# Tariq-Abuhashim/semantic-slam

Measured on AMD Instinct MI355X. Metric: Mvoxels/sec integrated, 512³ grid @ 640×480 depth; achieved HBM GB/s %peak, higher is better.
Workload: dtype f32

## Files before the change

### include/tsdf_hip_diag.h

```cpp
#ifndef TSDF_HIP_DIAG_H
#define TSDF_HIP_DIAG_H

#include "tsdf_hip.h"

#ifdef __cplusplus
extern "C" {
#endif


int tsdf_integrate_sequence_timed(tsdf_volume *vol, const float *depth_dev, const float *cam2world,
                                  int32_t n_frames, float *elapsed_ms);

int tsdf_integrate_frames_timed(tsdf_volume *vol, const float *const *depth_dev, const uint8_t *const *masks_dev,
                                const float *cam2world, int32_t n_frames, float *elapsed_ms);


int tsdf_probe_graph_replay(tsdf_volume *vol, const float *depth_dev, const float *cam2world, int32_t n_frames,
                            int32_t iters, float *ms_launches, float *ms_graph);

int tsdf_probe_stream(tsdf_volume *vol, int32_t non_temporal, int32_t n_iters, float *elapsed_ms);


int tsdf_selftest_fastdiv(int32_t device, uint64_t seed, uint64_t n_samples, float fx, float cx,
                          uint64_t *mismatches, float first_bad[4]);

int tsdf_selftest_fastdiv_band(int32_t device, uint64_t seed, uint64_t n_samples, uint64_t *mismatches,
                               float first_bad[4]);

int tsdf_selftest_round(int32_t device, uint64_t *mismatches, float first_bad[4]);

int tsdf_selftest_tile_tables(int32_t device, const float *depth_dev, const uint8_t *mask_dev, int32_t im_height,
                              int32_t im_width, float max_depth, uint64_t *mismatches);


int32_t tsdf_frames_per_launch(const tsdf_volume *vol);
int tsdf_shortcut_stats(tsdf_volume *vol, int32_t enable, uint64_t counts_out[3]);
int tsdf_brick_list_stats(tsdf_volume *vol, uint64_t counts_out[4]);
int tsdf_classification_info(tsdf_volume *vol, double info_out[2]);

int tsdf_last_cam2base(const tsdf_volume *vol, float out[16]);


int tsdf_set_kernel_variant(tsdf_volume *vol, int32_t variant);

int tsdf_set_brick_shape(tsdf_volume *vol, int32_t quads, int32_t rows, int32_t slices);
int tsdf_brick_shape(const tsdf_volume *vol, int32_t shape_out[3]);
int tsdf_default_brick_shape(const tsdf_config *cfg, int32_t shape_out[3]);

#ifdef __cplusplus
}
#endif
#endif
```

### semantic_slam_amd/capi.py

```python
import ctypes as C
import os

import numpy as np

_PKG = os.path.dirname(os.path.abspath(__file__))
LIB_PATH = os.environ.get("TSDF_HIP_LIB") or os.path.join(_PKG, "libtsdf_hip.so")

ABI_SYMBOLS = [
    "tsdf_config_default", "tsdf_create", "tsdf_destroy", "tsdf_reset", "tsdf_integrate",
    "tsdf_integrate_u16", "tsdf_convert_depth_u16", "tsdf_set_deferral",
    "tsdf_integrate_device", "tsdf_integrate_cam2base", "tsdf_integrate_masked_device",
    "tsdf_integrate_frames_device",
    "tsdf_sync", "tsdf_download", "tsdf_copy_slices", "tsdf_upload", "tsdf_refresh_summary", "tsdf_device_ptrs", "tsdf_slab_voxels", "tsdf_frames_per_launch", "tsdf_shortcut_stats", "tsdf_brick_list_stats", "tsdf_classification_info",
    "tsdf_get_config", "tsdf_last_cam2base", "tsdf_set_stream", "tsdf_get_stream",
    "tsdf_count_surface", "tsdf_extract_surface", "tsdf_extract_crossings", "tsdf_extract_mesh", "tsdf_save_mesh_ply", "tsdf_save_mesh_welded_ply", "tsdf_save_ply", "tsdf_save_bin", "tsdf_load_bin", "tsdf_save_state", "tsdf_load_state",
    "tsdf_integrate_sequence_timed", "tsdf_integrate_frames_timed", "tsdf_probe_graph_replay", "tsdf_probe_stream", "tsdf_selftest_fastdiv", "tsdf_selftest_fastdiv_band", "tsdf_selftest_round", "tsdf_selftest_tile_tables", "tsdf_set_kernel_variant", "tsdf_set_brick_shape", "tsdf_brick_shape", "tsdf_default_brick_shape", "tsdf_last_error",
    "tsdf_version", "tsdf_multiply_matrix", "tsdf_invert_matrix",
    "tsdf_labels_enable", "tsdf_compose_labels", "tsdf_integrate_labels_device", "tsdf_integrate_frames_labels_device",
    "tsdf_download_labels",
    "tsdf_colour_enable", "tsdf_integrate_colour_device", "tsdf_integrate_rgbd", "tsdf_download_colour",
    "tsdf_raycast_params_default", "tsdf_raycast_device", "tsdf_raycast", "tsdf_batch_raycast_device",
    "tsdf_track_params_default", "tsdf_track", "tsdf_track_system",
    "tsdf_batch_track", "tsdf_batch_track_system", "tsdf_track_member_systems",
    "tsdf_fuse_params_default", "tsdf_fuse_volume",
    "tsdf_extent_params_default", "tsdf_volume_extent", "tsdf_batch_extents", "tsdf_group_extent", "tsdf_extent_combine",
    "tsdf_extent_metric", "tsdf_extent_regrid",
    "tsdf_associate_params_default", "tsdf_associate_count", "tsdf_associate_assign", "tsdf_batch_associate",
    "tsdf_segment_params_default", "tsdf_segmenter_create", "tsdf_segmenter_destroy", "tsdf_segmenter_set_stream",
    "tsdf_segment_depth_device", "tsdf_segment_refine_masks_device", "tsdf_segment_frame",
    "tsdf_object_origin", "tsdf_batch_create", "tsdf_batch_destroy", "tsdf_batch_size", "tsdf_batch_volume",
    "tsdf_batch_integrate_device", "tsdf_batch_sync",
    "tsdf_group_create", "tsdf_group_destroy", "tsdf_group_size", "tsdf_group_voxels", "tsdf_group_volume",
    "tsdf_group_integrate", "tsdf_group_integrate_frames", "tsdf_group_set_deferral", "tsdf_group_sync", "tsdf_group_reset", "tsdf_group_download",
    "tsdf_group_extract_surface", "tsdf_group_extract_crossings", "tsdf_group_extract_mesh",
    "tsdf_group_save_ply", "tsdf_group_save_mesh_ply", "tsdf_group_save_bin",
]
DIAG_SYMBOLS = [
    "tsdf_integrate_sequence_timed", "tsdf_integrate_frames_timed",
    "tsdf_probe_graph_replay", "tsdf_probe_stream",
    "tsdf_selftest_fastdiv", "tsdf_selftest_fastdiv_band", "tsdf_selftest_round", "tsdf_selftest_tile_tables",
    "tsdf_shortcut_stats", "tsdf_brick_list_stats", "tsdf_classification_info", "tsdf_frames_per_launch", "tsdf_last_cam2base",
    "tsdf_set_kernel_variant", "tsdf_set_brick_shape", "tsdf_brick_shape", "tsdf_default_brick_shape",
]


class TsdfError(RuntimeError):
    pass


SHIPPED_VARIANTS = (0, 1, 3, 7, 8)


def experiments_build():
    return b"+experiments" in load().tsdf_version()


def variants(*wanted):
    exp = experiments_build()
    return [v for v in wanted if v in SHIPPED_VARIANTS or exp]


class TsdfConfig(C.Structure):
    _fields_ = [
        ("im_height", C.c_int32), ("im_width", C.c_int32),
        ("dim_x", C.c_int32), ("dim_y", C.c_int32), ("dim_z", C.c_int32),
        ("z_begin", C.c_int32), ("z_end", C.c_int32),
        ("voxel_size", C.c_float), ("trunc_margin", C.c_float), ("max_depth", C.c_float),
        ("origin", C.c_float * 3), ("cam_K", C.c_float * 9), ("base2world", C.c_float * 16),
        ("device", C.c_int32), ("id", C.c_int32),
    ]


class RaycastParams(C.Structure):
    _fields_ = [
        ("cam_K", C.c_float * 9), ("im_height", C.c_int32), ("im_width", C.c_int32),
        ("near_m", C.c_float), ("far_m", C.c_float), ("weight_thresh", C.c_float),
    ]


class TrackParams(C.Structure):
    _fields_ = [
        ("ray", RaycastParams), ("n_levels", C.c_int32), ("iters", C.c_int32 * 3), ("dist_thresh", C.c_float * 3),
        ("cos_normal_thresh", C.c_float), ("min_inliers", C.c_int32), ("eps_rot", C.c_float), ("eps_trans", C.c_float),
    ]


class TrackResult(C.Structure):
    _fields_ = [
        ("cam2world", C.c_float * 16), ("status", C.c_int32), ("iters_run", C.c_int32 * 3), ("inliers", C.c_int32),
        ("rmse", C.c_float),
    ]


class FuseParams(C.Structure):
    _fields_ = [("weight_thresh", C.c_float), ("agree_tol", C.c_float), ("write", C.c_int32)]


class FuseCounts(C.Structure):
    _fields_ = [("sampled", C.c_uint64), ("both", C.c_uint64), ("both_band", C.c_uint64), ("agree_band", C.c_uint64)]


class ExtentParams(C.Structure):
    _fields_ = [("weight_thresh", C.c_float), ("band", C.c_float), ("margin", C.c_int32)]


class Extent(C.Structure):
    _fields_ = [
        ("n_observed", C.c_uint64), ("n_surface", C.c_uint64), ("sum", C.c_uint64 * 3), ("sum2", C.c_uint64 * 6),
        ("border", C.c_uint64 * 6), ("lo", C.c_int32 * 3), ("hi", C.c_int32 * 3),
    ]

    def as_dict(self):
        return {"n_observed": int(self.n_observed), "n_surface": int(self.n_surface), "sum": [int(x) for x in self.sum],
                "sum2": [int(x) for x in self.sum2], "border": [int(x) for x in self.border], "lo": [int(x) for x in self.lo],
                "hi": [int(x) for x in self.hi]}

    @classmethod
    def from_dict(cls, d):
        e = cls()
        e.n_observed, e.n_surface = d["n_observed"], d["n_surface"]
        for name in ("sum", "sum2", "border", "lo", "hi"):
            getattr(e, name)[:] = d[name]
        return e


# ... 10 lines not shown


class AssociateLabels(C.Structure):
    _fields_ = [("mask_label", C.c_void_p), ("mask_score", C.c_void_p), ("member_label", C.c_void_p),
                ("member_score", C.c_void_p)]


class SegmentParams(C.Structure):
    _fields_ = [
        ("cam_K", C.c_float * 9), ("im_height", C.c_int32), ("im_width", C.c_int32), ("near_m", C.c_float), ("far_m", C.c_float),
        ("small_radius_m", C.c_float), ("large_radius_m", C.c_float), ("don_thresh", C.c_float), ("seg_radius_m", C.c_float),
        ("min_cluster", C.c_int32), ("max_cluster", C.c_int32), ("overlap", C.c_float), ("inset", C.c_int32),
    ]


TRACK_STATUS = {0: "converged", 1: "iterations exhausted", 2: "lost"}

_lib = None


def load():
    global _lib
    if _lib is not None:
        return _lib
    if not os.path.isfile(LIB_PATH):
        raise TsdfError(f"{LIB_PATH} not built: run `python -c 'import __graft_entry__ as g; g.build()'` "
                        "(there is no CPU fallback)")
    try:
        import torch
    except ImportError:
        pass
    L = C.CDLL(LIB_PATH)
    vp, f32p, i64p = C.c_void_p, C.POINTER(C.c_float), C.POINTER(C.c_int64)
    L.tsdf_config_default.argtypes = [C.POINTER(TsdfConfig), C.c_int32, C.c_int32]
    L.tsdf_create.argtypes = [C.POINTER(TsdfConfig), C.POINTER(vp)]
    L.tsdf_destroy.argtypes = [vp]
    L.tsdf_reset.argtypes = [vp]
    L.tsdf_integrate.argtypes = [vp, vp, vp]
    L.tsdf_set_deferral.argtypes = [vp, C.c_int32]
    L.tsdf_integrate_u16.argtypes = [vp, vp, C.c_float, C.c_int32, C.c_int32, vp]
    L.tsdf_convert_depth_u16.argtypes = [vp, vp, vp, C.c_float, C.c_int32, C.c_int32]
    L.tsdf_integrate_device.argtypes = [vp, vp, vp]
    L.tsdf_integrate_cam2base.argtypes = [vp, vp, vp]
    L.tsdf_integrate_masked_device.argtypes = [vp, vp, vp, vp]
    L.tsdf_integrate_frames_device.argtypes = [vp, vp, vp, vp, C.c_int32]
    L.tsdf_sync.argtypes = [vp]
    L.tsdf_download.argtypes = [vp, vp, vp]
    L.tsdf_upload.argtypes = [vp, vp, vp]
    L.tsdf_copy_slices.argtypes = [vp, C.c_int32, C.c_int32, vp, vp]
    L.tsdf_refresh_summary.argtypes = [vp]
    L.tsdf_device_ptrs.argtypes = [vp, C.POINTER(vp), C.POINTER(vp)]
    L.tsdf_slab_voxels.argtypes = [vp]
    L.tsdf_slab_voxels.restype = C.c_int64
    L.tsdf_frames_per_launch.argtypes = [vp]
    L.tsdf_frames_per_launch.restype = C.c_int32
    L.tsdf_shortcut_stats.argtypes = [vp, C.c_int32, vp]
    L.tsdf_classification_info.argtypes = [vp, vp]
    L.tsdf_brick_list_stats.argtypes = [vp, vp]
    L.tsdf_get_config.argtypes = [vp, C.POINTER(TsdfConfig)]
    L.tsdf_last_cam2base.argtypes = [vp, vp]
    L.tsdf_set_stream.argtypes = [vp, vp]
    L.tsdf_get_stream.argtypes = [vp, C.POINTER(vp)]
    L.tsdf_count_surface.argtypes = [vp, C.c_float, i64p]
    L.tsdf_extract_surface.argtypes = [vp, C.c_float, vp, C.c_int64, i64p]
    L.tsdf_extract_crossings.argtypes = [vp, vp, vp, C.c_float, vp, C.c_int64, i64p]
    L.tsdf_extract_mesh.argtypes = [vp, vp, vp, C.c_float, vp, C.c_int64, i64p]
    L.tsdf_save_mesh_ply.argtypes = [vp, C.c_char_p, C.c_float]
    L.tsdf_save_mesh_welded_ply.argtypes = [vp, C.c_char_p, C.c_float]
    L.tsdf_save_ply.argtypes = [vp, C.c_char_p, C.c_float]
    L.tsdf_save_bin.argtypes = [vp, C.c_char_p]
    L.tsdf_load_bin.argtypes = [vp, C.c_char_p]
    L.tsdf_save_state.argtypes = [vp, C.c_char_p]
    L.tsdf_load_state.argtypes = [vp, C.c_char_p]
    L.tsdf_integrate_sequence_timed.argtypes = [vp, vp, vp, C.c_int32, f32p]
    L.tsdf_integrate_frames_timed.argtypes = [vp, vp, vp, vp, C.c_int32, f32p]
    L.tsdf_probe_graph_replay.argtypes = [vp, vp, vp, C.c_int32, C.c_int32, f32p, f32p]
    L.tsdf_probe_stream.argtypes = [vp, C.c_int32, C.c_int32, f32p]
    L.tsdf_selftest_fastdiv.argtypes = [C.c_int32, C.c_uint64, C.c_uint64, C.c_float, C.c_float, C.POINTER(C.c_uint64), f32p]
    L.tsdf_selftest_fastdiv_band.argtypes = [C.c_int32, C.c_uint64, C.c_uint64, C.POINTER(C.c_uint64), f32p]
    L.tsdf_selftest_round.argtypes = [C.c_int32, C.POINTER(C.c_uint64), f32p]
    L.tsdf_selftest_tile_tables.argtypes = [C.c_int32, vp, vp, C.c_int32, C.c_int32, C.c_float, C.POINTER(C.c_uint64)]
    L.tsdf_set_kernel_variant.argtypes = [vp, C.c_int32]
    L.tsdf_set_brick_shape.argtypes = [vp, C.c_int32, C.c_int32, C.c_int32]
    L.tsdf_brick_shape.argtypes = [vp, C.POINTER(C.c_int32)]
    L.tsdf_default_brick_shape.argtypes = [C.POINTER(TsdfConfig), C.POINTER(C.c_int32)]
    L.tsdf_last_error.restype = C.c_char_p
    L.tsdf_version.restype = C.c_char_p
    L.tsdf_multiply_matrix.argtypes = [vp, vp, vp]
    L.tsdf_multiply_matrix.restype = None
    L.tsdf_invert_matrix.argtypes = [vp, vp]
    L.tsdf_labels_enable.argtypes = [vp, C.c_float]
    L.tsdf_compose_labels.argtypes = [vp, vp, vp, vp, C.c_int32, vp, vp]
    L.tsdf_integrate_labels_device.argtypes = [vp, vp, vp, vp, vp]
    L.tsdf_download_labels.argtypes = [vp, vp, vp, vp]
    L.tsdf_integrate_frames_labels_device.argtypes = [vp, vp, vp, vp, vp, C.c_int32]
    L.tsdf_colour_enable.argtypes = [vp]
    L.tsdf_integrate_colour_device.argtypes = [vp, vp, vp, vp]
    L.tsdf_integrate_rgbd.argtypes = [vp, vp, vp, vp]
    L.tsdf_download_colour.argtypes = [vp, vp]
    L.tsdf_raycast_params_default.argtypes = [C.POINTER(TsdfConfig), C.POINTER(RaycastParams)]
    L.tsdf_raycast_device.argtypes = [vp, C.POINTER(RaycastParams), vp, vp, vp, vp, vp]
    L.tsdf_raycast.argtypes = [vp, C.POINTER(RaycastParams), vp, vp, vp, vp, vp]
    L.tsdf_batch_raycast_device.argtypes = [vp, C.POINTER(RaycastParams), vp, vp, vp, vp]
    L.tsdf_track_params_default.argtypes = [C.POINTER(TsdfConfig), C.POINTER(TrackParams)]
    L.tsdf_track.argtypes = [vp, C.POINTER(TrackParams), vp, vp, vp, C.POINTER(TrackResult)]
    L.tsdf_track_system.argtypes = [vp, C.POINTER(TrackParams), vp, vp, vp, vp, C.c_int32, vp]
    L.tsdf_batch_track.argtypes = [vp, C.POINTER(TrackParams), vp, vp, vp, vp, C.POINTER(TrackResult), vp]
    L.tsdf_batch_track_system.argtypes = [vp, C.POINTER(TrackParams), vp, vp, vp, vp, C.c_int32, vp]
    L.tsdf_track_member_systems.argtypes = [C.c_int32, C.POINTER(TrackParams), vp, vp, vp, C.c_int32, vp, vp, vp, vp,
                                            C.c_int32, vp]
    L.tsdf_fuse_params_default.argtypes = [C.POINTER(TsdfConfig), C.POINTER(FuseParams)]
    L.tsdf_fuse_volume.argtypes = [vp, vp, C.POINTER(FuseParams), C.POINTER(FuseCounts)]
    L.tsdf_extent_params_default.argtypes = [C.POINTER(TsdfConfig), C.POINTER(ExtentParams)]
    L.tsdf_volume_extent.argtypes = [vp, C.POINTER(ExtentParams), C.POINTER(Extent)]
    L.tsdf_batch_extents.argtypes = [vp, C.POINTER(ExtentParams), C.POINTER(Extent)]
    L.tsdf_group_extent.argtypes = [vp, C.POINTER(ExtentParams), C.POINTER(Extent)]
    L.tsdf_extent_combine.argtypes = [C.POINTER(Extent), C.POINTER(Extent), C.POINTER(Extent)]
    L.tsdf_extent_metric.argtypes = [C.POINTER(TsdfConfig), C.POINTER(Extent), C.POINTER(ExtentMetric)]
    L.tsdf_extent_regrid.argtypes = [C.POINTER(TsdfConfig), C.POINTER(Extent), C.c_int32, C.c_int32, C.POINTER(TsdfConfig)]
    L.tsdf_associate_params_default.argtypes = [C.POINTER(TsdfConfig), C.POINTER(AssociateParams)]
    L.tsdf_associate_count.argtypes = [C.c_int32, C.POINTER(AssociateParams), vp, vp, C.c_int32, vp, vp, C.c_int32, vp]
    L.tsdf_associate_assign.argtypes = [C.POINTER(AssociateParams), vp, C.c_int32, C.c_int32, C.POINTER(AssociateLabels), vp,
                                        vp]
    L.tsdf_batch_associate.argtypes = [vp, C.POINTER(AssociateParams), vp, vp, vp, C.c_int32, C.POINTER(AssociateLabels),
                                       vp, vp, vp]
    L.tsdf_segment_params_default.argtypes = [C.POINTER(TsdfConfig), C.POINTER(SegmentParams)]
    L.tsdf_segmenter_create.argtypes = [C.c_int32, C.c_int32, C.c_int32, C.POINTER(vp)]
    L.tsdf_segmenter_destroy.argtypes = [vp]
    L.tsdf_segmenter_set_stream.argtypes = [vp, vp]
    L.tsdf_segment_depth_device.argtypes = [vp, C.POINTER(SegmentParams), vp, vp, vp, C.POINTER(C.c_int32)]
    L.tsdf_segment_refine_masks_device.argtypes = [vp, C.POINTER(SegmentParams), vp, C.c_int32, vp, C.c_int32, vp, vp]
    L.tsdf_segment_frame.argtypes = [vp, C.POINTER(SegmentParams), vp, vp, C.c_int32, vp, vp, C.POINTER(C.c_int32)]
    L.tsdf_object_origin.argtypes = [C.c_int32, vp, vp, C.c_int32, C.c_int32, vp, vp]
    L.tsdf_batch_create.argtypes = [C.POINTER(TsdfConfig), C.c_int32, C.POINTER(vp)]
    L.tsdf_batch_destroy.argtypes = [vp]
    L.tsdf_batch_size.argtypes = [vp]
    L.tsdf_batch_volume.argtypes = [vp, C.c_int32, C.POINTER(vp)]
    L.tsdf_batch_integrate_device.argtypes = [vp, vp, vp, vp]
    L.tsdf_batch_sync.argtypes = [vp]
    L.tsdf_group_create.argtypes = [C.POINTER(TsdfConfig), C.POINTER(C.c_int32), C.c_int32, C.POINTER(vp)]
    L.tsdf_group_destroy.argtypes = [vp]
    L.tsdf_group_size.argtypes = [vp]
    L.tsdf_group_voxels.argtypes = [vp]
    L.tsdf_group_voxels.restype = C.c_int64
    L.tsdf_group_volume.argtypes = [vp, C.c_int32, C.POINTER(vp)]
    L.tsdf_group_integrate.argtypes = [vp, vp, vp]
    L.tsdf_group_integrate_frames.argtypes = [vp, vp, vp, C.c_int32]
    L.tsdf_group_set_deferral.argtypes = [vp, C.c_int32]
    L.tsdf_group_sync.argtypes = [vp]
    L.tsdf_group_reset.argtypes = [vp]
    L.tsdf_group_download.argtypes = [vp, vp, vp]
    for name in ("tsdf_group_extract_surface", "tsdf_group_extract_crossings", "tsdf_group_extract_mesh"):
        getattr(L, name).argtypes = [vp, C.c_float, vp, C.c_int64, i64p]
    L.tsdf_group_save_ply.argtypes = [vp, C.c_char_p, C.c_float]
    L.tsdf_group_save_mesh_ply.argtypes = [vp, C.c_char_p, C.c_float]
    L.tsdf_group_save_bin.argtypes = [vp, C.c_char_p]
    _lib = L
    return L


def check(rc, what=""):
    if rc != 0:
        raise TsdfError(f"{what} failed ({rc}): {load().tsdf_last_error().decode()}")


def _f32(a, n=None):
# ... 346 lines not shown
        check(self.lib.tsdf_integrate_sequence_timed(self._h, depth_ptr, p.ctypes.data, n, C.byref(ms)),
              "tsdf_integrate_sequence_timed")
        return ms.value

    def integrate_frames_timed(self, depth_ptrs, poses, mask_ptrs=None):
        p = _f32(np.asarray(poses, dtype=np.float32))
        n = p.size // 16
        assert len(depth_ptrs) == n
        d = (C.c_void_p * n)(*[C.c_void_p(x) for x in depth_ptrs])
        m = None
        if mask_ptrs is not None:
            m = (C.c_void_p * n)(*[C.c_void_p(x) if x else C.c_void_p() for x in mask_ptrs])
        ms = C.c_float()
        check(self.lib.tsdf_integrate_frames_timed(self._h, d, m, p.ctypes.data, n, C.byref(ms)),
              "tsdf_integrate_frames_timed")
        return ms.value

    def frames_timed_call(self, depth_ptrs, poses, mask_ptrs=None):
        p = _f32(np.asarray(poses, dtype=np.float32))
        n = p.size // 16
        assert len(depth_ptrs) == n
        d = (C.c_void_p * n)(*depth_ptrs)
        m = None
        if mask_ptrs is not None:
            m = (C.c_void_p * n)(*[x if x else None for x in mask_ptrs])
        ms = C.c_float()

        def call():
            check(self.lib.tsdf_integrate_frames_timed(self._h, d, m, p.ctypes.data, n, C.byref(ms)), "tsdf_integrate_frames_timed")
            return ms.value
        return call

    def probe_graph_replay(self, depth_ptr, poses, iters=20):
        p = _f32(np.asarray(poses, dtype=np.float32))
        a, b = C.c_float(), C.c_float()
        check(self.lib.tsdf_probe_graph_replay(self._h, depth_ptr, p.ctypes.data, p.size // 16, iters, C.byref(a), C.byref(b)),
              "tsdf_probe_graph_replay")
        return a.value, b.value

    def probe_stream(self, non_temporal=False, iters=20):
        ms = C.c_float()
        check(self.lib.tsdf_probe_stream(self._h, int(non_temporal), iters, C.byref(ms)), "tsdf_probe_stream")
        return ms.value / iters

    def last_cam2base(self):
        out = np.empty(16, np.float32)
        check(self.lib.tsdf_last_cam2base(self._h, out.ctypes.data), "tsdf_last_cam2base")
        return out

    def sync(self):
        check(self.lib.tsdf_sync(self._h), "tsdf_sync")

    def reset(self):
        check(self.lib.tsdf_reset(self._h), "tsdf_reset")

    def download(self):
        n = self.n_voxels
        t, w = np.empty(n, np.float32), np.empty(n, np.float32)
        check(self.lib.tsdf_download(self._h, t.ctypes.data, w.ctypes.data), "tsdf_download")
        return t, w

    def copy_slices(self, z_local, n_slices):
        n = n_slices * self.cfg.dim_x * self.cfg.dim_y
        t, w = np.empty(n, np.float32), np.empty(n, np.float32)
        check(self.lib.tsdf_copy_slices(self._h, z_local, n_slices, t.ctypes.data, w.ctypes.data), "tsdf_copy_slices")
        return t, w

    def copy_slices_to_device(self, z_local, n_slices, tsdf_ptr, weight_ptr):
        check(self.lib.tsdf_copy_slices(self._h, z_local, n_slices, tsdf_ptr, weight_ptr), "tsdf_copy_slices")

    def upload(self, tsdf, weight):
        t, w = _f32(tsdf, self.n_voxels), _f32(weight, self.n_voxels)
        check(self.lib.tsdf_upload(self._h, t.ctypes.data, w.ctypes.data), "tsdf_upload")

    def set_stream(self, stream_ptr):
        check(self.lib.tsdf_set_stream(self._h, stream_ptr), "tsdf_set_stream")

    def set_kernel_variant(self, v):
        check(self.lib.tsdf_set_kernel_variant(self._h, v), "tsdf_set_kernel_variant")

    def set_brick_shape(self, quads=0, rows=0, slices=0):
        check(self.lib.tsdf_set_brick_shape(self._h, quads, rows, slices), "tsdf_set_brick_shape")

    def brick_shape(self):
        out = (C.c_int32 * 3)()
        check(self.lib.tsdf_brick_shape(self._h, out), "tsdf_brick_shape")
        return tuple(out)

    def labels_enable(self, prob_threshold=0.5):
        check(self.lib.tsdf_labels_enable(self._h, prob_threshold), "tsdf_labels_enable")

    def compose_labels(self, masks_ptr, labels, scores, label_im_ptr, score_im_ptr):
        lab = np.ascontiguousarray(labels, np.uint16)
        sc = _f32(scores)
        check(self.lib.tsdf_compose_labels(self._h, masks_ptr, lab.ctypes.data, sc.ctypes.data, lab.size,
                                           label_im_ptr, score_im_ptr), "tsdf_compose_labels")

    def integrate_labels_device(self, depth_ptr, label_im_ptr, score_im_ptr, cam2world):
        p = _f32(cam2world, 16)
        check(self.lib.tsdf_integrate_labels_device(self._h, depth_ptr, label_im_ptr, score_im_ptr, p.ctypes.data),
              "tsdf_integrate_labels_device")

    def integrate_frames_labels_device(self, depth_ptrs, label_im_ptrs, score_im_ptrs, poses):
        p = _f32(np.asarray(poses, dtype=np.float32))
        n = p.size // 16
        assert len(depth_ptrs) == len(label_im_ptrs) == len(score_im_ptrs) == n
        arr = lambda xs: (C.c_void_p * n)(*[C.c_void_p(x) for x in xs])
        check(self.lib.tsdf_integrate_frames_labels_device(self._h, arr(depth_ptrs), arr(label_im_ptrs), arr(score_im_ptrs),
                                                           p.ctypes.data, n), "tsdf_integrate_frames_labels_device")

    def download_labels(self):
        n = self.n_voxels
        lab, fp, bp = np.empty(n, np.uint16), np.empty(n, np.float32), np.empty(n, np.float32)
        check(self.lib.tsdf_download_labels(self._h, lab.ctypes.data, fp.ctypes.data, bp.ctypes.data), "tsdf_download_labels")
        return lab, fp, bp

    def colour_enable(self):
        check(self.lib.tsdf_colour_enable(self._h), "tsdf_colour_enable")

    def integrate_colour_device(self, depth_ptr, rgb_ptr, cam2world):
        p = _f32(cam2world, 16)
        check(self.lib.tsdf_integrate_colour_device(self._h, depth_ptr, rgb_ptr, p.ctypes.data), "tsdf_integrate_colour_device")

    def integrate_rgbd(self, depth_host, rgb_host, cam2world):
        d = _f32(depth_host, self.cfg.im_height * self.cfg.im_width)
        c = np.ascontiguousarray(rgb_host, dtype=np.uint8).ravel()
        if c.size != 3 * self.cfg.im_height * self.cfg.im_width:
            raise ValueError("colour image must be height x width x 3 bytes")
        p = _f32(cam2world, 16)
        check(self.lib.tsdf_integrate_rgbd(self._h, d.ctypes.data, c.ctypes.data, p.ctypes.data), "tsdf_integrate_rgbd")

    def download_colour(self):
        out = np.empty(self.n_voxels, np.uint32)
        check(self.lib.tsdf_download_colour(self._h, out.ctypes.data), "tsdf_download_colour")
        return out

    def raycast(self, cam2world, params=None, normals=True, labels=False, colour=False):
        p = raycast_params_default(self.cfg) if params is None else params
        h, w = p.im_height, p.im_width
        out = {"depth": np.empty((h, w), np.float32)}
        if normals:
            out["normal"] = np.empty((h, w, 3), np.float32)
        if labels:
            out["label"] = np.empty((h, w), np.uint16)
        if colour:
            out["colour"] = np.empty((h, w), np.uint32)
        ptr = lambda k: out[k].ctypes.data if k in out else None
        c2w = _f32(cam2world, 16)
        check(self.lib.tsdf_raycast(self._h, C.byref(p), c2w.ctypes.data, ptr("depth"), ptr("normal"), ptr("label"),
                                    ptr("colour")), "tsdf_raycast")
        return out

    def raycast_device(self, cam2world, depth_ptr, normal_ptr=None, label_ptr=None, colour_ptr=None, params=None):
        p = raycast_params_default(self.cfg) if params is None else params
        c2w = _f32(cam2world, 16)
        check(self.lib.tsdf_raycast_device(self._h, C.byref(p), c2w.ctypes.data, depth_ptr, normal_ptr, label_ptr, colour_ptr),
              "tsdf_raycast_device")

    def track(self, depth_ptr, guess_cam2world, params=None, mask_ptr=None):
        p = track_params_default(self.cfg) if params is None else params
        guess = _f32(guess_cam2world, 16)
        res = TrackResult()
        check(self.lib.tsdf_track(self._h, C.byref(p), depth_ptr, mask_ptr, guess.ctypes.data, C.byref(res)), "tsdf_track")
        pose = np.array(res.cam2world, np.float32).reshape(4, 4)
        stats = {"status": res.status, "status_name": TRACK_STATUS[res.status], "iters_run": list(res.iters_run),
                 "inliers": res.inliers, "rmse": res.rmse}
# ... 286 lines not shown
```

### semantic_slam_amd/csrc/frame_store.h

```cpp
#pragma once
#include <hip/hip_runtime.h>

#include <mutex>
#include <thread>
#include <utility>
#include <vector>

#include "hip_owned.h"

namespace tsdf_store {

constexpr int kRingSlots = 4;
constexpr int kSoftCapFrames = 160;
constexpr int kSoftCapTables = 16;

struct Slot {
    hip_owned::DevPtr<void> dev;
    const hip_owned::Event *release = nullptr;
    const void *owner = nullptr;
    int state = 0;
    unsigned long long seq = 0;
};

struct RingSlot {
// ... 14 lines not shown
    int device = 0;
    size_t px = 0;
    int refs = 0;
    std::mutex mu;
    RingSlot ring[kRingSlots];
    int ring_next = 0;
    SlotClass frames, masks, tables;
    hip_owned::Stream copy_stream;
};

inline std::mutex &registry_mutex() { static std::mutex m; return m; }
inline std::vector<FrameStore *> &registry() { static std::vector<FrameStore *> r; return r; }

inline hipError_t store_ref(int device, size_t px, size_t table_bytes, FrameStore **out)
{
    std::lock_guard<std::mutex> lk(registry_mutex());
    for (FrameStore *s : registry())
        if (s->device == device && s->px == px && s->tables.bytes == table_bytes) { ++s->refs; *out = s; return hipSuccess; }
    FrameStore *s = new FrameStore();
    s->device = device; s->px = px; s->refs = 1;
    s->frames.bytes = px * sizeof(float); s->frames.soft_cap = kSoftCapFrames; s->frames.quota = 64;
    s->masks.bytes = px; s->masks.soft_cap = kSoftCapFrames; s->masks.quota = 64;
    s->tables.bytes = table_bytes; s->tables.soft_cap = kSoftCapTables; s->tables.quota = 2;
    (void)hipSetDevice(device);
    const hipError_t e = hip_owned::stream_create(s->copy_stream);
    if (e != hipSuccess) { delete s; return e; }
    registry().push_back(s);
    *out = s;
    return hipSuccess;
}

inline void store_unref(FrameStore *s)
{
    if (!s) return;
    std::lock_guard<std::mutex> lk(registry_mutex());
    if (--s->refs > 0) return;
    (void)hipSetDevice(s->device);
    if (s->copy_stream) (void)hipStreamSynchronize(s->copy_stream);
    for (RingSlot &slot : s->ring)
        if (slot.copied) (void)hipEventSynchronize(slot.copied);
    auto &r = registry();
    for (size_t i = 0; i < r.size(); ++i) if (r[i] == s) { r.erase(r.begin() + (long)i); break; }
    delete s;
}

inline hipError_t ring_acquire(FrameStore *s, int *index)
{
    int i = -1;
    for (;;) {
        {
            std::lock_guard<std::mutex> lk(s->mu);
            for (int k = 0; k < kRingSlots; ++k) {
                const int j = (s->ring_next + k) % kRingSlots;
                if (!s->ring[j].busy) { i = j; s->ring[j].busy = true; s->ring_next = (j + 1) % kRingSlots; break; }
            }
        }
        if (i >= 0) break;
        std::this_thread::yield();
    }
    RingSlot &r = s->ring[i];
    hipError_t e = hipSuccess;
    if (!r.host) {
        hip_owned::HostPtr<float> host;
        hip_owned::Event copied;
        e = hip_owned::host_alloc(host, s->px * sizeof(float), hipHostMallocPortable);
        if (e == hipSuccess) e = hip_owned::event_create(copied);
        if (e == hipSuccess) { r.host = std::move(host); r.copied = std::move(copied); }
    }
    if (e == hipSuccess && r.used) e = hipEventSynchronize(r.copied);
    if (e != hipSuccess) { std::lock_guard<std::mutex> lk(s->mu); r.busy = false; return e; }
    *index = i;
    return hipSuccess;
}

inline hipError_t ring_release(FrameStore *s, int i, hipStream_t stream)
{
    const hipError_t e = hipEventRecord(s->ring[i].copied, stream);
    std::lock_guard<std::mutex> lk(s->mu);
    s->ring[i].used = true;
    s->ring[i].busy = false;
    return e;
}

inline hipError_t slot_acquire(FrameStore *s, SlotClass *c, const void *owner, hipStream_t first_user, bool force, int *index, void **dev)
{
    std::lock_guard<std::mutex> lk(s->mu);
    *index = -1;
    int pick = -1, mine = -1, oldest = -1, own = 0;
    for (size_t i = 0; i < c->slots.size(); ++i) {
        const Slot &x = c->slots[i];
        if (x.state == 0) { if (pick < 0) pick = (int)i; continue; }
        if (x.owner == owner) ++own;
        if (x.state != 2) continue;
        if (x.owner == owner && (mine < 0 || x.seq < c->slots[(size_t)mine].seq)) mine = (int)i;
        if (oldest < 0 || x.seq < c->slots[(size_t)oldest].seq) oldest = (int)i;
    }
    const bool at_cap = (int)c->slots.size() >= c->soft_cap;
    int wait_for = -1;
    if (pick < 0 && mine >= 0 && (own >= c->quota || at_cap)) wait_for = mine;
    else if (pick < 0 && at_cap && oldest >= 0) wait_for = oldest;
    if (wait_for >= 0) {
        const hipError_t e = hipStreamWaitEvent(first_user, *c->slots[(size_t)wait_for].release, 0);
        if (e != hipSuccess) return e;
        pick = wait_for;
    }
    if (pick < 0) {
        if (at_cap && !force) return hipSuccess;
        Slot x;
        const hipError_t e = hip_owned::dev_alloc(x.dev, c->bytes ? c->bytes : 1);
        if (e != hipSuccess) return e;
        c->slots.push_back(std::move(x));
        pick = (int)c->slots.size() - 1;
    }
    Slot &x = c->slots[(size_t)pick];
    x.state = 1; x.owner = owner; x.release = nullptr;
    *index = pick;
    *dev = x.dev;
    return hipSuccess;
}

inline void slots_release_after(FrameStore *s, SlotClass *c, const int *idx, int n, const hip_owned::Event *release, const void *owner)
{
    std::lock_guard<std::mutex> lk(s->mu);
    for (int k = 0; k < n; ++k) {
        if (idx[k] < 0) continue;
        Slot &x = c->slots[(size_t)idx[k]];
        x.state = 2; x.release = release; x.owner = owner; x.seq = ++c->seq;
    }
}

inline void slots_drop_owner(FrameStore *s, const void *owner)
{
    std::lock_guard<std::mutex> lk(s->mu);
    for (SlotClass *c : {&s->frames, &s->masks, &s->tables})
        for (Slot &x : c->slots)
            if (x.state != 0 && x.owner == owner) { x.state = 0; x.release = nullptr; x.owner = nullptr; }
}

inline size_t store_device_bytes(FrameStore *s)
{
    std::lock_guard<std::mutex> lk(s->mu);
    size_t b = 0;
    for (SlotClass *c : {&s->frames, &s->masks, &s->tables}) b += c->slots.size() * c->bytes;
    return b;
}

}
```

### semantic_slam_amd/csrc/host_derive.h

```cpp
#pragma once
#include <algorithm>
#include <cmath>
#include <cstddef>
#include <cstdint>

#include "tsdf_hip.h"

namespace tsdf_host {

inline bool brick_shape_ok(const tsdf_config &c, int q, int r, int s)
{
    return c.dim_x % 4 == 0 && q >= 1 && r >= 1 && s >= 1 && q * r * s <= 64 && (c.dim_x / 4) % q == 0 &&
           (long long)s * c.dim_x * c.dim_y < (1ll << 30);
}

inline void choose_brick_default(const tsdf_config &c, int &bq, int &br, int &bs)
{
    bq = 0; br = 0; bs = 1;
    if (c.dim_x % 4 != 0) return;
    const int quads = c.dim_x / 4;
    const int nz = c.z_end - c.z_begin;
    double best = 1e300;
    for (int q = 1; q <= 64 && q <= quads; ++q) {
        if (quads % q) continue;
        for (int sl = 1; q * sl <= 64 && sl <= std::max(nz, 1); ++sl) {
            const int r = std::min(64 / (q * sl), std::max(c.dim_y, 1));
            if (!brick_shape_ok(c, q, r, sl)) continue;
            const double X = 4.0 * q, Y = r, Z = sl;
            const double cost = (X + 8.0) * (Y + 8.0) * (Z + 10.0) / (X * Y * Z) * (1.0 + 0.25 / q) * 64.0 / (q * r * sl);
            if (cost < best) { best = cost; bq = q; br = r; bs = sl; }
        }
    }
}

struct ProjectionGuards {
    float cz_margin;
    int fast_ok;
    int trunc_fast;
    float cz_short;
    float cz_pad;
    float px_margin_u, px_margin_v;
};

inline ProjectionGuards derive_projection_guards(const tsdf_config &c, const float *c2b)
{
    ProjectionGuards g;
    const double fx = c.cam_K[0], fy = c.cam_K[4], cx = c.cam_K[2], cy = c.cam_K[5];
    const double ext[3] = {(double)(c.dim_x - 1) * c.voxel_size, (double)(c.dim_y - 1) * c.voxel_size,
                           (double)(c.dim_z - 1) * c.voxel_size};
    const double o[3] = {c.origin[0], c.origin[1], c.origin[2]}, t[3] = {c2b[3], c2b[7], c2b[11]};
    double dmax[3];
    for (int k = 0; k < 3; ++k) dmax[k] = std::fmax(std::fabs(o[k] - t[k]), std::fabs(o[k] + ext[k] - t[k])) * 1.001 + 1e-30;
    const double rows[3][3] = {{c2b[0], c2b[4], c2b[8]}, {c2b[1], c2b[5], c2b[9]}, {c2b[2], c2b[6], c2b[10]}};
    bool ok = true;
    double bz = 0;
    for (int i = 0; i < 3; ++i) {
        double b = 0;
        for (int k = 0; k < 3; ++k) b += std::fabs(rows[i][k]) * dmax[k];
        ok = ok && (b < 5.7e17);
        if (i == 2) bz = b;
    }
    g.cz_margin = ok ? (float)std::fmax(1e-5 * bz, 1e-17) : 3.0e38f;
    ok = ok && std::fabs(fx) < 16384.0 && std::fabs(fy) < 16384.0 &&
         std::fabs(cx) < 1048576.0 && std::fabs(cy) < 1048576.0 &&
         (int64_t)c.im_width * c.im_height <= (1 << 24) &&
         c.im_width < (1 << 24) && c.im_height < (1 << 24);
    g.fast_ok = ok ? 1 : 0;
    g.trunc_fast = (ok && c.trunc_margin >= 9.5367431640625e-07f && c.trunc_margin <= 1048576.0f &&
                    c.max_depth <= 5.7e17f) ? 1 : 0;
    double bmax = 0, eps = 0;
    for (int i = 0; i < 3; ++i) {
        double b = 0, e = 0;
        for (int k = 0; k < 3; ++k) {
            const double Ek = 1.2e-7 * (std::fabs(o[k]) + ext[k] + std::fabs(t[k])) + 6e-8 * dmax[k];
            b += std::fabs(rows[i][k]) * dmax[k];
            e += std::fabs(rows[i][k]) * Ek;
        }
        bmax = std::fmax(bmax, b);
        eps = std::fmax(eps, 2.0 * (e + 3.0e-7 * b));
    }
    const bool sok = ok && bmax > 0 && eps < 1e30;
    g.cz_short = sok ? (float)(std::fmax(bmax / 64.0, eps / 3.2e-5) * 1.0001) : 3.0e38f;
    g.cz_pad = sok ? (float)(std::fmax(2.0 * eps, (double)g.cz_margin) * 1.0001) : 3.0e38f;
    g.px_margin_u = (float)(0.5625 + 3.2e-5 * (std::fabs(fx) + 4.0 * (c.im_width + std::fabs(cx))));
    g.px_margin_v = (float)(0.5625 + 3.2e-5 * (std::fabs(fy) + 4.0 * (c.im_height + std::fabs(cy))));
    return g;
}

constexpr int kMaxFramesPerLaunch = 32;
constexpr int kTileLdsEntries = 5120;
constexpr int kFineTile = 4;
constexpr int kFineLevels = 3;

enum class Classify { Adaptive, Never, Always };

struct Variant {
    bool known = false;
    bool fuses = false;
    bool scalar = false;
    Classify classify = Classify::Adaptive;
};

inline Variant decode_variant(int variant)
{
    switch (variant) {
        case 0: return {true, true, false, Classify::Adaptive};
        case 1: return {true, false, true, Classify::Adaptive};
        case 3: return {true, false, false, Classify::Adaptive};
        case 7: return {true, true, false, Classify::Never};
        case 8: return {true, true, false, Classify::Always};
        default: return {};
    }
}

inline int64_t slab_voxels(const tsdf_config &c) { return (int64_t)c.dim_x * c.dim_y * (int64_t)(c.z_end - c.z_begin); }

inline int tile_levels(int n) { int l = 0; while (n > 0) { ++l; n >>= 1; } return l; }

inline size_t tile_table_elems(int tiles_w, int tiles_h)
{
    return (size_t)tile_levels(tiles_w) * tile_levels(tiles_h) * tiles_w * tiles_h;
}

constexpr int64_t kMaxTableTiles = 16384;
inline bool tiles_fit(int tiles_w, int tiles_h) { return (int64_t)tiles_w * tiles_h <= kMaxTableTiles; }

constexpr int64_t kFineTileMinVoxels = 10000000;
inline int tile_edge(const tsdf_config &c, bool batch_member)
{
    const int64_t fine_tiles = (int64_t)((c.im_width + 7) / 8) * ((c.im_height + 7) / 8);
    return (!batch_member && slab_voxels(c) >= kFineTileMinVoxels && fine_tiles <= kTileLdsEntries) ? 8 : 16;
}

constexpr int64_t kFineLevelMinVoxels = 64000000;
inline bool fine_tables(const tsdf_config &c, int tile) { return tile == 8 && slab_voxels(c) >= kFineLevelMinVoxels; }

inline size_t launch_table_bytes(const tsdf_config &c, int tile, bool fine)
{
    const int tw = (c.im_width + tile - 1) / tile, th = (c.im_height + tile - 1) / tile;
    const int fw = (c.im_width + kFineTile - 1) / kFineTile, fh = (c.im_height + kFineTile - 1) / kFineTile;
    const size_t fine_elems = fine ? (size_t)kFineLevels * kFineLevels * fw * fh : 0;
    return tiles_fit(tw, th) ? kMaxFramesPerLaunch * (tile_table_elems(tw, th) + fine_elems) * (2 * sizeof(float)) : 0;
}

constexpr int64_t kPipelineMaxVoxels = 64000000;
inline bool pipelines(const tsdf_config &c) { return slab_voxels(c) < kPipelineMaxVoxels; }

constexpr int64_t kClassifyMinVoxels = 48000000;
inline bool classify_one_frame(Classify mode, int64_t launch_voxels)
{
    if (mode == Classify::Never) return false;
    return mode == Classify::Always || launch_voxels >= kClassifyMinVoxels;
}

constexpr double kMinClaimFraction = 0.10;
constexpr int kProbeEvery = 8;
inline bool classify_fused(Classify mode, bool claims_known, double claim_fraction, int launches_unclassified)
{
    if (mode != Classify::Adaptive) return mode == Classify::Always;
    return !claims_known || claim_fraction >= kMinClaimFraction || launches_unclassified >= kProbeEvery - 1;
}

constexpr int64_t kWindowBytes = 512ll << 20;

struct SweepWindow { int cache_lo, cache_hi; };

inline SweepWindow sweep_window(int nz, int dim_x, int dim_y, int64_t window_bytes, bool reverse)
{
    const int64_t slice_bytes = 8 * (int64_t)dim_x * dim_y;
    const int w = (int)std::min<int64_t>(nz, window_bytes / slice_bytes);
    return reverse ? SweepWindow{0, w} : SweepWindow{nz - w, nz};
}

inline bool batch_defers(int members, int64_t total_voxels) { return 2 * (int64_t)members < 10 + total_voxels / 1000000; }

constexpr int64_t kBatchMinVoxelsPerMember = 2000000;
inline bool batch_classifies(Classify mode, int members, int64_t launch_voxels)
{
    const bool big_enough = mode == Classify::Always || launch_voxels >= (int64_t)members * kBatchMinVoxelsPerMember;
    return big_enough && classify_one_frame(mode, launch_voxels);
}

constexpr int kBatchSideStreams = 4;
inline int batch_lanes(int members) { return members < 8 ? 1 : kBatchSideStreams; }

struct Regions {
    size_t add(size_t bytes) { const size_t at = (end_ + 255) / 256 * 256; end_ = at + bytes; return at; }
    size_t total() const { return end_; }
    size_t end_ = 0;
};

}
```

### semantic_slam_amd/csrc/tsdf_capi.hip

```cpp
#include "../../include/tsdf_hip.h"
#include "../../include/tsdf_hip_diag.h"

#include <hip/hip_runtime.h>

#include <algorithm>
#include <cmath>
#include <cstdarg>
#include <cstdio>
#include <cstdlib>
#include <cstring>
#include <new>
#include <string>
#include <vector>

#include "pose_math.h"
#include "host_derive.h"
#include "host_copy.h"
#include "hip_owned.h"
#include "frame_store.h"
#include "tsdf_kernels.hip.h"
#include "tsdf_multiframe.hip.h"
#include "tsdf_labels.hip.h"
#include "tsdf_colour.hip.h"
#include "tsdf_extract.hip.h"
#include "tsdf_raycast.hip.h"
#include "tsdf_track.hip.h"
#include "tsdf_batch_track.hip.h"
#include "tsdf_fuse.hip.h"
#include "tsdf_extent.hip.h"
#include "tsdf_associate.hip.h"
#include "tsdf_segment.hip.h"
#ifdef TSDF_EXPERIMENTS
#include "tsdf_experiments.hip.h"
#endif

using namespace hip_owned;

namespace {

thread_local std::string g_last_error;

int fail(int code, const char *fmt, ...)
{
    char buf[512];
    va_list ap;
    va_start(ap, fmt);
    vsnprintf(buf, sizeof buf, fmt, ap);
    va_end(ap);
    g_last_error = buf;
    return code;
}

#define HIP_TRY_OR(undo, expr)                                                                 \
    do {                                                                                       \
        hipError_t _e = (expr);                                                                \
        if (_e != hipSuccess)                                                                  \
            return undo(fail(TSDF_ERR_HIP, "%s failed: %s (%s:%d)", #expr,                     \
                             hipGetErrorString(_e), __FILE__, __LINE__));                      \
    } while (0)
#define HIP_TRY(expr) HIP_TRY_OR(, expr)

constexpr int kStageSlots = 3;

#ifdef TSDF_EXPERIMENTS
constexpr bool kExperiments = true;
#else
constexpr bool kExperiments = false;
#endif

#ifndef TSDF_BRICK_NT
#define TSDF_BRICK_NT 0
#endif
constexpr bool kBrickNT = TSDF_BRICK_NT != 0;
constexpr size_t kClaimBlockBytes = (tsdfk::kCounterBytes + sizeof(tsdfk::ClassPoseTable) + 255) / 256 * 256;
#ifndef TSDF_WEDGE_MODE
#define TSDF_WEDGE_MODE 0
#endif
constexpr int kWedgeMode = TSDF_WEDGE_MODE;

}

struct tsdf_volume {
    tsdf_config cfg = {};
    float base2world_inv[16] = {};
    float last_cam2base[16] = {};
    int64_t n_vox = 0;
    DevPtr<float> d_tsdf;
    DevPtr<float> d_weight;
    Stream own_stream;
    hipStream_t stream = nullptr;
    tsdf_store::FrameStore *store = nullptr;
    hipStream_t copy_stream = nullptr;
    Event flush_done[2];
    int flush_parity = 0;
    int table_slot = -1;
    int defer_n = tsdfk::kMaxFramesPerLaunch;
    Event pend_copied;
    int pend_count = 0;
    int pend_slot[tsdfk::kMaxFramesPerLaunch] = {}, pend_mask_slot[tsdfk::kMaxFramesPerLaunch] = {};
    const float *pend_depth[tsdfk::kMaxFramesPerLaunch] = {};
    struct tsdf_batch *owner = nullptr;
    struct tsdf_group *group_owner = nullptr;
    bool in_flush = false;
    float pend_c2b[16 * tsdfk::kMaxFramesPerLaunch] = {};
    const uint8_t *pend_mask[tsdfk::kMaxFramesPerLaunch] = {};
    int variant = 0;
    int sweep_parity = 0;
#ifdef TSDF_EXPERIMENTS
    StageRing<Staged<tsdfk::FramePose>, kStageSlots> frames;
#endif
    DevPtr<uint16_t> d_label;
    DevPtr<float> d_fp, d_bp;
    float prob_thd = 0.0f;
    DevPtr<uint32_t> d_colour;
    StageRing<Staged<uint8_t>, kStageSlots> rgb;
    DevPtr<uint32_t> d_flags;
    size_t n_flags = 0;
    int nseg = 0;
    int chunks_per_slice = 0;
    bool flat = false;
    int brick_q = 0, brick_r = 0, brick_s = 0;
    int tile = 0;
    bool fine_tables = false;
    bool flags_known_zero = false;
#ifdef TSDF_EXPERIMENTS
    DevBuf<unsigned int> d_super;
#endif
    DevBuf<uint4> d_work;
    int64_t work_nsuper = 0, work_bucket_supers = 0;
    int work_wedge_mode = -1;
    DevPtr<unsigned int> d_shortcut_stats;
    DevPtr<unsigned long long> d_claims;
    HostPtr<unsigned long long> h_claims;
    Event claims_done;
    Stream pre_stream, rb_stream;
    int rb_parity = -1;
    Event pre_done[2], list_free[2], seq_ready;
    int list_parity = 0;
    bool list_used[2] = {false, false};
    bool pipeline_ok = false;
    bool claims_pending = false, claims_known = false;
    double claims_total = 0.0;
    double claim_fraction = 0.0;
    int launches_unclassified = 0;
    DevBuf<char> d_scratch;
    DevBuf<uint8_t> d_wg_class;
    DevBuf<char> d_list;
    DevBuf<char> d_track;
    HostPtr<tsdfk::TrackState> h_track;
    DevPtr<unsigned long long> d_fuse;
    HostPtr<unsigned long long> h_fuse;
    Event fuse_src_ready, fuse_done;
    DevPtr<unsigned long long> d_extent;
    HostPtr<unsigned long long> h_extent;
};

using tsdf_host::kBatchSideStreams;

struct tsdf_batch {
    int device = 0;
    std::vector<tsdf_volume *> vols;
    Stream stream;
    struct FrameBlocks { Staged<tsdfk::IntegrateParams> params; Staged<tsdfk::FramePose> poses; };
    StageRing<FrameBlocks, kStageSlots> blocks;
    DevPtr<int2> d_slice_map;
    int total_slices = 0, max_blocks = 0;
    DevPtr<int2> d_group_map;
    int total_groups = 0;
    std::vector<int> group_s;
    DevPtr<float2> d_tiles;
    size_t tiles_per_object = 0;
    DevPtr<uint8_t> d_wg_class;
    DevBuf<uint8_t> d_brick_class;
    DevPtr<float> d_depth_pool;
    DevPtr<uint8_t> d_mask_pool;
    std::vector<float> pend_c2b;
    std::vector<const uint8_t *> pend_mask;
    int pend_count = 0;
    bool in_flush = false;
    Stream side[kBatchSideStreams];
    Event side_done[kBatchSideStreams];
    Event collected;
    StageRing<Staged<tsdfk::RayVolume>, 1> ray;
    DevBuf<char> d_assoc;
    HostBuf<uint32_t> h_assoc;
    DevBuf<char> d_track;
    HostBuf<char> h_track;
    DevPtr<unsigned long long> d_extent;
    HostPtr<unsigned long long> h_extent;
    Staged<tsdfk::ExtentVolume> extent_vols;
    int extent_blocks = 0;
};

namespace {

int flush_pending(tsdf_volume *v);
int batch_flush(tsdf_batch *b);
int group_flush(tsdf_group *g);
int batch_collect(tsdf_batch *b, const float *depth_dev, const uint8_t *const *masks_dev, const float cam2world[16]);

int bind_device(tsdf_volume *v, bool flush = true)
{
    HIP_TRY(hipSetDevice(v->cfg.device));
    if (v->owner && !v->in_flush) {
        int rc = batch_flush(v->owner);
        if (rc) return rc;
    }
    if (v->group_owner && !v->in_flush) {
        int rc = group_flush(v->group_owner);
        if (rc) return rc;
    }
    if (flush && v->pend_count > 0 && !v->in_flush) return flush_pending(v);
    return TSDF_OK;
}

int store_slot(tsdf_volume *v, tsdf_store::SlotClass *c, hipStream_t first_user, int *index, void **dev)
{
    hipError_t e = tsdf_store::slot_acquire(v->store, c, v, first_user, false, index, dev);
    if (e == hipSuccess && *index < 0) {
        if (v->pend_count > 0 && !v->in_flush) {
            int rc = flush_pending(v);
            if (rc) return rc;
        }
        e = tsdf_store::slot_acquire(v->store, c, v, first_user, true, index, dev);
    }
    if (e != hipSuccess) return fail(TSDF_ERR_HIP, "frame store: %s", hipGetErrorString(e));
    return TSDF_OK;
}

int store_release(tsdf_volume *v, tsdf_store::SlotClass *c, const int *idx, int n)
{
    const Event *evt = &v->flush_done[v->flush_parity];
    HIP_TRY(hipEventRecord(*evt, v->stream));
    tsdf_store::slots_release_after(v->store, c, idx, n, evt, v);
    return TSDF_OK;
}

void store_next_pass(tsdf_volume *v) { v->flush_parity ^= 1; }

int tables_begin(tsdf_volume *v, float2 **tiles, hipStream_t first_user = nullptr)
{
    void *dev = nullptr;
    hipError_t e = tsdf_store::slot_acquire(v->store, &v->store->tables, v, first_user ? first_user : v->stream, true, &v->table_slot, &dev);
    if (e != hipSuccess) return fail(TSDF_ERR_HIP, "frame store (tile tables): %s", hipGetErrorString(e));
    *tiles = static_cast<float2 *>(dev);
    return TSDF_OK;
}

int tables_end(tsdf_volume *v)
{
    if (v->table_slot < 0) return TSDF_OK;
    const int slot = v->table_slot;
    v->table_slot = -1;
    return store_release(v, &v->store->tables, &slot, 1);
}

using tsdf_host::brick_shape_ok;

void choose_brick_for(const tsdf_config &c, int &bq, int &br, int &bs)
{
#ifdef TSDF_EXPERIMENTS
    if (const char *e = std::getenv("TSDF_BRICK3D")) {
        int q = 0, r = 0, sl = 0;
        if (c.dim_x % 4 == 0 && std::sscanf(e, "%d,%d,%d", &q, &r, &sl) == 3 && brick_shape_ok(c, q, r, sl)) {
            bq = q; br = r; bs = sl;
            return;
        }
    }
#endif
    tsdf_host::choose_brick_default(c, bq, br, bs);
}

void choose_brick(tsdf_volume *v) { choose_brick_for(v->cfg, v->brick_q, v->brick_r, v->brick_s); }

tsdfk::IntegrateParams make_params(const tsdf_volume *v, const float *depth_dev,
                                   const uint8_t *mask_dev, const float *c2b, int vx)
{
    const tsdf_config &c = v->cfg;
    tsdfk::IntegrateParams p;
    p.depth = depth_dev;
    p.mask = mask_dev;
    p.tsdf = v->d_tsdf;
    p.weight = v->d_weight;
    p.fx = c.cam_K[0]; p.fy = c.cam_K[4]; p.cx = c.cam_K[2]; p.cy = c.cam_K[5];
    p.rx0 = c2b[0]; p.rx1 = c2b[4]; p.rx2 = c2b[8];
    p.ry0 = c2b[1]; p.ry1 = c2b[5]; p.ry2 = c2b[9];
    p.rz0 = c2b[2]; p.rz1 = c2b[6]; p.rz2 = c2b[10];
    p.tx = c2b[3]; p.ty = c2b[7]; p.tz = c2b[11];
    p.ox = c.origin[0]; p.oy = c.origin[1]; p.oz = c.origin[2];
    p.vs = c.voxel_size; p.trunc = c.trunc_margin; p.max_depth = c.max_depth;
    p.dim_x = c.dim_x; p.dim_y = c.dim_y;
    p.nz = c.z_end - c.z_begin; p.z_begin = c.z_begin;
    p.H = c.im_height; p.W = c.im_width;
    p.xgroups = (c.dim_x + vx - 1) / vx;
    p.flags = v->d_flags;
    p.nseg = v->nseg;
    p.quads_per_row = c.dim_x / 4;
    p.quads_per_slice = (int)((int64_t)c.dim_x * c.dim_y / 4);
    p.chunks_per_slice = v->chunks_per_slice;
    p.brick_q = v->brick_q; p.brick_r = v->brick_r; p.brick_s = v->brick_s > 0 ? v->brick_s : 1;
    p.bricks_per_group = 0; p.brick_groups = 0;
    p.brick_q_magic = 0; p.brick_per_magic = 0;
    if (p.brick_q > 0) {
        p.bricks_per_group = p.quads_per_row / p.brick_q;
        p.brick_groups = (c.dim_y + p.brick_r - 1) / p.brick_r;
        p.brick_q_magic = 65536 / p.brick_q + 1;
        p.brick_per_magic = 65536 / (p.brick_q * p.brick_r) + 1;
    }
    const tsdf_host::ProjectionGuards g = tsdf_host::derive_projection_guards(c, c2b);
    p.cz_margin = g.cz_margin; p.fast_ok = g.fast_ok; p.trunc_fast = g.trunc_fast;
    p.cz_short = g.cz_short; p.cz_pad = g.cz_pad;
    p.tiles_w = (c.im_width + v->tile - 1) / v->tile;
    p.tiles_h = (c.im_height + v->tile - 1) / v->tile;
    p.tile_inv = 1.0f / (float)v->tile;
    p.fine = nullptr;
    p.fine_w = v->fine_tables ? (c.im_width + tsdfk::kFineTile - 1) / tsdfk::kFineTile : 0;
    p.fine_h = v->fine_tables ? (c.im_height + tsdfk::kFineTile - 1) / tsdfk::kFineTile : 0;
    p.px_margin_u = g.px_margin_u; p.px_margin_v = g.px_margin_v;
    p.shortcut_stats = v->d_shortcut_stats;
    p.claim_counter = nullptr;
    p.wg_class = nullptr;
    return p;
}

void pose_from_params(tsdfk::FramePose &fp, const tsdfk::IntegrateParams &q)
{
    fp.depth = q.depth; fp.mask = q.mask;
    fp.rx0 = q.rx0; fp.rx1 = q.rx1; fp.rx2 = q.rx2;
    fp.ry0 = q.ry0; fp.ry1 = q.ry1; fp.ry2 = q.ry2;
    fp.rz0 = q.rz0; fp.rz1 = q.rz1; fp.rz2 = q.rz2;
    fp.tx = q.tx; fp.ty = q.ty; fp.tz = q.tz;
    fp.fast_ok = q.fast_ok; fp.cz_margin = q.cz_margin;
    fp.label_im = nullptr; fp.score_im = nullptr;
    fp.tiles = nullptr;
    fp.cz_short = q.cz_short; fp.cz_pad = q.cz_pad;
}

static_assert(tsdf_host::kMaxFramesPerLaunch == tsdfk::kMaxFramesPerLaunch, "host_derive.h: kMaxFramesPerLaunch");
static_assert(tsdf_host::kTileLdsEntries == tsdfk::kTileLdsEntries, "host_derive.h: kTileLdsEntries");
static_assert(tsdf_host::kFineTile == tsdfk::kFineTile, "host_derive.h: kFineTile");
static_assert(tsdf_host::kFineLevels == tsdfk::kFineLevels, "host_derive.h: kFineLevels");
using tsdf_host::tiles_fit;

int build_tile_tables(hipStream_t stream, const tsdf_config &c, const tsdfk::IntegrateParams &p, const float *const *depth,
                      const uint8_t *const *masks, int n, float2 *tables, unsigned long long *zero_me = nullptr, float2 *fine = nullptr,
                      bool beside_a_launch = false)
{
    const size_t per = tsdf_host::tile_table_elems(p.tiles_w, p.tiles_h);
    if (fine != nullptr && (p.tile_inv != 0.125f || n > tsdfk::kMaxFramesPerLaunch))
        return fail(TSDF_ERR_INVALID, "build_tile_tables: fine tables go with 8-pixel tiles, one launch at a time");
    for (int k = 0; k < n; k += tsdfk::kMaxFramesPerLaunch) {
        const int m = std::min(tsdfk::kMaxFramesPerLaunch, n - k);
        tsdfk::TileSummaryParams tp;
        for (int f = 0; f < tsdfk::kMaxFramesPerLaunch; ++f) {
            tp.depth[f] = depth[k + (f < m ? f : 0)];
            tp.mask[f] = masks ? masks[k + (f < m ? f : 0)] : nullptr;
        }
        tp.tiles = tables + (size_t)k * per;
        tp.H = c.im_height; tp.W = c.im_width; tp.tiles_w = p.tiles_w; tp.tiles_h = p.tiles_h;
        tp.max_depth = c.max_depth;
        tp.fine = fine; tp.fw = p.fine_w; tp.fh = p.fine_h;
        if (p.tile_inv == 0.0625f) {
            const int strips = ((p.tiles_w + 3) / 4) * p.tiles_h;
            hipLaunchKernelGGL(tsdfk::depth_tile_summary<16>, dim3((unsigned)((strips + 3) / 4), m), dim3(64, 4), 0, stream, tp);
        } else {
            const int strips = ((p.tiles_w + 7) / 8) * p.tiles_h;
            hipLaunchKernelGGL(tsdfk::depth_tile_summary<8>, dim3((unsigned)((strips + 3) / 4), m), dim3(64, 4), 0, stream, tp);
        }
        if (p.tiles_w * p.tiles_h <= tsdfk::kTileLdsEntries) {
            const unsigned threads = (p.tiles_w * p.tiles_h > 2048 && !beside_a_launch) ? 1024 : 256;
            const unsigned fine_blocks = fine ? ((unsigned)(p.fine_w * p.fine_h) + threads - 1) / threads : 0u;
            hipLaunchKernelGGL(tsdfk::tile_sparse_table, dim3((unsigned)tsdf_host::tile_levels(p.tiles_w) + fine_blocks, m), dim3(threads), 0, stream, tp.tiles,
                               p.tiles_w, p.tiles_h, k == 0 ? zero_me : (unsigned long long *)nullptr, fine, p.fine_w, p.fine_h);
        } else {
            if (zero_me && k == 0) HIP_TRY(hipMemsetAsync(zero_me, 0, tsdfk::kCounterBytes, stream));
            hipLaunchKernelGGL(tsdfk::tile_sparse_table_scan, dim3((unsigned)tsdf_host::tile_levels(p.tiles_w), m), dim3(256), 0, stream, tp.tiles,
                               p.tiles_w, p.tiles_h);
            if (fine)
                hipLaunchKernelGGL(tsdfk::fine_tile_levels, dim3((unsigned)((p.fine_w * p.fine_h + 255) / 256), m), dim3(256), 0, stream, fine, p.fine_w, p.fine_h);
        }
    }
    HIP_TRY(hipGetLastError());
    return TSDF_OK;
}

int launch_masked_bricks(tsdf_volume *v, tsdfk::IntegrateParams &p)
{
    const int blocks = (p.brick_groups * p.bricks_per_group + 3) / 4, nz = (p.nz + p.brick_s - 1) / p.brick_s;
    float2 *tiles = nullptr;
    int rc0 = tables_begin(v, &tiles);
    if (rc0) return rc0;
    const size_t n_bricks = (size_t)blocks * nz * 4;
    HIP_TRY(v->d_wg_class.ensure(n_bricks));
    const float *d = p.depth;
    const uint8_t *m = p.mask;
    int rc = build_tile_tables(v->stream, v->cfg, p, &d, &m, 1, tiles);
    if (rc) return rc;
    tsdfk::FramePose pose;
    pose_from_params(pose, p);
    pose.tiles = tiles;
    hipLaunchKernelGGL(tsdfk::classify_bricks, dim3((unsigned)((n_bricks + 255) / 256)), dim3(256), 0, v->stream, p, pose,
                       v->d_wg_class, blocks, nz);
    p.wg_class = v->d_wg_class;
    hipLaunchKernelGGL((tsdfk::integrate_single_bricks<kBrickNT>), dim3(blocks, 1, nz), dim3(64, 4, 1), 0, v->stream, p, pose);
    HIP_TRY(hipGetLastError());
    return tables_end(v);
}

int drop_summary(tsdf_volume *v)
{
    if (v->flags_known_zero || v->n_flags == 0) return TSDF_OK;
    HIP_TRY(hipMemsetAsync(v->d_flags, 0, v->n_flags * sizeof(uint32_t), v->stream));
    v->flags_known_zero = true;
    return TSDF_OK;
}

int rebuild_summary(tsdf_volume *v)
{
    if (v->n_flags == 0 || v->n_vox == 0) return TSDF_OK;
    const int nz = v->cfg.z_end - v->cfg.z_begin;
    const int qps = (int)((int64_t)v->cfg.dim_x * v->cfg.dim_y / 4);
// ... 66 lines not shown
#endif
    const tsdf_host::Variant var = variant_of(v->variant);
    if (c.dim_x % 4 != 0 || var.scalar) {
        int rc = drop_summary(v);
        if (rc) return rc;
        const tsdfk::IntegrateParams p = make_params(v, depth_dev, mask_dev, c2b, 1);
        dim3 block(64, 4, 1), grid((c.dim_x + 63) / 64, (c.dim_y + 3) / 4, nz);
        if (mask_dev) hipLaunchKernelGGL((tsdfk::integrate_scalar<true>), grid, block, 0, v->stream, p);
        else hipLaunchKernelGGL((tsdfk::integrate_scalar<false>), grid, block, 0, v->stream, p);
        HIP_TRY(hipGetLastError());
        return TSDF_OK;
    }
    if (v->flat) {
        return launch_multi(v, &depth_dev, mask_dev ? &mask_dev : nullptr, c2b, 1);
    }
    tsdfk::IntegrateParams p = make_params(v, depth_dev, mask_dev, c2b, 4);
    v->flags_known_zero = false;
    const dim3 block(64, 4, 1), grid((p.xgroups + 63) / 64, (p.dim_y + 7) / 8, p.nz);
    if (mask_dev) {
        const bool classify = tsdf_host::classify_one_frame(var.classify, v->n_vox) && tiles_fit(p.tiles_w, p.tiles_h);
        if (classify && p.brick_q > 0 && (!kExperiments || v->variant != 11)) {
            int rc = launch_masked_bricks(v, p);
            if (rc) return rc;
        } else {
#ifdef TSDF_EXPERIMENTS
            if (v->variant == 11 && classify) return launch_integrate_experiment(v, depth_dev, mask_dev, c2b);
#endif
            set_sweep(v, p);
            hipLaunchKernelGGL((tsdfk::integrate_tile<2, true>), grid, block, 0, v->stream, p);
        }
    } else {
        set_sweep(v, p);
        hipLaunchKernelGGL((tsdfk::integrate_tile<2, false>), grid, block, 0, v->stream, p);
    }
    HIP_TRY(hipGetLastError());
    return TSDF_OK;
}

void compose_cam2base(const tsdf_volume *v, const float *cam2world, float *c2b)
{
    tsdf_host::multiply_matrix(v->base2world_inv, cam2world, c2b);
}

int launch_multi(tsdf_volume *v, const float *const *depth_dev, const uint8_t *const *masks_dev,
                 const float *c2b, int n, const uint16_t *const *label_ims, const float *const *score_ims, hipEvent_t inputs_ready)
{
    const tsdf_config &c = v->cfg;
    const int nz = c.z_end - c.z_begin;
    if (nz == 0 || n == 0) return TSDF_OK;
    auto fill_pose = [&](tsdfk::FramePose &fp, int f) {
        pose_from_params(fp, make_params(v, depth_dev[f], masks_dev ? masks_dev[f] : nullptr, c2b + 16 * f, 4));
        fp.label_im = label_ims ? label_ims[f] : nullptr;
        fp.score_im = label_ims ? score_ims[f] : nullptr;
    };
    const dim3 block(64, 4, 1);
    if (n == 1 && !label_ims) {
        tsdfk::IntegrateParams common = make_params(v, depth_dev[0], nullptr, c2b, 4);
        tsdfk::FramePose pose;
        fill_pose(pose, 0);
        std::memcpy(v->last_cam2base, c2b, sizeof v->last_cam2base);
        v->flags_known_zero = false;
#ifdef TSDF_EXPERIMENTS
        {
            bool handled = false;
            int rc = launch_single_experiment(v, common, pose, depth_dev[0], c2b, &handled);
            if (rc || handled) return rc;
        }
#endif
        if (v->flat && pose.mask != nullptr && tsdf_host::classify_one_frame(variant_of(v->variant).classify, v->n_vox) &&
            tiles_fit(common.tiles_w, common.tiles_h) && common.brick_q > 0) {
            tsdfk::IntegrateParams cp = make_params(v, depth_dev[0], pose.mask, c2b, 4);
            return launch_masked_bricks(v, cp);
        }
        if (v->flat) {
            dim3 grid((v->chunks_per_slice + 3) / 4, 1, nz);
            hipLaunchKernelGGL((tsdfk::integrate_multi_single<true, true>), grid, block, 0, v->stream, common, pose);
        } else {
            dim3 grid((common.xgroups + 63) / 64, (c.dim_y + 3) / 4, nz);
            hipLaunchKernelGGL((tsdfk::integrate_multi_single<true, false>), grid, block, 0, v->stream, common, pose);
        }
        HIP_TRY(hipGetLastError());
        return TSDF_OK;
    }
    std::memcpy(v->last_cam2base, c2b + 16 * (n - 1), sizeof v->last_cam2base);
    v->flags_known_zero = false;
    tsdfk::MultiParamsInline mi;
    mi.common = make_params(v, depth_dev[0], nullptr, c2b, 4);
    mi.n_frames = n;
    for (int f = 0; f < n; ++f) fill_pose(mi.frames[f], f);
    for (int f = n; f < tsdfk::kMaxFramesPerLaunch; ++f) mi.frames[f] = mi.frames[0];
    mi.labels.label = v->d_label; mi.labels.fp = v->d_fp; mi.labels.bp = v->d_bp; mi.labels.prob_thd = v->prob_thd;
    bool any_mask = false;
    for (int f = 0; f < n && masks_dev; ++f) any_mask = any_mask || masks_dev[f] != nullptr;

    if (v->claims_pending) {
        const hipError_t qe = hipEventQuery(v->claims_done);
        if (qe == hipSuccess) {
            v->claim_fraction = claims_read_back(v);
            v->claims_pending = false;
            v->claims_known = true;
        } else if (qe == hipErrorNotReady) {
            (void)hipGetLastError();
        } else {
            v->claims_pending = false;
            v->claims_known = false;
            (void)hipGetLastError();
            return fail(TSDF_ERR_HIP, "claims read-back: hipEventQuery failed: %s", hipGetErrorString(qe));
        }
    }
    bool classify = tiles_fit(mi.common.tiles_w, mi.common.tiles_h) && mi.common.brick_q > 0;
    mi.z_fastest = 2;
#ifdef TSDF_EXPERIMENTS
    experiment_adjust(v, label_ims != nullptr, &classify, &mi.z_fastest);
#endif
    classify = classify && tsdf_host::classify_fused(variant_of(v->variant).classify, v->claims_known, v->claim_fraction,
                                                     v->launches_unclassified);
    v->launches_unclassified = classify ? 0 : v->launches_unclassified + 1;
    const bool count_claims = classify && !v->claims_pending;
    if (classify && !v->d_claims) {
        DevPtr<unsigned long long> dc;
        HostPtr<unsigned long long> hc;
        Event ev[6];
        hipError_t e = dev_alloc(dc, 2 * kClaimBlockBytes);
        if (e == hipSuccess) e = host_alloc(hc, tsdfk::kCounterBytes, hipHostMallocDefault);
        for (int i = 0; i < 6 && e == hipSuccess; ++i) e = event_create(ev[i]);
        if (e != hipSuccess) return fail(TSDF_ERR_HIP, "claim counters: %s", hipGetErrorString(e));
        v->d_claims = std::move(dc); v->h_claims = std::move(hc); v->claims_done = std::move(ev[0]);
        v->pre_done[0] = std::move(ev[1]); v->pre_done[1] = std::move(ev[2]); v->list_free[0] = std::move(ev[3]);
        v->list_free[1] = std::move(ev[4]); v->seq_ready = std::move(ev[5]);
    }
    const int P = v->pipeline_ok ? v->list_parity : 0;
    unsigned long long *const claims_p = classify ? v->d_claims + (size_t)P * (kClaimBlockBytes / sizeof(unsigned long long)) : nullptr;
    bool pipelined = classify && inputs_ready != nullptr && v->pipeline_ok;
#ifdef TSDF_EXPERIMENTS
    if (!tsdf_host::decode_variant(v->variant).known || std::getenv("TSDF_NO_PIPELINE")) pipelined = false;
#endif
    if (pipelined && !v->pre_stream) {
        Stream a, b;
        int prio = 0;
#ifdef TSDF_EXPERIMENTS
        if (std::getenv("TSDF_PRE_PRIORITY")) { int lo = 0, hi = 0; (void)hipDeviceGetStreamPriorityRange(&lo, &hi); prio = hi; }
#endif
        hipError_t e = hipStreamCreateWithPriority(a.put(), hipStreamNonBlocking, prio);
        if (e == hipSuccess) e = stream_create(b);
        if (e != hipSuccess) return fail(TSDF_ERR_HIP, "side streams: %s", hipGetErrorString(e));
        v->pre_stream = std::move(a); v->rb_stream = std::move(b);
    }
    const int nz_groups = (nz + mi.common.brick_s - 1) / mi.common.brick_s;
    bool listed = classify;
#ifdef TSDF_EXPERIMENTS
    listed = listed && !experiment_takes_multi(v, label_ims != nullptr, classify);
#endif
    tsdfk::BrickListParams bl;
    int64_t n_super = 0, cap = 0;
    const size_t lists = v->pipeline_ok ? 2 : 1;
    if (listed) {
        bl.nsx = (mi.common.bricks_per_group + tsdfk::kSuperBX - 1) / tsdfk::kSuperBX;
        bl.nsy = (mi.common.brick_groups + tsdfk::kSuperBY - 1) / tsdfk::kSuperBY;
        bl.nsz = (nz_groups + tsdfk::kSuperBZ - 1) / tsdfk::kSuperBZ;
        bl.wedge_mode = kWedgeMode;
#ifdef TSDF_EXPERIMENTS
        if (const char *e = std::getenv("TSDF_WEDGE_MODE")) bl.wedge_mode = std::atoi(e);
#endif
        bl.super_h = tsdfk::kSuperBY * mi.common.brick_r;
        bl.super_d = tsdfk::kSuperBZ * mi.common.brick_s;
        bl.wedge_oy = (int)std::lround(std::fmax(-30000.0, std::fmin(30000.0, (double)c.origin[1] / c.voxel_size)));
        bl.wedge_oz = (int)std::lround(std::fmax(-30000.0, std::fmin(30000.0, (double)c.origin[2] / c.voxel_size + c.z_begin)));
        bl.fy_px = (int)std::lround(std::fmax(1.0, std::fmin(16000.0, std::fabs((double)c.cam_K[4]))));
        if (!(c.voxel_size > 0) || std::isnan(c.origin[1]) || std::isnan(c.origin[2])) bl.wedge_mode = 0;
        n_super = (int64_t)bl.nsx * bl.nsy * bl.nsz;
        if (v->work_nsuper != n_super || v->work_wedge_mode != bl.wedge_mode) {
            std::vector<int64_t> per((size_t)tsdfk::kListBuckets, 0);
            for (int64_t id = 0; id < n_super; ++id) {
                const int sz = (int)(id % bl.nsz), sx = (int)((id / bl.nsz) % bl.nsx), sy = (int)((id / bl.nsz) / bl.nsx);
                ++per[(size_t)tsdfk::list_bucket((unsigned int)id, sx, sy, sz, bl)];
            }
            v->work_bucket_supers = *std::max_element(per.begin(), per.end());
            v->work_nsuper = n_super;
            v->work_wedge_mode = bl.wedge_mode;
        }
        cap = v->work_bucket_supers * tsdfk::kSuperBricks;
        const int64_t total = cap * tsdfk::kListBuckets;
        if (total > 0x7fffffffll - 1024) return fail(TSDF_ERR_INVALID, "fused launch: %lld bricks exceed the work list's 32-bit index", (long long)total);
        if (!v->d_work.fits(lists * (size_t)total) && v->d_work) {
            if (v->pre_stream) HIP_TRY(hipStreamSynchronize(v->pre_stream));
            HIP_TRY(hipStreamSynchronize(v->stream));
        }
        HIP_TRY(v->d_work.ensure(lists * (size_t)total));
    }
    const hipStream_t ps = pipelined ? v->pre_stream : v->stream;
    auto unwind = [&](int code) {
        if (pipelined && hipEventRecord(v->pre_done[P], ps) == hipSuccess) (void)hipStreamWaitEvent(v->stream, v->pre_done[P], 0);
        (void)tables_end(v);
        return code;
    };
    if (pipelined) {
        HIP_TRY_OR(unwind, hipStreamWaitEvent(ps, inputs_ready, 0));
        if (v->list_used[P]) HIP_TRY_OR(unwind, hipStreamWaitEvent(ps, v->list_free[P], 0));
        if (v->rb_parity == P) HIP_TRY_OR(unwind, hipStreamWaitEvent(ps, v->claims_done, 0));
    } else if (classify && v->rb_parity == P) {
        HIP_TRY(hipStreamWaitEvent(v->stream, v->claims_done, 0));
    }
    if (count_claims) mi.common.claim_counter = claims_p + 1;
    if (classify) {
        const size_t per_frame = tsdf_host::tile_table_elems(mi.common.tiles_w, mi.common.tiles_h);
        float2 *tiles = nullptr;
        int rc = tables_begin(v, &tiles, ps);
        if (rc) return unwind(rc);
        float2 *fine = v->fine_tables ? tiles + (size_t)tsdfk::kMaxFramesPerLaunch * per_frame : nullptr;
        rc = build_tile_tables(ps, c, mi.common, depth_dev, masks_dev, n, tiles, claims_p, fine, pipelined);
        if (rc) return unwind(rc);
        mi.common.fine = fine;
        for (int f = 0; f < n; ++f) mi.frames[f].tiles = tiles + (size_t)f * per_frame;
        for (int f = n; f < tsdfk::kMaxFramesPerLaunch; ++f) mi.frames[f] = mi.frames[0];
    }
    double claims_total = 0.0;
    bool launched = false;
#ifdef TSDF_EXPERIMENTS
    {
        int rc = launch_multi_experiment(v, mi, depth_dev, masks_dev, c2b, n, label_ims != nullptr, any_mask, classify, &launched, &claims_total);
        if (rc) return unwind(rc);
    }
#endif
    if (listed) {
        const int64_t per_group = (int64_t)mi.common.brick_groups * mi.common.bricks_per_group;
        uint4 *const work_p = v->d_work + (size_t)P * (v->d_work.capacity() / lists);
        bl.list = work_p;
        bl.counters = reinterpret_cast<unsigned char *>(claims_p);
        bl.bucket_cap = (unsigned int)cap;
        bl.poses = reinterpret_cast<tsdfk::ClassPoseTable *>(bl.counters + tsdfk::kCounterBytes);
        hipLaunchKernelGGL(tsdfk::classify_brick_list, dim3((unsigned)((n_super + 3) / 4)), block, 0, ps, mi, bl);
        if (pipelined) {
            HIP_TRY_OR(unwind, hipEventRecord(v->pre_done[P], ps));
            HIP_TRY_OR(unwind, hipStreamWaitEvent(v->stream, v->pre_done[P], 0));
        }
        const dim3 grid_list((unsigned)(((cap + 3) / 4 + 1) * tsdfk::kListBuckets));
        const uint4 *wl = work_p;
        const unsigned char *wc = bl.counters;
        const tsdfk::ClassPoseTable *wp = bl.poses;
        if (label_ims)
            hipLaunchKernelGGL((tsdfk::integrate_brick_list<kBrickNT, true, false>), grid_list, block, 0, v->stream, mi, wl, wc, bl.bucket_cap, wp);
        else if (any_mask)
            hipLaunchKernelGGL((tsdfk::integrate_brick_list<kBrickNT, false, true>), grid_list, block, 0, v->stream, mi, wl, wc, bl.bucket_cap, wp);
        else
            hipLaunchKernelGGL((tsdfk::integrate_brick_list<kBrickNT, false, false>), grid_list, block, 0, v->stream, mi, wl, wc, bl.bucket_cap, wp);
        claims_total = (double)per_group * nz_groups * n;
        launched = true;
    }
    if (!launched) {
        dim3 grid_flat((v->chunks_per_slice + 3) / 4, 1, nz), grid_rows((mi.common.xgroups + 63) / 64, (c.dim_y + 3) / 4, nz);
        const dim3 &g0 = v->flat ? grid_flat : grid_rows;
        if (g0.x > 65535u) mi.z_fastest = 0;
        if (mi.z_fastest) {
            std::swap(grid_flat.x, grid_flat.z);
            std::swap(grid_rows.x, grid_rows.z);
        }
        if (label_ims && v->flat)
            hipLaunchKernelGGL((tsdfk::integrate_multi_inline<1, true, true, true, false>), grid_flat, block, 0, v->stream, mi);
        else if (label_ims)
            hipLaunchKernelGGL((tsdfk::integrate_multi_inline<1, true, false, true, false>), grid_rows, block, 0, v->stream, mi);
        else if (v->flat && any_mask)
            hipLaunchKernelGGL((tsdfk::integrate_multi_inline<1, true, true, false, true>), grid_flat, block, 0, v->stream, mi);
        else if (v->flat)
            hipLaunchKernelGGL((tsdfk::integrate_multi_inline<1, true, true, false, false>), grid_flat, block, 0, v->stream, mi);
        else if (any_mask)
            hipLaunchKernelGGL((tsdfk::integrate_multi_inline<1, true, false, false, true>), grid_rows, block, 0, v->stream, mi);
        else
            hipLaunchKernelGGL((tsdfk::integrate_multi_inline<1, true, false, false, false>), grid_rows, block, 0, v->stream, mi);
    }
    if (listed) {
        HIP_TRY_OR(unwind, hipEventRecord(v->list_free[P], v->stream));
        v->list_used[P] = true;
        v->list_parity = v->pipeline_ok ? P ^ 1 : 0;
    }
    if (count_claims) {
        v->claims_total = claims_total;
        const hipStream_t rs = (pipelined && listed) ? v->rb_stream : v->stream;
        if (rs != v->stream) HIP_TRY_OR(unwind, hipStreamWaitEvent(rs, v->list_free[P], 0));
        HIP_TRY_OR(unwind, hipMemcpyAsync(v->h_claims, claims_p, tsdfk::kCounterBytes, hipMemcpyDeviceToHost, rs));
        HIP_TRY_OR(unwind, hipEventRecord(v->claims_done, rs));
        v->claims_pending = true;
        v->rb_parity = (rs != v->stream) ? P : -1;
    }
    HIP_TRY_OR(unwind, hipGetLastError());
    const int rc_end = tables_end(v);
    if (pipelined) store_next_pass(v);
    return rc_end;
}

int frames_per_launch(const tsdf_volume *)
{
    return tsdfk::kMaxFramesPerLaunch;
}

bool can_fuse(const tsdf_volume *v) { return variant_of(v->variant).fuses && v->cfg.dim_x % 4 == 0; }

int integrate_frames(tsdf_volume *v, const float *const *depth_dev, const uint8_t *const *masks_dev,
                     const float *cam2world, int n_frames)
{
    const bool fuse = can_fuse(v);
    int rc = TSDF_OK;
    bool seq_event = false;
    for (int k = 0; k < n_frames && rc == TSDF_OK;) {
        const int n = fuse ? std::min(frames_per_launch(v), n_frames - k) : 1;
        float c2b[16 * tsdfk::kMaxFramesPerLaunch];
        for (int i = 0; i < n; ++i) compose_cam2base(v, cam2world + 16 * (k + i), c2b + 16 * i);
        if (fuse && !seq_event && v->seq_ready && v->pipeline_ok && n_frames > n) {
            HIP_TRY(hipEventRecord(v->seq_ready, v->stream));
            seq_event = true;
        }
        if (fuse) rc = launch_multi(v, depth_dev + k, masks_dev ? masks_dev + k : nullptr, c2b, n, nullptr, nullptr, seq_event ? v->seq_ready : nullptr);
        else rc = launch_integrate(v, depth_dev[k], masks_dev ? masks_dev[k] : nullptr, c2b);
        k += n;
    }
    return rc;
}

int flush_pending(tsdf_volume *v)
{
    if (v->pend_count == 0 || v->in_flush) return TSDF_OK;
    v->in_flush = true;
    const int n = v->pend_count;
    v->pend_count = 0;
    int rc = TSDF_OK;
    hipError_t e = hipSetDevice(v->cfg.device);
    if (e == hipSuccess) e = hipEventRecord(v->pend_copied, v->copy_stream);
    if (e == hipSuccess) e = hipStreamWaitEvent(v->stream, v->pend_copied, 0);
    if (e == hipSuccess) {
        bool any_mask = false;
        for (int f = 0; f < n; ++f) any_mask = any_mask || v->pend_mask[f] != nullptr;
        if (can_fuse(v) && n > 1) {
            rc = launch_multi(v, v->pend_depth, any_mask ? v->pend_mask : nullptr, v->pend_c2b, n);
        } else {
            for (int f = 0; f < n && rc == TSDF_OK; ++f) rc = launch_integrate(v, v->pend_depth[f], v->pend_mask[f], v->pend_c2b + 16 * f);
        }
        if (rc == TSDF_OK) rc = store_release(v, &v->store->frames, v->pend_slot, n);
        if (rc == TSDF_OK && any_mask) rc = store_release(v, &v->store->masks, v->pend_mask_slot, n);
        store_next_pass(v);
    }
    v->in_flush = false;
    if (e != hipSuccess) return fail(TSDF_ERR_HIP, "deferred integration: %s", hipGetErrorString(e));
    return rc;
}

struct Collected {
    int slot, mask_slot;
    float *dev;
    const uint8_t *mask;
};

int pool_slot_begin(tsdf_volume *v, hipStream_t first_user, Collected *c)
{
    c->slot = c->mask_slot = -1;
    c->mask = nullptr;
    void *dev = nullptr;
    int rc = store_slot(v, &v->store->frames, first_user, &c->slot, &dev);
    c->dev = static_cast<float *>(dev);
    return rc;
}

int pool_slot_commit(tsdf_volume *v, const Collected &c, const float cam2world[16], const float *cam2base = nullptr)
{
    const int slot = v->pend_count;
    v->pend_slot[slot] = c.slot;
    v->pend_mask_slot[slot] = c.mask_slot;
    v->pend_depth[slot] = c.dev;
    v->pend_mask[slot] = c.mask;
    if (cam2base) std::memcpy(v->pend_c2b + 16 * slot, cam2base, 16 * sizeof(float));
    else compose_cam2base(v, cam2world, v->pend_c2b + 16 * slot);
    std::memcpy(v->last_cam2base, v->pend_c2b + 16 * slot, sizeof v->last_cam2base);
    v->pend_count = slot + 1;
    if (v->pend_count >= std::min(v->defer_n, (int)tsdfk::kMaxFramesPerLaunch)) return flush_pending(v);
    return TSDF_OK;
}

int collect_device_frame(tsdf_volume *v, const float *depth_dev, const uint8_t *mask_dev, const float *cam2world,
                         const float *cam2base)
{
    const size_t px = (size_t)v->cfg.im_height * v->cfg.im_width;
    Collected c;
    int rc = pool_slot_begin(v, v->stream, &c);
    if (rc) return rc;
    HIP_TRY(hipMemcpyAsync(c.dev, depth_dev, px * sizeof(float), hipMemcpyDeviceToDevice, v->stream));
    if (mask_dev) {
        void *m = nullptr;
        rc = store_slot(v, &v->store->masks, v->stream, &c.mask_slot, &m);
        if (rc) return rc;
        HIP_TRY(hipMemcpyAsync(m, mask_dev, px, hipMemcpyDeviceToDevice, v->stream));
// ... 75 lines not shown
int tsdf_config_default(tsdf_config *cfg, int32_t im_height, int32_t im_width)
{
    if (!cfg) return fail(TSDF_ERR_INVALID, "tsdf_config_default: cfg is NULL");
    std::memset(cfg, 0, sizeof *cfg);
    cfg->im_height = im_height;
    cfg->im_width = im_width;
    cfg->dim_x = cfg->dim_y = cfg->dim_z = 200;
    cfg->z_begin = 0;
    cfg->z_end = 200;
    cfg->voxel_size = 0.004f;
    cfg->trunc_margin = cfg->voxel_size * 5;
    cfg->max_depth = 6.0f;
    const float K[9] = {535.4f, 0, 320.1f, 0, 539.2f, 247.6f, 0, 0, 1};
    std::memcpy(cfg->cam_K, K, sizeof K);
    for (int i = 0; i < 4; ++i) cfg->base2world[5 * i] = 1.0f;
    return TSDF_OK;
}

static int config_ok(const tsdf_config *cfg)
{
    if (cfg->dim_x <= 0 || cfg->dim_y <= 0 || cfg->dim_z <= 0)
        return fail(TSDF_ERR_INVALID, "tsdf_create: grid dims must be positive (%d,%d,%d)",
                    cfg->dim_x, cfg->dim_y, cfg->dim_z);
    if (cfg->z_begin < 0 || cfg->z_end < cfg->z_begin || cfg->z_end > cfg->dim_z)
        return fail(TSDF_ERR_INVALID, "tsdf_create: slab [%d,%d) outside grid z range [0,%d)",
                    cfg->z_begin, cfg->z_end, cfg->dim_z);
    if (cfg->im_height <= 0 || cfg->im_width <= 0 ||
        (int64_t)cfg->im_height * cfg->im_width > (int64_t)1 << 30)
        return fail(TSDF_ERR_INVALID, "tsdf_create: bad image size %dx%d", cfg->im_height, cfg->im_width);
    if (!(cfg->voxel_size > 0.0f) || !(cfg->trunc_margin > 0.0f))
        return fail(TSDF_ERR_INVALID, "tsdf_create: voxel_size and trunc_margin must be > 0");
    if (cfg->dim_y > 65535 * 4 || (cfg->z_end - cfg->z_begin) > 65535)
        return fail(TSDF_ERR_INVALID, "tsdf_create: slab exceeds launch limits (dim_y <= 262140, slices <= 65535)");
    if ((int64_t)cfg->dim_x * cfg->dim_y > ((int64_t)1 << 31) - 1024)
        return fail(TSDF_ERR_INVALID, "tsdf_create: a slice may hold at most 2^31 voxels (dim_x * dim_y)");
    return TSDF_OK;
}

static int create_volume(const tsdf_config *cfg, bool batch_member, tsdf_volume **out)
{
    *out = nullptr;
    int ok = config_ok(cfg);
    if (ok) return ok;

    int n_dev = 0;
    if (hipGetDeviceCount(&n_dev) != hipSuccess || n_dev <= 0)
        return fail(TSDF_ERR_NO_DEVICE, "tsdf_create: no HIP device visible (this library has no CPU path)");
    if (cfg->device < 0 || cfg->device >= n_dev)
        return fail(TSDF_ERR_INVALID, "tsdf_create: device %d not in [0,%d)", cfg->device, n_dev);

    tsdf_volume *v = new (std::nothrow) tsdf_volume();
    if (!v) return fail(TSDF_ERR_INVALID, "tsdf_create: out of host memory");
    v->cfg = *cfg;
    v->n_vox = (int64_t)cfg->dim_x * cfg->dim_y * (cfg->z_end - cfg->z_begin);
    tsdf_host::invert_matrix(cfg->base2world, v->base2world_inv);

    int rc = TSDF_OK;
    auto cleanup = [&](int code) { tsdf_destroy(v); return code; };
    if (hipSetDevice(cfg->device) != hipSuccess)
        return cleanup(fail(TSDF_ERR_HIP, "tsdf_create: hipSetDevice(%d) failed", cfg->device));
    hipError_t e;
    if ((e = stream_create(v->own_stream)) != hipSuccess)
        return cleanup(fail(TSDF_ERR_HIP, "tsdf_create: hipStreamCreate: %s", hipGetErrorString(e)));
    v->stream = v->own_stream;
    size_t bytes = (size_t)(v->n_vox > 0 ? v->n_vox : 1) * sizeof(float);
    if ((e = dev_alloc(v->d_tsdf, bytes)) != hipSuccess ||
        (e = dev_alloc(v->d_weight, bytes)) != hipSuccess)
        return cleanup(fail(TSDF_ERR_HIP, "tsdf_create: hipMalloc of %zu bytes x2: %s", bytes, hipGetErrorString(e)));
    v->flat = cfg->dim_x % 256 != 0;
    v->nseg = v->flat ? 0 : cfg->dim_x / 256;
    v->chunks_per_slice = (int)(((int64_t)cfg->dim_x * cfg->dim_y + 255) / 256);
    choose_brick(v);
    v->n_flags = cfg->dim_x % 4 == 0 ? (size_t)v->chunks_per_slice * (size_t)(cfg->z_end - cfg->z_begin) : 0;
    if ((e = dev_alloc(v->d_flags, (v->n_flags ? v->n_flags : 1) * sizeof(uint32_t))) != hipSuccess)
        return cleanup(fail(TSDF_ERR_HIP, "tsdf_create: hipMalloc of the summary: %s", hipGetErrorString(e)));
    v->tile = tsdf_host::tile_edge(*cfg, batch_member);
    v->fine_tables = tsdf_host::fine_tables(*cfg, v->tile);
    v->pipeline_ok = tsdf_host::pipelines(*cfg);
#ifdef TSDF_EXPERIMENTS
    if (const char *e = std::getenv("TSDF_FINE_TILES")) v->fine_tables = v->tile == 8 && std::atoi(e) != 0;
    if (const char *e = std::getenv("TSDF_PIPELINE")) v->pipeline_ok = std::atoi(e) != 0;
#endif
    const size_t table_bytes = tsdf_host::launch_table_bytes(*cfg, v->tile, v->fine_tables);
    if ((e = tsdf_store::store_ref(cfg->device, (size_t)cfg->im_height * cfg->im_width, table_bytes, &v->store)) != hipSuccess ||
        (e = event_create(v->flush_done[0])) != hipSuccess ||
        (e = event_create(v->flush_done[1])) != hipSuccess ||
        (e = event_create(v->pend_copied)) != hipSuccess)
        return cleanup(fail(TSDF_ERR_HIP, "tsdf_create: frame store: %s", hipGetErrorString(e)));
    v->copy_stream = v->store->copy_stream;
    if ((rc = fill(v)) != TSDF_OK) return cleanup(rc);
    *out = v;
    return TSDF_OK;
}

int tsdf_create(const tsdf_config *cfg, tsdf_volume **out)
{
    if (!cfg || !out) return fail(TSDF_ERR_INVALID, "tsdf_create: NULL argument");
    return create_volume(cfg, false, out);
}

int tsdf_destroy(tsdf_volume *v)
{
    if (!v) return TSDF_OK;
    (void)hipSetDevice(v->cfg.device);
    if (v->own_stream) (void)hipStreamSynchronize(v->own_stream);
    if (v->stream && v->stream != v->own_stream) (void)hipStreamSynchronize(v->stream);
    if (v->copy_stream) (void)hipStreamSynchronize(v->copy_stream);
    if (v->pre_stream) (void)hipStreamSynchronize(v->pre_stream);
    if (v->rb_stream) (void)hipStreamSynchronize(v->rb_stream);
    v->pend_count = 0;
    if (v->store) {
        tsdf_store::slots_drop_owner(v->store, v);
        tsdf_store::store_unref(v->store);
        v->store = nullptr;
    }
    delete v;
    return TSDF_OK;
}

int tsdf_reset(tsdf_volume *v)
{
    if (!v) return fail(TSDF_ERR_INVALID, "tsdf_reset: NULL handle");
    int rc = bind_device(v);
    if (rc) return rc;
    return fill(v);
}

int tsdf_integrate(tsdf_volume *v, const float *depth_host, const float cam2world[16])
{
    if (!v || !depth_host || !cam2world) return fail(TSDF_ERR_INVALID, "tsdf_integrate: NULL argument");
    const bool defer = v->defer_n > 1;
    int rc = bind_device(v, !defer);
    if (rc) return rc;
    const size_t img = (size_t)v->cfg.im_height * v->cfg.im_width * sizeof(float);
    int slot = -1;
    void *dev = nullptr;
    rc = stage_begin(v, img, [&](float *pinned) { tsdf_host::copy_to_pinned(pinned, depth_host, img); }, &slot, &dev);
    if (rc) return rc;
    if (defer) {
        Collected c;
        c.slot = slot; c.mask_slot = -1; c.dev = static_cast<float *>(dev); c.mask = nullptr;
        return pool_slot_commit(v, c, cam2world);
    }
    rc = stream_waits_for_copies(v);
    if (rc) return rc;
    float c2b[16];
    compose_cam2base(v, cam2world, c2b);
    rc = launch_integrate(v, static_cast<const float *>(dev), nullptr, c2b);
    if (rc) return rc;
    return stage_end(v, &slot, 1);
}

int tsdf_set_deferral(tsdf_volume *v, int32_t n_frames)
{
    if (!v) return fail(TSDF_ERR_INVALID, "tsdf_set_deferral: NULL handle");
    if (n_frames < 0 || n_frames > tsdfk::kMaxFramesPerLaunch)
        return fail(TSDF_ERR_INVALID, "tsdf_set_deferral: n_frames must be in [0, %d]", tsdfk::kMaxFramesPerLaunch);
    int rc = bind_device(v);
    if (rc) return rc;
    v->defer_n = n_frames;
    return TSDF_OK;
}

int tsdf_convert_depth_u16(tsdf_volume *v, const uint16_t *raw_dev, float *depth_dev, float depth_factor,
                           int32_t row_step, int32_t col_step)
{
// ... 33 lines not shown
            tsdf_store::slots_release_after(v->store, &v->store->frames, held, n, &v->pend_copied, v);
        }
        return failed;
    };
    rc = store_slot(v, &v->store->frames, v->copy_stream, &slot, &dev);
    if (rc) { slot = -1; return give_back(rc); }
    hipLaunchKernelGGL(tsdfk::depth_u16_to_f32, dim3((unsigned)((px + 255) / 256)), dim3(256), 0, v->copy_stream,
                       static_cast<const uint16_t *>(raw_dev), static_cast<float *>(dev), v->cfg.im_height, v->cfg.im_width,
                       1.0f / depth_factor, row_step, col_step);
    {
        const hipError_t le = hipGetLastError();
        if (le != hipSuccess) return give_back(fail(TSDF_ERR_HIP, "depth_u16_to_f32: %s", hipGetErrorString(le)));
    }
    {
        const hipError_t ee = hipEventRecord(v->pend_copied, v->copy_stream);
        if (ee != hipSuccess) return give_back(fail(TSDF_ERR_HIP, "hipEventRecord: %s", hipGetErrorString(ee)));
    }
    tsdf_store::slots_release_after(v->store, &v->store->frames, &raw_slot, 1, &v->pend_copied, v);
    raw_slot = -1;
    if (defer) {
        Collected c;
        c.slot = slot; c.mask_slot = -1; c.dev = static_cast<float *>(dev); c.mask = nullptr;
        return pool_slot_commit(v, c, cam2world);
    }
    {
        const hipError_t we = hipStreamWaitEvent(v->stream, v->pend_copied, 0);
        if (we != hipSuccess) return give_back(fail(TSDF_ERR_HIP, "hipStreamWaitEvent: %s", hipGetErrorString(we)));
    }
    float c2b[16];
    compose_cam2base(v, cam2world, c2b);
    rc = launch_integrate(v, static_cast<const float *>(dev), nullptr, c2b);
    const int rc_end = stage_end(v, &slot, 1);
    return rc ? rc : rc_end;
}

int tsdf_integrate_device(tsdf_volume *v, const float *depth_dev, const float cam2world[16])
{
    if (!v || !depth_dev || !cam2world) return fail(TSDF_ERR_INVALID, "tsdf_integrate_device: NULL argument");
    const bool defer = v->defer_n > 1 && can_fuse(v);
    int rc = bind_device(v, !defer);
    if (rc) return rc;
    if (defer) return collect_device_frame(v, depth_dev, nullptr, cam2world, nullptr);
    float c2b[16];
    compose_cam2base(v, cam2world, c2b);
    return launch_integrate(v, depth_dev, nullptr, c2b);
}

int tsdf_integrate_cam2base(tsdf_volume *v, const float *depth_dev, const float cam2base[16])
{
    if (!v || !depth_dev || !cam2base) return fail(TSDF_ERR_INVALID, "tsdf_integrate_cam2base: NULL argument");
    const bool defer = v->defer_n > 1 && can_fuse(v);
    int rc = bind_device(v, !defer);
    if (rc) return rc;
    if (defer) return collect_device_frame(v, depth_dev, nullptr, nullptr, cam2base);
    return launch_integrate(v, depth_dev, nullptr, cam2base);
}

int tsdf_integrate_frames_device(tsdf_volume *v, const float *const *depth_dev, const uint8_t *const *masks_dev,
                                 const float *cam2world, int32_t n_frames)
{
    if (!v || !depth_dev || !cam2world || n_frames < 0)
        return fail(TSDF_ERR_INVALID, "tsdf_integrate_frames_device: bad argument");
    for (int k = 0; k < n_frames; ++k)
        if (!depth_dev[k]) return fail(TSDF_ERR_INVALID, "tsdf_integrate_frames_device: depth_dev[%d] is NULL", k);
    int rc = bind_device(v);
    if (rc) return rc;
    return integrate_frames(v, depth_dev, masks_dev, cam2world, n_frames);
}

int tsdf_integrate_frames_labels_device(tsdf_volume *v, const float *const *depth_dev, const uint16_t *const *label_im_dev,
                                        const float *const *score_im_dev, const float *cam2world, int32_t n_frames)
{
    if (!v || !depth_dev || !label_im_dev || !score_im_dev || !cam2world || n_frames < 0)
        return fail(TSDF_ERR_INVALID, "tsdf_integrate_frames_labels_device: bad argument");
    if (!v->d_label) return fail(TSDF_ERR_INVALID, "tsdf_integrate_frames_labels_device: call tsdf_labels_enable first");
    for (int k = 0; k < n_frames; ++k)
        if (!depth_dev[k] || !label_im_dev[k] || !score_im_dev[k])
            return fail(TSDF_ERR_INVALID, "tsdf_integrate_frames_labels_device: frame %d has a NULL image", k);
    int rc = bind_device(v);
    if (rc) return rc;
    bool seq_event = false;
    for (int k = 0; k < n_frames && rc == TSDF_OK;) {
        const int n = std::min(frames_per_launch(v), n_frames - k);
        float c2b[16 * tsdfk::kMaxFramesPerLaunch];
        for (int i = 0; i < n; ++i) compose_cam2base(v, cam2world + 16 * (k + i), c2b + 16 * i);
        if (!seq_event && v->seq_ready && v->pipeline_ok && n_frames > n) {
            HIP_TRY(hipEventRecord(v->seq_ready, v->stream));
            seq_event = true;
        }
        rc = launch_multi(v, depth_dev + k, nullptr, c2b, n, label_im_dev + k, score_im_dev + k, seq_event ? v->seq_ready : nullptr);
        k += n;
    }
    return rc;
}

int tsdf_integrate_masked_device(tsdf_volume *v, const float *depth_dev, const uint8_t *mask_dev,
                                 const float cam2world[16])
{
    if (!v || !depth_dev || !mask_dev || !cam2world)
        return fail(TSDF_ERR_INVALID, "tsdf_integrate_masked_device: NULL argument");
    const bool defer = v->defer_n > 1 && can_fuse(v);
    int rc = bind_device(v, !defer);
    if (rc) return rc;
    if (defer) return collect_device_frame(v, depth_dev, mask_dev, cam2world, nullptr);
    float c2b[16];
    compose_cam2base(v, cam2world, c2b);
    return launch_integrate(v, depth_dev, mask_dev, c2b);
}

int tsdf_sync(tsdf_volume *v)
{
    if (!v) return fail(TSDF_ERR_INVALID, "tsdf_sync: NULL handle");
    int rc = bind_device(v);
    if (rc) return rc;
    HIP_TRY(hipStreamSynchronize(v->stream));
    return TSDF_OK;
}

int tsdf_download(tsdf_volume *v, float *tsdf_host, float *weight_host)
{
    if (!v) return fail(TSDF_ERR_INVALID, "tsdf_download: NULL handle");
    int rc = bind_device(v);
    if (rc) return rc;
    size_t bytes = (size_t)v->n_vox * sizeof(float);
    HIP_TRY(hipStreamSynchronize(v->stream));
    if (bytes == 0) return TSDF_OK;
    if (tsdf_host) HIP_TRY(hipMemcpy(tsdf_host, v->d_tsdf, bytes, hipMemcpyDeviceToHost));
    if (weight_host) HIP_TRY(hipMemcpy(weight_host, v->d_weight, bytes, hipMemcpyDeviceToHost));
    return TSDF_OK;
}

int tsdf_copy_slices(tsdf_volume *v, int32_t z_local, int32_t n_slices, void *tsdf_dst, void *weight_dst)
{
    if (!v) return fail(TSDF_ERR_INVALID, "tsdf_copy_slices: NULL handle");
    const int nz = v->cfg.z_end - v->cfg.z_begin;
    if (z_local < 0 || n_slices < 0 || z_local + n_slices > nz)
        return fail(TSDF_ERR_INVALID, "tsdf_copy_slices: slices [%d,%d) outside the slab's %d", z_local, z_local + n_slices, nz);
    int rc = bind_device(v);
    if (rc) return rc;
    const size_t slice = (size_t)v->cfg.dim_x * v->cfg.dim_y;
    const size_t bytes = slice * (size_t)n_slices * sizeof(float);
    if (bytes == 0) return TSDF_OK;
    if (tsdf_dst) HIP_TRY(hipMemcpyAsync(tsdf_dst, v->d_tsdf + slice * z_local, bytes, hipMemcpyDefault, v->stream));
    if (weight_dst) HIP_TRY(hipMemcpyAsync(weight_dst, v->d_weight + slice * z_local, bytes, hipMemcpyDefault, v->stream));
    HIP_TRY(hipStreamSynchronize(v->stream));
    return TSDF_OK;
}

int tsdf_upload(tsdf_volume *v, const float *tsdf_host, const float *weight_host)
{
    if (!v) return fail(TSDF_ERR_INVALID, "tsdf_upload: NULL handle");
    int rc = bind_device(v);
    if (rc) return rc;
    size_t bytes = (size_t)v->n_vox * sizeof(float);
    HIP_TRY(hipStreamSynchronize(v->stream));
    if (bytes == 0) return TSDF_OK;
    if (tsdf_host) HIP_TRY(hipMemcpy(v->d_tsdf, tsdf_host, bytes, hipMemcpyHostToDevice));
    if (weight_host) HIP_TRY(hipMemcpy(v->d_weight, weight_host, bytes, hipMemcpyHostToDevice));
    return rebuild_summary(v);
}

int tsdf_refresh_summary(tsdf_volume *v)
{
    if (!v) return fail(TSDF_ERR_INVALID, "tsdf_refresh_summary: NULL handle");
    int rc = bind_device(v);
    if (rc) return rc;
    return rebuild_summary(v);
// ... 509 lines not shown
```

### semantic_slam_amd/csrc/tsdf_diag.hip.h

```cpp
#pragma once

namespace {

template <typename Queue>
int time_on_stream(tsdf_volume *v, const char *who, float *elapsed_ms, Queue &&queue)
{
    Event e0, e1;
    HIP_TRY(event_create(e0, hipEventDefault));
    HIP_TRY(event_create(e1, hipEventDefault));
    HIP_TRY(hipEventRecord(e0, v->stream));
    const int rc = queue();
    hipError_t er = hipEventRecord(e1, v->stream);
    hipError_t es = hipEventSynchronize(e1);
    float ms = 0.f;
    hipError_t et = hipEventElapsedTime(&ms, e0, e1);
    if (rc) return rc;
    if (er != hipSuccess || es != hipSuccess || et != hipSuccess)
        return fail(TSDF_ERR_HIP, "%s: event timing failed", who);
    *elapsed_ms = ms;
    return TSDF_OK;
}

int frames_timed(tsdf_volume *v, const float *const *depth_dev, const uint8_t *const *masks_dev,
                 const float *cam2world, int32_t n_frames, float *elapsed_ms, const char *who)
// ... 250 lines not shown
int32_t tsdf_frames_per_launch(const tsdf_volume *v)
{
    if (!v) return 0;
    return can_fuse(v) ? frames_per_launch(v) : 1;
}

int tsdf_shortcut_stats(tsdf_volume *v, int32_t enable, uint64_t counts_out[3])
{
    if (!v) return fail(TSDF_ERR_INVALID, "tsdf_shortcut_stats: NULL handle");
    int rc = bind_device(v);
    if (rc) return rc;
    HIP_TRY(hipStreamSynchronize(v->stream));
    if (counts_out) {
        unsigned int h[3] = {0, 0, 0};
        if (v->d_shortcut_stats) HIP_TRY(hipMemcpy(h, v->d_shortcut_stats, sizeof h, hipMemcpyDeviceToHost));
        for (int i = 0; i < 3; ++i) counts_out[i] = h[i];
    }
    if (enable && !v->d_shortcut_stats) HIP_TRY(dev_alloc(v->d_shortcut_stats, 8 * sizeof(unsigned int)));
    if (v->d_shortcut_stats) {
        if (enable) HIP_TRY(hipMemset(v->d_shortcut_stats, 0, 8 * sizeof(unsigned int)));
        else v->d_shortcut_stats.reset();
    }
    return TSDF_OK;
}

int tsdf_brick_list_stats(tsdf_volume *v, uint64_t counts_out[4])
{
    if (!v || !counts_out) return fail(TSDF_ERR_INVALID, "tsdf_brick_list_stats: NULL argument");
    int rc = bind_device(v);
    if (rc) return rc;
    HIP_TRY(hipStreamSynchronize(v->stream));
    unsigned int h[8] = {0, 0, 0, 0, 0, 0, 0, 0};
    if (v->d_shortcut_stats) HIP_TRY(hipMemcpy(h, v->d_shortcut_stats, sizeof h, hipMemcpyDeviceToHost));
    for (int i = 0; i < 4; ++i) counts_out[i] = h[3 + i];
    return TSDF_OK;
}

int tsdf_classification_info(tsdf_volume *v, double info_out[2])
{
    if (!v || !info_out) return fail(TSDF_ERR_INVALID, "tsdf_classification_info: NULL argument");
    int rc = bind_device(v);
    if (rc) return rc;
    HIP_TRY(hipStreamSynchronize(v->stream));
    if (v->rb_stream) HIP_TRY(hipStreamSynchronize(v->rb_stream));
    if (v->claims_pending && hipEventQuery(v->claims_done) == hipSuccess) {
        v->claim_fraction = claims_read_back(v);
        v->claims_pending = false;
        v->claims_known = true;
    }
    info_out[0] = v->claims_known ? v->claim_fraction : -1.0;
    info_out[1] = (double)v->launches_unclassified;
    return TSDF_OK;
}

int tsdf_last_cam2base(const tsdf_volume *v, float out[16])
{
    if (!v || !out) return fail(TSDF_ERR_INVALID, "tsdf_last_cam2base: NULL argument");
    std::memcpy(out, v->last_cam2base, sizeof v->last_cam2base);
    return TSDF_OK;
}


int tsdf_set_kernel_variant(tsdf_volume *v, int32_t variant)
{
    if (!v) return fail(TSDF_ERR_INVALID, "tsdf_set_kernel_variant: NULL handle");
    if (!variant_of(variant).known)
        return fail(TSDF_ERR_INVALID, "tsdf_set_kernel_variant: unknown variant %d (this build knows 0, 1, 3, 7, 8%s)", variant,
                    kExperiments ? " and the experiments" : "; the others live in the -DTSDF_EXPERIMENTS build");
    v->variant = variant;
    return TSDF_OK;
}

int tsdf_set_brick_shape(tsdf_volume *v, int32_t quads, int32_t rows, int32_t slices)
{
    if (!v) return fail(TSDF_ERR_INVALID, "tsdf_set_brick_shape: NULL handle");
    if (quads == 0 && rows == 0 && slices == 0) { choose_brick(v); return TSDF_OK; }
    if (!brick_shape_ok(v->cfg, quads, rows, slices))
        return fail(TSDF_ERR_INVALID, "tsdf_set_brick_shape: %d quads x %d rows x %d slices: needs quads * rows * slices <= 64 and "
                    "quads dividing dim_x / 4 = %d", quads, rows, slices, v->cfg.dim_x / 4);
    v->brick_q = quads; v->brick_r = rows; v->brick_s = slices;
    return TSDF_OK;
}

int tsdf_brick_shape(const tsdf_volume *v, int32_t shape_out[3])
{
    if (!v || !shape_out) return fail(TSDF_ERR_INVALID, "tsdf_brick_shape: NULL argument");
    shape_out[0] = v->brick_q; shape_out[1] = v->brick_q ? v->brick_r : 0; shape_out[2] = v->brick_q ? v->brick_s : 0;
    return TSDF_OK;
}

int tsdf_default_brick_shape(const tsdf_config *cfg, int32_t shape_out[3])
{
    if (!cfg || !shape_out) return fail(TSDF_ERR_INVALID, "tsdf_default_brick_shape: NULL argument");
    if (cfg->dim_x <= 0 || cfg->dim_y <= 0 || cfg->z_end < cfg->z_begin)
        return fail(TSDF_ERR_INVALID, "tsdf_default_brick_shape: bad grid");
    int q, r, s;
    choose_brick_for(*cfg, q, r, s);
    shape_out[0] = q; shape_out[1] = q ? r : 0; shape_out[2] = q ? s : 0;
    return TSDF_OK;
}

}
```

### semantic_slam_amd/csrc/tsdf_multiframe.hip.h

```cpp
#pragma once
#include "tsdf_kernels.hip.h"

namespace tsdfk {

constexpr int kMaxFramesPerLaunch = 32;
constexpr int kFineTile = 4;
constexpr int kFineLevels = 3;
__host__ __device__ inline size_t fine_table_elems(int fw, int fh) { return (size_t)kFineLevels * kFineLevels * fw * fh; }

struct FramePose {
    const float *depth;
    const uint8_t *mask;
    float rx0, ry0, rx1, ry1, rx2, ry2, rz0, rz1, rz2, tz, tx, ty;
    int fast_ok;
    float cz_margin;
    const uint16_t *label_im;
    const float *score_im;
    const float2 *tiles;
    float cz_short;
    float cz_pad;
};

constexpr int kListBuckets = 64;
constexpr int kBucketStride = 256;
constexpr int kCounterBytes = kListBuckets * kBucketStride;

struct TileSummaryParams {
    const float *depth[kMaxFramesPerLaunch];
    const uint8_t *mask[kMaxFramesPerLaunch];
    float2 *tiles;
    int H, W, tiles_w, tiles_h;
    float max_depth;
    float2 *fine = nullptr;
    int fw = 0, fh = 0;
};

__device__ __forceinline__ int tile_levels(int n) { return 32 - __clz(n); }
__device__ __forceinline__ size_t tile_table_elems(int tw, int th) { return (size_t)tile_levels(tw) * tile_levels(th) * tw * th; }

template <int kTile>
__global__ __launch_bounds__(256) void depth_tile_summary_per_tile(TileSummaryParams tp)
{
    static_assert(kTile == 8 || kTile == 16, "one wavefront per tile: 64 lanes x 1 or 4 pixels");
    const int tile = blockIdx.x * 4 + threadIdx.y, f = blockIdx.y;
    if (tile >= tp.tiles_w * tp.tiles_h) return;
    const int ty = tile / tp.tiles_w, tx = tile - ty * tp.tiles_w;
    const int lane = threadIdx.x;
    constexpr int kPxPerLane = kTile * kTile / 64, kLanesPerRow = kTile / kPxPerLane;
    const int py = ty * kTile + lane / kLanesPerRow, px0 = tx * kTile + (lane % kLanesPerRow) * kPxPerLane;
    const float *d = tp.depth[f];
    const uint8_t *m = tp.mask[f];
    const float inf = __builtin_inff();
    float mn = inf, mx = -inf;
    bool all_valid = true, nan = false;
    if (py < tp.H) {
#pragma unroll
        for (int i = 0; i < kPxPerLane; ++i) {
            const int px = px0 + i;
            if (px < tp.W) {
                float v = d[(size_t)py * tp.W + px];
                if (m != nullptr) v = v * (m[(size_t)py * tp.W + px] >= 128 ? 1.0f : 0.0f);
                nan |= v != v;
                const bool valid = (v > 0.0f) & (v <= tp.max_depth);
                all_valid &= valid;
                if (valid) { mn = fminf(mn, v); mx = fmaxf(mx, v); }
            }
        }
    }
#pragma unroll
    for (int off = 32; off > 0; off >>= 1) {
        mn = fminf(mn, __shfl_xor(mn, off));
        mx = fmaxf(mx, __shfl_xor(mx, off));
    }
    const bool any_nan = __ballot(nan) != 0ull, every_valid = __ballot(!all_valid) == 0ull;
    if (lane == 0) {
        float2 out;
        out.x = (every_valid && !any_nan) ? mn : -inf;
        out.y = any_nan ? inf : mx;
        tp.tiles[(size_t)f * tile_table_elems(tp.tiles_w, tp.tiles_h) + (size_t)ty * tp.tiles_w + tx] = out;
    }
}

template <int kTile>
__global__ __launch_bounds__(256) void depth_tile_summary(TileSummaryParams tp)
{
    static_assert(kTile == 8 || kTile == 16, "64-pixel strips of 16- or 8-pixel tiles");
    constexpr int kTilesPerStrip = 64 / kTile;
    constexpr int kLanesPerTileRow = kTile / 4;
// ... 232 lines not shown
    const bool vec = (tp.W & 3) == 0 && (reinterpret_cast<uintptr_t>(d) & 15) == 0 && (m == nullptr || (reinterpret_cast<uintptr_t>(m) & 3) == 0);
#pragma unroll
    for (int r = 0; r < kFineTile; ++r) {
        const int py = ty * kFineTile + r;
        if (py >= tp.H) continue;
        const size_t at = (size_t)py * tp.W + px0;
        float v[4];
        bool in[4];
        if (vec) {
            const float4 q = *reinterpret_cast<const float4 *>(d + at);
            v[0] = q.x; v[1] = q.y; v[2] = q.z; v[3] = q.w;
            in[0] = in[1] = in[2] = in[3] = true;
            if (m != nullptr) {
                const uchar4 k = *reinterpret_cast<const uchar4 *>(m + at);
                v[0] = v[0] * (k.x >= 128 ? 1.0f : 0.0f); v[1] = v[1] * (k.y >= 128 ? 1.0f : 0.0f);
                v[2] = v[2] * (k.z >= 128 ? 1.0f : 0.0f); v[3] = v[3] * (k.w >= 128 ? 1.0f : 0.0f);
            }
        } else {
#pragma unroll
            for (int j = 0; j < 4; ++j) {
                in[j] = px0 + j < tp.W;
                v[j] = in[j] ? d[at + j] : 0.0f;
                if (in[j] && m != nullptr) v[j] = v[j] * (m[at + j] >= 128 ? 1.0f : 0.0f);
            }
        }
#pragma unroll
        for (int j = 0; j < 4; ++j) {
            if (!in[j]) continue;
            nan |= v[j] != v[j];
            const bool valid = (v[j] > 0.0f) & (v[j] <= tp.max_depth);
            all_valid &= valid;
            if (valid) { mn = fminf(mn, v[j]); mx = fmaxf(mx, v[j]); }
        }
    }
    float2 out;
    out.x = (all_valid && !nan) ? mn : -inf;
    out.y = nan ? inf : mx;
    tp.fine[(size_t)f * fine_table_elems(tp.fw, tp.fh) + (size_t)ty * tp.fw + tx] = out;
}

__global__ __launch_bounds__(256) void fine_tile_levels(float2 *fine, int fw, int fh)
{
    const int k = blockIdx.x * 256 + threadIdx.x;
    if (k >= fw * fh) return;
    fine_levels_at(fine + (size_t)blockIdx.y * fine_table_elems(fw, fh), fw, fh, k);
}

__global__ __launch_bounds__(256) void fine_table_reference(FineTileParams tp)
{
    const int n = tp.fw * tp.fh;
    const int id = blockIdx.x * 256 + threadIdx.x, f = blockIdx.y;
    if (id >= kFineLevels * kFineLevels * n) return;
    const int level = id / n, k = id - level * n, ky = level / kFineLevels, kx = level - ky * kFineLevels;
    const int ty = k / tp.fw, tx = k - ty * tp.fw;
    const int x0 = tx * kFineTile, x1 = min((tx + (1 << kx)) * kFineTile, tp.W), y0 = ty * kFineTile, y1 = min((ty + (1 << ky)) * kFineTile, tp.H);
    const float inf = __builtin_inff();
    float mn = inf, mx = -inf;
    bool all_valid = true, nan = false;
    for (int y = y0; y < y1; ++y)
        for (int x = x0; x < x1; ++x) {
            float v = tp.depth[f][(size_t)y * tp.W + x];
            if (tp.mask[f] != nullptr) v = v * (tp.mask[f][(size_t)y * tp.W + x] >= 128 ? 1.0f : 0.0f);
            nan |= v != v;
            const bool valid = (v > 0.0f) & (v <= tp.max_depth);
            all_valid &= valid;
            if (valid) { mn = fminf(mn, v); mx = fmaxf(mx, v); }
        }
    float2 out;
    out.x = (all_valid && !nan) ? mn : -inf;
    out.y = nan ? inf : mx;
    tp.fine[(size_t)f * fine_table_elems(tp.fw, tp.fh) + (size_t)level * n + k] = out;
}

struct ClassPose {
    float rx0, ry0, rz0, tx;
    float rx1, ry1, rz1, ty;
    float rx2, ry2, rz2, tz;
    const float2 *tiles;
    float cz_short, cz_pad;
};
static_assert(sizeof(ClassPose) == 64, "four 16-byte words");

struct ClassPoseTable {
    float4 w[4][kMaxFramesPerLaunch];
};

__device__ __forceinline__ ClassPose class_pose(const FramePose &q)
{
    ClassPose c;
    c.rx0 = q.rx0; c.ry0 = q.ry0; c.rz0 = q.rz0; c.tx = q.tx;
    c.rx1 = q.rx1; c.ry1 = q.ry1; c.rz1 = q.rz1; c.ty = q.ty;
    c.rx2 = q.rx2; c.ry2 = q.ry2; c.rz2 = q.rz2; c.tz = q.tz;
    c.tiles = q.tiles; c.cz_short = q.cz_short; c.cz_pad = q.cz_pad;
    return c;
}

__device__ __forceinline__ ClassPose class_pose(const ClassPoseTable *__restrict__ t, const int f)
{
    union { ClassPose c; float4 w[4]; } u;
#pragma unroll
    for (int k = 0; k < 4; ++k) u.w[k] = t->w[k][f];
    return u.c;
}

__device__ __forceinline__ void class_pose_store(ClassPoseTable *t, const int f, const ClassPose &c)
{
    union { ClassPose c; float4 w[4]; } u;
    u.c = c;
#pragma unroll
    for (int k = 0; k < 4; ++k) t->w[k][f] = u.w[k];
}

template <bool PAIRED = false>
__device__ __forceinline__ int classify_patch(const IntegrateParams &p, const ClassPose &q, const int xa,
                                              const int xb, const int ya, const int yb, const int gz, const int gz1 = -1,
                                              const float2 *__restrict__ fine = nullptr)
{
    if constexpr (!PAIRED) { if (q.tiles == nullptr) return 0; }
    const float dxa = (p.ox + (float)xa * p.vs) - q.tx, dxb = (p.ox + (float)xb * p.vs) - q.tx;
    const float dya = (p.oy + (float)ya * p.vs) - q.ty, dyb = (p.oy + (float)yb * p.vs) - q.ty;
    const float inf = __builtin_inff();
    float umin = inf, umax = -inf, vmin = inf, vmax = -inf, czmin = inf, czmax = -inf;
    bool finite = true;
    auto slice_corners = [&](const int z) {
        const float dz = (p.oz + (float)z * p.vs) - q.tz;
        const float zx = q.rx2 * dz, zy = q.ry2 * dz, zz = q.rz2 * dz;
        auto corner = [&](const float dx, const float dy) {
            const float cx = q.rx0 * dx + q.rx1 * dy + zx;
            const float cy = q.ry0 * dx + q.ry1 * dy + zy;
            const float cz = q.rz0 * dx + q.rz1 * dy + zz;
            const float inv = __builtin_amdgcn_rcpf(cz);
            const float u = p.fx * (cx * inv) + p.cx, v = p.fy * (cy * inv) + p.cy;
            umin = fminf(umin, u); umax = fmaxf(umax, u);
            vmin = fminf(vmin, v); vmax = fmaxf(vmax, v);
            czmin = fminf(czmin, cz); czmax = fmaxf(czmax, cz);
            finite &= (u == u) & (v == v) & (cz == cz);
        };
        corner(dxa, dya); corner(dxb, dya);
        corner(dxa, dyb); corner(dxb, dyb);
    };
    if constexpr (PAIRED) {
        slice_corners((threadIdx.x & 32u) ? max(gz1, gz) : gz);
        umin = fminf(umin, __shfl_xor(umin, 32)); umax = fmaxf(umax, __shfl_xor(umax, 32));
        vmin = fminf(vmin, __shfl_xor(vmin, 32)); vmax = fmaxf(vmax, __shfl_xor(vmax, 32));
        czmin = fminf(czmin, __shfl_xor(czmin, 32)); czmax = fmaxf(czmax, __shfl_xor(czmax, 32));
        finite = finite & (__shfl_xor((int)finite, 32) != 0);
        if (q.tiles == nullptr) return 0;
    } else {
        slice_corners(gz);
        if (gz1 > gz) slice_corners(gz1);
    }
    if (!(finite & (czmin > q.cz_short) & (czmax < 3.0e38f))) return 0;
    const float u0 = umin - p.px_margin_u, u1 = umax + p.px_margin_u;
    const float v0 = vmin - p.px_margin_v, v1 = vmax + p.px_margin_v;
    const float wmax = (float)(p.W - 1), hmax = (float)(p.H - 1);
    if (!(u1 >= 0.0f) | !(v1 >= 0.0f) | !(u0 <= wmax) | !(v0 <= hmax)) return 2;
    const bool inside = (u0 >= 0.0f) & (v0 >= 0.0f) & (u1 <= wmax) & (v1 <= hmax);
    const float uc0 = fmaxf(u0, 0.0f), uc1 = fminf(u1, wmax), vc0 = fmaxf(v0, 0.0f), vc1 = fminf(v1, hmax);
    int tx0 = (int)(uc0 * p.tile_inv), tx1 = (int)(uc1 * p.tile_inv);
    int ty0 = (int)(vc0 * p.tile_inv), ty1 = (int)(vc1 * p.tile_inv);
    int kx = 31 - __clz(tx1 - tx0 + 1), ky = 31 - __clz(ty1 - ty0 + 1);
    int tw = p.tiles_w;
    const float2 *L = q.tiles + (size_t)(ky * tile_levels(p.tiles_w) + kx) * (p.tiles_w * p.tiles_h);
    if (fine != nullptr) {
        const float finv = 1.0f / (float)kFineTile;
        const int fx0 = (int)(uc0 * finv), fx1 = (int)(uc1 * finv), fy0 = (int)(vc0 * finv), fy1 = (int)(vc1 * finv);
        const int fkx = 31 - __clz(fx1 - fx0 + 1), fky = 31 - __clz(fy1 - fy0 + 1);
        if (fkx < kFineLevels && fky < kFineLevels) {
            tx0 = fx0; tx1 = fx1; ty0 = fy0; ty1 = fy1; kx = fkx; ky = fky; tw = p.fine_w;
            L = fine + (size_t)(fky * kFineLevels + fkx) * (p.fine_w * p.fine_h);
        }
    }
    const int xb2 = tx1 - (1 << kx) + 1, yb2 = ty1 - (1 << ky) + 1;
    const float2 a = L[ty0 * tw + tx0], b = L[ty0 * tw + xb2];
    const float2 c = L[yb2 * tw + tx0], d = L[yb2 * tw + xb2];
    const float dmin = fminf(fminf(a.x, b.x), fminf(c.x, d.x));
    const float dmax = fmaxf(fmaxf(a.y, b.y), fmaxf(c.y, d.y));
    const float thr_free = (czmax + q.cz_pad) + p.trunc;
    const float thr_skip = (czmin - q.cz_pad) - p.trunc;
    if (inside & (dmin >= thr_free)) return 1;
    if (dmax <= thr_skip) return 2;
    return 0;
}

__global__ __launch_bounds__(256) void classify_bricks(IntegrateParams p, FramePose pose, uint8_t *cls, int blocks, int nzg)
{
    const int id = blockIdx.x * 256 + threadIdx.x;
    if (id >= blocks * nzg * 4) return;
    const int wave = id & 3, wg = (id >> 2) % blocks, lz = (id >> 2) / blocks;
    const int brick = wg * 4 + wave;
    const int g = brick / p.bricks_per_group, i = brick - g * p.bricks_per_group;
    int c = 2;
    if (g < p.brick_groups) {
        const int xa = i * p.brick_q * 4, ya = g * p.brick_r;
        const int z0 = lz * p.brick_s, z1 = min(z0 + p.brick_s - 1, p.nz - 1);
        c = classify_patch(p, class_pose(pose), xa, xa + p.brick_q * 4 - 1, ya, min(ya + p.brick_r - 1, p.dim_y - 1), p.z_begin + z0,
                           p.z_begin + z1);
    }
    cls[id] = (uint8_t)c;
}

__global__ __launch_bounds__(256) void classify_bricks_batched(const IntegrateParams *__restrict__ params,
                                                               const FramePose *__restrict__ poses,
                                                               const int2 *__restrict__ group_map, uint8_t *cls,
                                                               int max_blocks, int total_groups)
{
    const int id = blockIdx.x * 256 + threadIdx.x;
    if (id >= max_blocks * total_groups * 4) return;
    const int wave = id & 3, wg = (id >> 2) % max_blocks, z = (id >> 2) / max_blocks;
    const int2 m = group_map[z];
    const IntegrateParams p = params[m.x];
    const int brick = wg * 4 + wave;
    const int g = brick / p.bricks_per_group, i = brick - g * p.bricks_per_group;
    int c = 2;
    if (g < p.brick_groups) {
        const int xa = i * p.brick_q * 4, ya = g * p.brick_r;
        const int z0 = m.y * p.brick_s, z1 = min(z0 + p.brick_s - 1, p.nz - 1);
        c = classify_patch(p, class_pose(poses[m.x]), xa, xa + p.brick_q * 4 - 1, ya, min(ya + p.brick_r - 1, p.dim_y - 1), p.z_begin + z0,
                           p.z_begin + z1);
    }
    cls[id] = (uint8_t)c;
}

struct LabelState {
    uint16_t *label;
    float *fp, *bp;
    float prob_thd;
};

struct MultiParamsInline {
    IntegrateParams common;
    FramePose frames[kMaxFramesPerLaunch];
    int n_frames;
    LabelState labels;
    int z_fastest;
#ifdef TSDF_EXPERIMENTS
    const unsigned int *super_mask;
    int nz_super;
#endif
};

constexpr int kSuperZ = 4;

template <int R, bool NT, bool FLAT, bool LABELS = false, bool MASKS = true, bool SHORT = false, bool BRICK = false, bool EAGER_W = false>
__device__ __forceinline__ void multi_body(const IntegrateParams &p, const FramePose *__restrict__ frames,
                                           const int n_frames, const int b0, const int b1, const int lz,
                                           const LabelState ls = LabelState(), const unsigned int free_frames = 0u,
                                           const unsigned int skip_frames = 0u)
{
    static_assert(!SHORT || R == 1, "patch classification is written for one row per lane");
    static_assert(!LABELS || R == 1, "label fusion rides on the one-row kernel");
    static_assert(!FLAT || R == 1, "the flat mapping handles one quad per lane");
    static_assert(!BRICK || (R == 1 && !FLAT), "bricks are their own mapping");
    static_assert(!EAGER_W || BRICK, "eager weights are for the bricks of a work list");
    int xg, gy0;
    size_t row0, flag0;
    size_t brick_base = 0;
    unsigned int lane_byte = 0u;
    uint32_t flag32 = 0u;
    constexpr bool kBuf = BRICK && !NT;
    __amdgpu_buffer_rsrc_t t_buf, w_buf;
    auto load_quad = [&](const bool tsdf, const int r) -> float4 {
        if constexpr (kBuf) {
            const v4u v = __builtin_amdgcn_raw_buffer_load_b128(tsdf ? t_buf : w_buf, (int)lane_byte, 0, 0);
            return make_float4(__uint_as_float(v.x), __uint_as_float(v.y), __uint_as_float(v.z), __uint_as_float(v.w));
        } else {
            return vol_load<NT>((tsdf ? p.tsdf : p.weight) + row0 + (size_t)r * p.dim_x);
        }
    };
    auto store_quad = [&](const bool tsdf, const int r, const float4 q) {
        if constexpr (kBuf) {
            const v4u v = {__float_as_uint(q.x), __float_as_uint(q.y), __float_as_uint(q.z), __float_as_uint(q.w)};
            __builtin_amdgcn_raw_buffer_store_b128(v, tsdf ? t_buf : w_buf, (int)lane_byte, 0, 0);
        } else {
            vol_store<NT>((tsdf ? p.tsdf : p.weight) + row0 + (size_t)r * p.dim_x, q);
        }
    };
    int lzz = lz;
    auto brick_flag_index = [&](const int gy, const int quad) -> size_t {
        if (p.nseg > 0) return ((size_t)lzz * p.dim_y + gy) * (size_t)p.nseg + (size_t)(quad >> 6);
        return (size_t)lzz * p.chunks_per_slice + (size_t)((gy * p.quads_per_row + quad) >> 6);
    };
    if constexpr (BRICK) {
        const int brick = b0;
        const int g = brick / p.bricks_per_group, i = brick - g * p.bricks_per_group;
        const int per = p.brick_q * p.brick_r;
        const int zz = (int)(((unsigned)threadIdx.x * (unsigned)p.brick_per_magic) >> 16), rem = (int)threadIdx.x - zz * per;
        const int rr = (int)(((unsigned)rem * (unsigned)p.brick_q_magic) >> 16), qq = rem - rr * p.brick_q;
        xg = i * p.brick_q + qq;
        gy0 = g * p.brick_r + rr;
        lzz = lz * p.brick_s + zz;
        if (g >= p.brick_groups || zz >= p.brick_s || lzz >= p.nz || gy0 >= p.dim_y) return;
        brick_base = ((size_t)(lz * p.brick_s) * p.dim_y + (size_t)(g * p.brick_r)) * (size_t)p.dim_x + (size_t)(i * p.brick_q) * 4;
        lane_byte = (((unsigned)zz * (unsigned)p.dim_y + (unsigned)rr) * (unsigned)p.dim_x + (unsigned)qq * 4u) * 4u;
        row0 = brick_base + (size_t)(lane_byte >> 2);
        if constexpr (kBuf) {
            t_buf = __builtin_amdgcn_make_buffer_rsrc(p.tsdf + brick_base, 0, -1, 0x00020000);
            w_buf = __builtin_amdgcn_make_buffer_rsrc(p.weight + brick_base, 0, -1, 0x00020000);
        }
        flag0 = brick_flag_index(gy0, xg);
        flag32 = (uint32_t)flag0;
    } else if constexpr (FLAT) {
        const int chunk = b0 * 4 + threadIdx.y;
        const int q = chunk * 64 + threadIdx.x;
        if (q >= p.quads_per_slice) return;
        gy0 = q / p.quads_per_row;
        xg = q - gy0 * p.quads_per_row;
        row0 = ((size_t)lz * p.quads_per_slice + q) * 4;
        flag0 = (size_t)lz * p.chunks_per_slice + chunk;
    } else {
        xg = b0 * 64 + threadIdx.x;
        gy0 = (b1 * 4 + threadIdx.y) * R;
        if (xg >= p.xgroups || gy0 >= p.dim_y) return;
        row0 = ((size_t)lz * p.dim_y + gy0) * (size_t)p.dim_x + (size_t)xg * 4;
        flag0 = ((size_t)lz * p.dim_y + gy0) * (size_t)p.nseg + b0;
    }
    const int gz = p.z_begin + lzz;

    uint32_t fl[R];
    bool ones[R];
    float4 t4[R], w4[R];
    bool touched[R], tchanged[R];
#pragma unroll
    for (int r = 0; r < R; ++r) {
        fl[r] = (R == 1 || gy0 + r < p.dim_y) ? p.flags[flag0 + (size_t)r * p.nseg] : 0u;
        ones[r] = (fl[r] & 1u) != 0u;
        t4[r] = make_float4(1.f, 1.f, 1.f, 1.f);
        w4[r] = make_float4(0.f, 0.f, 0.f, 0.f);
        touched[r] = tchanged[r] = false;
    }
    bool have_w = false;
// ... 15 lines not shown
    float diff[R][4];
    bool upd[R][4], rowany[R], bandr[R];
    bool any = false, band = false;
    auto apply_frame = [&]() __attribute__((always_inline)) {
#pragma unroll
        for (int r = 0; r < R; ++r) {
            if (rowany[r] && !touched[r]) {
                if (!have_w) w4[r] = load_quad(false, r);
                if (!(fl[r] & 1u)) t4[r] = load_quad(true, r);
                touched[r] = true;
            }
        }
        float dist[R][4];
        if (__ballot(band) != 0ull) {
            if (fast_frame && p.trunc_fast != 0) {
#pragma unroll
                for (int r = 0; r < R; ++r)
#pragma unroll
                    for (int j = 0; j < 4; ++j) dist[r][j] = fminf(1.0f, fast_div_r(diff[r][j], p.trunc, trunc_r1));
            } else {
#pragma unroll
                for (int r = 0; r < R; ++r)
#pragma unroll
                    for (int j = 0; j < 4; ++j) dist[r][j] = fminf(1.0f, diff[r][j] / p.trunc);
            }
        } else {
#pragma unroll
            for (int r = 0; r < R; ++r)
#pragma unroll
                for (int j = 0; j < 4; ++j) dist[r][j] = 1.0f;
        }

#pragma unroll
        for (int r = 0; r < R; ++r) {
            if (__ballot(!(ones[r] && (fl[r] & 2u)) || bandr[r]) == 0ull) {
                if (upd[r][0]) w4[r].x += 1.0f;
                if (upd[r][1]) w4[r].y += 1.0f;
                if (upd[r][2]) w4[r].z += 1.0f;
                if (upd[r][3]) w4[r].w += 1.0f;
                continue;
            }
            float tv[4] = {t4[r].x, t4[r].y, t4[r].z, t4[r].w};
            float wv[4] = {w4[r].x, w4[r].y, w4[r].z, w4[r].w};
            float num[4], wn[4];
            const bool wave_band = __ballot(bandr[r]) != 0ull;
            bool need = false;
#pragma unroll
            for (int j = 0; j < 4; ++j) {
                wn[j] = wv[j] + 1.0f;
                num[j] = tv[j] * wv[j] + dist[r][j];
            }
            if (!wave_band) {
#pragma unroll
                for (int j = 0; j < 4; ++j) need |= upd[r][j] && !(num[j] == wn[j] && wn[j] < 3.0e38f && wn[j] > 0.0f);
            }
            float nt[4];
            if (wave_band || __ballot(rowany[r] && need) != 0ull) {
#pragma unroll
                for (int j = 0; j < 4; ++j) nt[j] = num[j] / wn[j];
            } else {
#pragma unroll
                for (int j = 0; j < 4; ++j) nt[j] = 1.0f;
            }
            bool changed = wave_band, notone = false;
#pragma unroll
            for (int j = 0; j < 4; ++j) {
                const float newt = upd[r][j] ? nt[j] : tv[j];
                if (!wave_band) changed |= __float_as_uint(newt) != __float_as_uint(tv[j]);
                notone |= upd[r][j] && __float_as_uint(newt) != 0x3f800000u;
                tv[j] = newt;
                wv[j] = upd[r][j] ? wn[j] : wv[j];
            }
            t4[r] = make_float4(tv[0], tv[1], tv[2], tv[3]);
            w4[r] = make_float4(wv[0], wv[1], wv[2], wv[3]);
            tchanged[r] |= changed;
            {
                const unsigned long long nb = __ballot(notone);
                if constexpr (BRICK) { if (notone) ones[r] = false; }
                else { if (nb != 0ull) ones[r] = false; }
            }
        }
    };

    unsigned int todo = n_frames >= 32 ? 0xffffffffu : ((1u << n_frames) - 1u);
    if constexpr (SHORT) {
        if (p.shortcut_stats != nullptr && (threadIdx.x & 63) == 0 && (skip_frames & todo) != 0u)
            atomicAdd(p.shortcut_stats + 2, (unsigned)__popc(skip_frames & todo));
        todo &= ~skip_frames;
    }
#pragma unroll 1
    for (int f = 0; f < n_frames; ++f) {
        if constexpr (SHORT) {
            if (todo == 0u) break;
            f = __ffs((int)todo) - 1;
            todo &= todo - 1u;
            const bool all_free = (free_frames >> f) & 1u;
            if (all_free) {
                if (__ballot(!((touched[0] || have_w) && ones[0] && (fl[0] & 2u))) == 0ull) {
                    touched[0] = true;
                    const unsigned int rest = ~(free_frames >> f);
                    unsigned int run = rest != 0u ? (unsigned)(__ffs((int)rest) - 1) : 32u - (unsigned)f;
                    run = min(run, (unsigned)(n_frames - f));
                    const float4 w = w4[0];
                    const bool whole = w.x == truncf(w.x) && w.y == truncf(w.y) && w.z == truncf(w.z) && w.w == truncf(w.w) &&
                                       fmaxf(fmaxf(w.x, w.y), fmaxf(w.z, w.w)) < 16777184.0f;
                    if (run > 1u && __ballot(!whole) == 0ull) {
                        const float k = (float)run;
                        w4[0].x += k; w4[0].y += k; w4[0].z += k; w4[0].w += k;
                        todo &= ~((run >= 32u ? 0xffffffffu : ((1u << run) - 1u)) << f);
                        if (p.shortcut_stats != nullptr && (threadIdx.x & 63) == 0) atomicAdd(p.shortcut_stats + 1, run);
                        continue;
                    }
                    if (p.shortcut_stats != nullptr && (threadIdx.x & 63) == 0) atomicAdd(p.shortcut_stats + 1, 1u);
                    w4[0].x += 1.0f; w4[0].y += 1.0f; w4[0].z += 1.0f; w4[0].w += 1.0f;
                    continue;
                }
                if (p.shortcut_stats != nullptr && (threadIdx.x & 63) == 0) atomicAdd(p.shortcut_stats + 1, 1u);
#pragma unroll
                for (int r = 0; r < R; ++r) {
                    rowany[r] = true;
                    bandr[r] = false;
#pragma unroll
                    for (int j = 0; j < 4; ++j) { upd[r][j] = true; diff[r][j] = p.trunc; }
                }
                band = false;
                apply_frame();
                continue;
            }
        }
        if constexpr (SHORT) {
            if (p.shortcut_stats != nullptr && (threadIdx.x & 63) == 0) atomicAdd(p.shortcut_stats, 1u);
        }
        any = false;
        band = false;
        {
        const FramePose q = frames[f];

        float ax[4], ay[4], az[4];
#pragma unroll
        for (int j = 0; j < 4; ++j) {
            const float dx = bxv[j] - q.tx;
            ax[j] = q.rx0 * dx; ay[j] = q.ry0 * dx; az[j] = q.rz0 * dx;
        }
        const float dz = bz - q.tz;
        const float x2 = q.rx2 * dz, y2 = q.ry2 * dz, z2 = q.rz2 * dz;
        float pcz[R][4], dval[R][4];
        int mval[MASKS ? R : 1][4];
        uint32_t pixel[LABELS ? R : 1][4];
        auto fetch = [&](const int r, const int j, const bool ok, const uint32_t px) {
            if constexpr (LABELS) pixel[r][j] = px;
            float d = 0.0f;
            int m = 255;
            if (ok) {
                d = gather_f32(q.depth, px);
                if constexpr (MASKS) if (q.mask != nullptr) m = q.mask[px];
            }
            dval[r][j] = d;
            if constexpr (MASKS) mval[r][j] = m;
        };
#pragma unroll
        for (int r = 0; r < R; ++r) {
            const float z1 = q.rz1 * (byv[r] - q.ty);
#pragma unroll
            for (int j = 0; j < 4; ++j) pcz[r][j] = az[j] + z1 + z2;
        }
        bool all_front = (pcz[0][0] > q.cz_margin) & (pcz[0][3] > q.cz_margin);
        bool all_behind = (pcz[0][0] < -q.cz_margin) & (pcz[0][3] < -q.cz_margin);
        if constexpr (R > 1) {
            all_front &= (pcz[R - 1][0] > q.cz_margin) & (pcz[R - 1][3] > q.cz_margin);
            all_behind &= (pcz[R - 1][0] < -q.cz_margin) & (pcz[R - 1][3] < -q.cz_margin);
        }
        const bool unsafe = !(all_front | all_behind);
        fast_frame = q.fast_ok != 0 && __ballot(unsafe) == 0ull;
        if (fast_frame) {
            const bool front = all_front;
#pragma unroll
            for (int r = 0; r < R; ++r) {
                const bool row_ok = R == 1 || gy0 + r < p.dim_y;
                const float dy = byv[r] - q.ty;
                const v2f XY1 = {q.rx1 * dy, q.ry1 * dy};
                const v2f XY2 = {x2, y2};
#pragma unroll
                for (int j = 0; j < 4; ++j) {
                    const v2f A = {ax[j], ay[j]};
                    const v2f n = A + XY1 + XY2;
                    const float cz = pcz[r][j];
                    const v2f uv = F * fast_div2(n, cz) + C;
                    const int iu = round_half_up_i32(uv.x), iv = round_half_up_i32(uv.y);
                    const bool ok = row_ok & front & (uv.x > -0.5f) & (uv.y > -0.5f) &
                                    ((unsigned)iu < (unsigned)p.W) & ((unsigned)iv < (unsigned)p.H);
                    fetch(r, j, ok, (uint32_t)pixel_index24(iv, p.W, iu));
                }
// ... 33 lines not shown
            bandr[r] = false;
#pragma unroll
            for (int j = 0; j < 4; ++j) {
                const float d = dval[r][j];
                const float df = d - pcz[r][j];
                diff[r][j] = df;
                const bool u = !((d <= 0.0f) | (d > p.max_depth)) & !(df <= -p.trunc);
                upd[r][j] = u;
                rowany[r] |= u;
                bandr[r] |= u & !(df >= p.trunc);
            }
            band |= bandr[r];
            any |= rowany[r];
        }
        if (__ballot(any) == 0ull) continue;

        if constexpr (LABELS) {
            if (q.label_im != nullptr && __ballot(band) != 0ull) {
                uint16_t lab_in[4];
                float sc_in[4];
                bool hit = false;
#pragma unroll
                for (int j = 0; j < 4; ++j) {
                    const bool seen = upd[0][j] & (diff[0][j] < p.trunc);
                    lab_in[j] = 0;
                    sc_in[j] = 0.0f;
                    if (seen) { lab_in[j] = q.label_im[pixel[0][j]]; sc_in[j] = q.score_im[pixel[0][j]]; }
                    hit |= lab_in[j] != 0;
                }
                if (hit) {
                    ushort4 L4 = *reinterpret_cast<const ushort4 *>(ls.label + row0);
                    float4 F4 = *reinterpret_cast<const float4 *>(ls.fp + row0);
                    float4 B4 = *reinterpret_cast<const float4 *>(ls.bp + row0);
                    uint16_t L[4] = {L4.x, L4.y, L4.z, L4.w};
                    float Fv[4] = {F4.x, F4.y, F4.z, F4.w}, Bv[4] = {B4.x, B4.y, B4.z, B4.w};
#pragma unroll
                    for (int j = 0; j < 4; ++j) {
                        const uint16_t l = lab_in[j];
                        const float sc = sc_in[j];
                        if (l == 0) continue;
                        if (L[j] == 0) { L[j] = l; Fv[j] = sc; Bv[j] = 0.0f; }
                        else if (L[j] == l) { Fv[j] = Fv[j] + sc; }
                        else {
                            Bv[j] = Bv[j] + sc;
                            if (Fv[j] / (Fv[j] + Bv[j]) < ls.prob_thd) { L[j] = l; Fv[j] = sc; Bv[j] = 0.0f; }
                        }
                    }
                    ushort4 Lo; Lo.x = L[0]; Lo.y = L[1]; Lo.z = L[2]; Lo.w = L[3];
                    *reinterpret_cast<ushort4 *>(ls.label + row0) = Lo;
                    *reinterpret_cast<float4 *>(ls.fp + row0) = make_float4(Fv[0], Fv[1], Fv[2], Fv[3]);
                    *reinterpret_cast<float4 *>(ls.bp + row0) = make_float4(Bv[0], Bv[1], Bv[2], Bv[3]);
                }
            }
        }

        }

        apply_frame();
    }

#pragma unroll
    for (int r = 0; r < R; ++r) {
        const bool store_t = __ballot(touched[r] && tchanged[r]) != 0ull;
        if (touched[r]) {
            if (store_t) store_quad(true, r, t4[r]);
            store_quad(false, r, w4[r]);
        }
        if ((fl[r] & 1u) && !ones[r]) {
            if constexpr (BRICK) {
                p.flags[flag32] = fl[r] & 2u;
            } else {
                p.flags[flag0 + (size_t)r * p.nseg] = fl[r] & 2u;
            }
        }
    }
}

#ifndef TSDF_BRICK_WAVES
#define TSDF_BRICK_WAVES 8
#endif
template <int R, bool NT, bool FLAT, bool LABELS = false, bool MASKS = true>
__global__ __launch_bounds__(256, R == 2 ? 6 : 1) void integrate_multi_inline(MultiParamsInline mp)
{
    typedef const char __attribute__((address_space(4))) *kernarg_ptr;
    kernarg_ptr base = (kernarg_ptr)__builtin_amdgcn_kernarg_segment_ptr();
    typedef const FramePose __attribute__((address_space(4))) *frames_ptr;
    frames_ptr frames = (frames_ptr)(base + offsetof(MultiParamsInline, frames));
    const int wg_x = mp.z_fastest ? (int)blockIdx.z : (int)blockIdx.x, wg_y = (int)blockIdx.y;
    int wg_z = mp.z_fastest ? (int)blockIdx.x : (int)blockIdx.z;
    if (mp.z_fastest == 2) {
        wg_z += (int)((unsigned)(wg_x + wg_y) % gridDim.x);
        if (wg_z >= (int)gridDim.x) wg_z -= (int)gridDim.x;
    }
    multi_body<R, NT, FLAT, LABELS, MASKS>(mp.common, (const FramePose *)frames, mp.n_frames, wg_x, wg_y, wg_z, mp.labels);
}

constexpr int kSuperBX = 4, kSuperBY = 2, kSuperBZ = 1;
constexpr int kSuperBricks = kSuperBX * kSuperBY * kSuperBZ;
static_assert(kSuperBricks <= 32, "one lane of a half-wave per brick of the super-brick");
constexpr unsigned int kBrickUndecided = 0x80000000u;

struct BrickListParams {
    uint4 *list;
    unsigned char *counters;
    unsigned int bucket_cap;
    ClassPoseTable *poses;
    int nsx, nsy, nsz;
    int wedge_mode, wedge_oy, wedge_oz, super_h, super_d, fy_px;
};

__host__ __device__ inline unsigned int list_bucket(const unsigned int id, const int sx, const int sy, const int sz, const BrickListParams &bl)
{
    const unsigned int h = id * 2654435761u;
    if (bl.wedge_mode == 0) return h >> 26;
    const int yc = bl.wedge_oy + (2 * sy + 1) * bl.super_h / 2;
    int zc = bl.wedge_oz + (2 * sz + 1) * bl.super_d / 2;
    if (zc < 1) zc = 1;
    int t = (yc * 256) / zc;
    t = t > 65536 ? 65536 : (t < -65536 ? -65536 : t);
    const int stripe = (t * bl.fy_px) >> (bl.wedge_mode == 3 ? 11 : 12);
    const int rot = bl.wedge_mode >= 2 ? 3 * (sx >> 2) : 0;
    return ((h >> 29) << 3) | ((unsigned int)(stripe + rot) & 7u);
}

__global__ __launch_bounds__(256) void classify_brick_list(MultiParamsInline mp, BrickListParams bl)
{
    typedef const char __attribute__((address_space(4))) *kernarg_ptr;
    kernarg_ptr base = (kernarg_ptr)__builtin_amdgcn_kernarg_segment_ptr();
    const FramePose *frames = (const FramePose *)(base + offsetof(MultiParamsInline, frames));
    const IntegrateParams &p = mp.common;
    const int id = (int)blockIdx.x * 4 + __builtin_amdgcn_readfirstlane((int)threadIdx.y), lane = threadIdx.x;
    if (id >= bl.nsx * bl.nsy * bl.nsz) return;
    const int sz = id % bl.nsz, t = id / bl.nsz, sx = t % bl.nsx, sy = t / bl.nsx;
    const int nzg = (p.nz + p.brick_s - 1) / p.brick_s;
    const int i0 = sx * kSuperBX, g0 = sy * kSuperBY, zg0 = sz * kSuperBZ;
    const int i1 = min(i0 + kSuperBX, p.bricks_per_group) - 1, g1 = min(g0 + kSuperBY, p.brick_groups) - 1, zg1 = min(zg0 + kSuperBZ, nzg) - 1;
    const unsigned int frames_mask = mp.n_frames >= 32 ? 0xffffffffu : ((1u << mp.n_frames) - 1u);
    static_assert(kMaxFramesPerLaunch == 32, "one frame per lane of a half-wave");
    const int xa = i0 * p.brick_q * 4, xb = (i1 + 1) * p.brick_q * 4 - 1;
    const int ya = g0 * p.brick_r, yb = min((g1 + 1) * p.brick_r, p.dim_y) - 1;
    const int z0 = zg0 * p.brick_s, z1 = min((zg1 + 1) * p.brick_s, p.nz) - 1;
    const ClassPose mine_q = class_pose(frames[lane & 31]);
    if (id == 0 && lane < kMaxFramesPerLaunch) class_pose_store(bl.poses, lane, mine_q);
    const float2 *fine_f = p.fine != nullptr ? p.fine + (size_t)(lane & 31) * fine_table_elems(p.fine_w, p.fine_h) : nullptr;
    const int cls = classify_patch<true>(p, mine_q, xa, xb, ya, yb, p.z_begin + z0, p.z_begin + z1, fine_f);
    const unsigned int super_free = (unsigned int)__ballot(cls == 1) & frames_mask;
    const unsigned int super_skip = (unsigned int)__ballot(cls == 2) & frames_mask;
    const int n_in = (i1 - i0 + 1) * (g1 - g0 + 1) * (zg1 - zg0 + 1);
    static_assert(kListBuckets == 64, "six bits: list_bucket");
    const unsigned int bkt = list_bucket((unsigned int)id, sx, sy, sz, bl);
    unsigned char *bucket = bl.counters + (size_t)bkt * kBucketStride;
    if (lane == 0) {
        if (p.claim_counter != nullptr && (super_free | super_skip) != 0u)
            atomicAdd(reinterpret_cast<unsigned long long *>(bucket + 8),
                      ((unsigned long long)(n_in * __popc(super_free)) << 32) | (unsigned long long)(n_in * __popc(super_skip)));
        if (p.shortcut_stats != nullptr) {
            if (super_skip == frames_mask) { atomicAdd(p.shortcut_stats + 2, (unsigned)(n_in * mp.n_frames)); atomicAdd(p.shortcut_stats + 3, 1u); }
            else {
                atomicAdd(p.shortcut_stats + 4, (unsigned)n_in);
                if ((super_free | super_skip) != frames_mask) atomicAdd(p.shortcut_stats + 5, (unsigned)n_in);
            }
        }
    }
    if (super_skip == frames_mask) return;
    const int k = lane;
    const int i = i0 + k % kSuperBX, g = g0 + (k / kSuperBX) % kSuperBY, zg = zg0 + k / (kSuperBX * kSuperBY);
    const bool mine = k < kSuperBricks && i <= i1 && g <= g1 && zg <= zg1;
    const unsigned long long live_mask = __ballot(mine);
    const unsigned int undecided = (super_free | super_skip) != frames_mask ? kBrickUndecided : 0u;
    const unsigned int n_live = (unsigned)__popcll(live_mask);
    unsigned int at = 0u;
    if (lane == 0) at = atomicAdd(reinterpret_cast<unsigned int *>(bucket) + (undecided ? 0 : 1), n_live);
    at = __builtin_amdgcn_readfirstlane(at);
    at = bkt * bl.bucket_cap + (undecided ? at : bl.bucket_cap - at - n_live);
    if (mine)
        bl.list[at + (unsigned)__popcll(live_mask & ((1ull << lane) - 1ull))] =
            make_uint4((unsigned)(g * p.bricks_per_group + i) | undecided, (unsigned)zg, super_free, super_skip);
}

template <bool NT, bool LABELS, bool MASKS>
__global__ __launch_bounds__(256, LABELS ? 6 : TSDF_BRICK_WAVES) void integrate_brick_list(MultiParamsInline mp, const uint4 *__restrict__ list,
                                                                                          const unsigned char *__restrict__ counters,
                                                                                          const unsigned int bucket_cap,
                                                                                          const ClassPoseTable *__restrict__ poses)
{
    typedef const char __attribute__((address_space(4))) *kernarg_ptr;
    kernarg_ptr base = (kernarg_ptr)__builtin_amdgcn_kernarg_segment_ptr();
    const FramePose *frames = (const FramePose *)(base + offsetof(MultiParamsInline, frames));
    const unsigned int b = blockIdx.x % kListBuckets, grp = blockIdx.x / kListBuckets;
    const unsigned int wave = (unsigned)__builtin_amdgcn_readfirstlane((int)threadIdx.y);
    const uint2 n = *reinterpret_cast<const uint2 *>(counters + (size_t)b * kBucketStride);
    const unsigned int front_groups = (n.x + 3u) / 4u;
    unsigned int at;
    if (grp < front_groups) {
        at = grp * 4u + wave;
        if (at >= n.x) return;
    } else {
        const unsigned int k = (grp - front_groups) * 4u + wave;
        if (k >= n.y) return;
        at = bucket_cap - 1u - k;
    }
    const uint4 e = list[(size_t)b * bucket_cap + at];
    const int brick = (int)(e.x & ~kBrickUndecided), zg = (int)e.y;
    unsigned int free_frames = e.z, skip_frames = e.w;
    if (e.x & kBrickUndecided) {
        const IntegrateParams &p = mp.common;
        const int lane = threadIdx.x;
        const unsigned int frames_mask = mp.n_frames >= 32 ? 0xffffffffu : ((1u << mp.n_frames) - 1u);
        const int g = brick / p.bricks_per_group, i = brick - g * p.bricks_per_group;
        const int xa = i * p.brick_q * 4, ya = g * p.brick_r;
        const int z0 = zg * p.brick_s, z1 = min(z0 + p.brick_s - 1, p.nz - 1);
        const float2 *fine_f = p.fine != nullptr ? p.fine + (size_t)(lane & 31) * fine_table_elems(p.fine_w, p.fine_h) : nullptr;
        const int cls = classify_patch<true>(p, class_pose(poses, lane & 31), xa, xa + p.brick_q * 4 - 1, ya, min(ya + p.brick_r - 1, p.dim_y - 1),
                                             p.z_begin + z0, p.z_begin + z1, fine_f);
        free_frames |= (unsigned int)__ballot(cls == 1) & frames_mask;
        skip_frames |= (unsigned int)__ballot(cls == 2) & frames_mask;
        free_frames = __builtin_amdgcn_readfirstlane(free_frames);
        skip_frames = __builtin_amdgcn_readfirstlane(skip_frames);
        if (skip_frames == frames_mask) {
            if (p.shortcut_stats != nullptr && lane == 0) { atomicAdd(p.shortcut_stats + 2, (unsigned)mp.n_frames); atomicAdd(p.shortcut_stats + 6, 1u); }
            return;
        }
    }
    multi_body<1, NT, false, LABELS, MASKS, true, true, true>(mp.common, frames, mp.n_frames, brick, 0, zg, mp.labels, free_frames, skip_frames);
}

template <bool NT, bool FLAT>
__global__ __launch_bounds__(256) void integrate_multi_single(IntegrateParams p, FramePose pose)
{
    multi_body<1, NT, FLAT>(p, &pose, 1, blockIdx.x, blockIdx.y, blockIdx.z);
}

template <bool NT>
__global__ __launch_bounds__(256) void integrate_multi_batched(const IntegrateParams *__restrict__ params,
                                                               const FramePose *__restrict__ poses,
                                                               const int2 *__restrict__ slice_map)
{
    const int2 m = slice_map[blockIdx.z];
    const IntegrateParams p = params[m.x];
    multi_body<1, NT, true>(p, poses + m.x, 1, blockIdx.x, 0, m.y);
}

template <bool NT>
__global__ __launch_bounds__(256, 8) void integrate_single_bricks(IntegrateParams p, FramePose pose)
{
    const unsigned c = p.wg_class[(blockIdx.x + gridDim.x * blockIdx.z) * 4u + threadIdx.y];
    if (c == 2u) return;
    multi_body<1, NT, false, false, true, true, true>(p, &pose, 1, (int)blockIdx.x * 4 + __builtin_amdgcn_readfirstlane((int)threadIdx.y), 0,
                                                      blockIdx.z, LabelState(), c == 1u ? 1u : 0u, 0u);
}

template <bool NT>
__global__ __launch_bounds__(256, 8) void integrate_multi_batched_bricks(const IntegrateParams *__restrict__ params,
                                                                        const FramePose *__restrict__ poses,
                                                                        const int2 *__restrict__ group_map,
                                                                        const uint8_t *__restrict__ wg_class)
{
    const unsigned c = wg_class[(blockIdx.x + gridDim.x * blockIdx.z) * 4u + threadIdx.y];
    if (c == 2u) return;
    const int2 m = group_map[blockIdx.z];
    const IntegrateParams p = params[m.x];
    multi_body<1, NT, false, false, true, true, true>(p, poses + m.x, 1, (int)blockIdx.x * 4 + __builtin_amdgcn_readfirstlane((int)threadIdx.y), 0,
                                                      m.y, LabelState(), c == 1u ? 1u : 0u, 0u);
}

constexpr int kGatherMasks = 32;
struct MaskGatherParams {
    const uint8_t *src[kGatherMasks];
    uint8_t *dst[kGatherMasks];
    size_t bytes;
};

__global__ __launch_bounds__(256) void gather_masks(MaskGatherParams gp)
{
    const uint8_t *src = gp.src[blockIdx.y];
    uint8_t *dst = gp.dst[blockIdx.y];
    if (src == nullptr) return;
    const size_t i = ((size_t)blockIdx.x * 256 + threadIdx.x) * 16;
    if (i + 16 <= gp.bytes && (((uintptr_t)src | (uintptr_t)dst) & 15) == 0) {
        *reinterpret_cast<uint4 *>(dst + i) = *reinterpret_cast<const uint4 *>(src + i);
    } else {
        for (size_t k = i; k < gp.bytes && k < i + 16; ++k) dst[k] = src[k];
    }
}

}
```

Measured before the change: 425,200.

## Fuse up to 64 frames per integration pass for large volumes

Raises the number of depth frames fused into one brick-list integration pass from 32 to 64 for volumes above a size threshold. Frame poses move from kernel arguments to a device-staged table, and free/skip masks widen to 64 bits with a companion high-bits list. Tile tables are built in two halves using two store slots. The intent is to halve the read-modify-write sweeps of the TSDF volume per frame, at the cost of extra staging launches, more table memory and 64-lane classification without the half-wave path.

```diff
diff --git a/include/tsdf_hip_diag.h b/include/tsdf_hip_diag.h
--- a/include/tsdf_hip_diag.h
+++ b/include/tsdf_hip_diag.h
@@ -45,6 +45,7 @@
 
 int tsdf_set_brick_shape(tsdf_volume *vol, int32_t quads, int32_t rows, int32_t slices);
 int tsdf_brick_shape(const tsdf_volume *vol, int32_t shape_out[3]);
+int tsdf_set_frames_per_pass(tsdf_volume *vol, int32_t n_frames);
 int tsdf_default_brick_shape(const tsdf_config *cfg, int32_t shape_out[3]);
 
 #ifdef __cplusplus
diff --git a/semantic_slam_amd/capi.py b/semantic_slam_amd/capi.py
--- a/semantic_slam_amd/capi.py
+++ b/semantic_slam_amd/capi.py
@@ -14,7 +14,7 @@
     "tsdf_sync", "tsdf_download", "tsdf_copy_slices", "tsdf_upload", "tsdf_refresh_summary", "tsdf_device_ptrs", "tsdf_slab_voxels", "tsdf_frames_per_launch", "tsdf_shortcut_stats", "tsdf_brick_list_stats", "tsdf_classification_info",
     "tsdf_get_config", "tsdf_last_cam2base", "tsdf_set_stream", "tsdf_get_stream",
     "tsdf_count_surface", "tsdf_extract_surface", "tsdf_extract_crossings", "tsdf_extract_mesh", "tsdf_save_mesh_ply", "tsdf_save_mesh_welded_ply", "tsdf_save_ply", "tsdf_save_bin", "tsdf_load_bin", "tsdf_save_state", "tsdf_load_state",
-    "tsdf_integrate_sequence_timed", "tsdf_integrate_frames_timed", "tsdf_probe_graph_replay", "tsdf_probe_stream", "tsdf_selftest_fastdiv", "tsdf_selftest_fastdiv_band", "tsdf_selftest_round", "tsdf_selftest_tile_tables", "tsdf_set_kernel_variant", "tsdf_set_brick_shape", "tsdf_brick_shape", "tsdf_default_brick_shape", "tsdf_last_error",
+    "tsdf_integrate_sequence_timed", "tsdf_integrate_frames_timed", "tsdf_probe_graph_replay", "tsdf_probe_stream", "tsdf_selftest_fastdiv", "tsdf_selftest_fastdiv_band", "tsdf_selftest_round", "tsdf_selftest_tile_tables", "tsdf_set_kernel_variant", "tsdf_set_brick_shape", "tsdf_set_frames_per_pass", "tsdf_brick_shape", "tsdf_default_brick_shape", "tsdf_last_error",
     "tsdf_version", "tsdf_multiply_matrix", "tsdf_invert_matrix",
     "tsdf_labels_enable", "tsdf_compose_labels", "tsdf_integrate_labels_device", "tsdf_integrate_frames_labels_device",
     "tsdf_download_labels",
@@ -40,7 +40,7 @@
     "tsdf_probe_graph_replay", "tsdf_probe_stream",
     "tsdf_selftest_fastdiv", "tsdf_selftest_fastdiv_band", "tsdf_selftest_round", "tsdf_selftest_tile_tables",
     "tsdf_shortcut_stats", "tsdf_brick_list_stats", "tsdf_classification_info", "tsdf_frames_per_launch", "tsdf_last_cam2base",
-    "tsdf_set_kernel_variant", "tsdf_set_brick_shape", "tsdf_brick_shape", "tsdf_default_brick_shape",
+    "tsdf_set_kernel_variant", "tsdf_set_brick_shape", "tsdf_set_frames_per_pass", "tsdf_brick_shape", "tsdf_default_brick_shape",
 ]
 
 
@@ -217,6 +217,7 @@
     L.tsdf_selftest_tile_tables.argtypes = [C.c_int32, vp, vp, C.c_int32, C.c_int32, C.c_float, C.POINTER(C.c_uint64)]
     L.tsdf_set_kernel_variant.argtypes = [vp, C.c_int32]
     L.tsdf_set_brick_shape.argtypes = [vp, C.c_int32, C.c_int32, C.c_int32]
+    L.tsdf_set_frames_per_pass.argtypes = [vp, C.c_int32]
     L.tsdf_brick_shape.argtypes = [vp, C.POINTER(C.c_int32)]
     L.tsdf_default_brick_shape.argtypes = [C.POINTER(TsdfConfig), C.POINTER(C.c_int32)]
     L.tsdf_last_error.restype = C.c_char_p
@@ -729,6 +730,9 @@
     def set_brick_shape(self, quads=0, rows=0, slices=0):
         check(self.lib.tsdf_set_brick_shape(self._h, quads, rows, slices), "tsdf_set_brick_shape")
 
+    def set_frames_per_pass(self, n_frames=0):
+        check(self.lib.tsdf_set_frames_per_pass(self._h, n_frames), "tsdf_set_frames_per_pass")
+
     def brick_shape(self):
         out = (C.c_int32 * 3)()
         check(self.lib.tsdf_brick_shape(self._h, out), "tsdf_brick_shape")
diff --git a/semantic_slam_amd/csrc/frame_store.h b/semantic_slam_amd/csrc/frame_store.h
--- a/semantic_slam_amd/csrc/frame_store.h
+++ b/semantic_slam_amd/csrc/frame_store.h
@@ -120,8 +120,10 @@
     return e;
 }
 
-inline hipError_t slot_acquire(FrameStore *s, SlotClass *c, const void *owner, hipStream_t first_user, bool force, int *index, void **dev)
+inline hipError_t slot_acquire(FrameStore *s, SlotClass *c, const void *owner, hipStream_t first_user, bool force, int *index, void **dev,
+                               int quota = 0)
 {
+    if (quota <= 0) quota = c->quota;
     std::lock_guard<std::mutex> lk(s->mu);
     *index = -1;
     int pick = -1, mine = -1, oldest = -1, own = 0;
@@ -135,7 +137,7 @@
     }
     const bool at_cap = (int)c->slots.size() >= c->soft_cap;
     int wait_for = -1;
-    if (pick < 0 && mine >= 0 && (own >= c->quota || at_cap)) wait_for = mine;
+    if (pick < 0 && mine >= 0 && (own >= quota || at_cap)) wait_for = mine;
     else if (pick < 0 && at_cap && oldest >= 0) wait_for = oldest;
     if (wait_for >= 0) {
         const hipError_t e = hipStreamWaitEvent(first_user, *c->slots[(size_t)wait_for].release, 0);
diff --git a/semantic_slam_amd/csrc/host_derive.h b/semantic_slam_amd/csrc/host_derive.h
--- a/semantic_slam_amd/csrc/host_derive.h
+++ b/semantic_slam_amd/csrc/host_derive.h
@@ -88,6 +88,7 @@
 }
 
 constexpr int kMaxFramesPerLaunch = 32;
+constexpr int kMaxFramesPerPass = 64;
 constexpr int kTileLdsEntries = 5120;
 constexpr int kFineTile = 4;
 constexpr int kFineLevels = 3;
@@ -143,6 +144,18 @@
     return tiles_fit(tw, th) ? kMaxFramesPerLaunch * (tile_table_elems(tw, th) + fine_elems) * (2 * sizeof(float)) : 0;
 }
 
+constexpr int64_t kPass64MinVoxels = 8000000;
+inline int frames_per_pass(int64_t slab_voxels, size_t slot_bytes)
+{
+    if (slot_bytes == 0 || (int64_t)slot_bytes > 4 * slab_voxels) return kMaxFramesPerLaunch;
+    return slab_voxels >= kPass64MinVoxels ? kMaxFramesPerPass : kMaxFramesPerLaunch;
+}
+inline bool pass_frames_ok(int n) { return n == 32 || n == 48 || n == 64; }
+
+constexpr float kFreeRunWeightBound = 16777216.0f - (float)kMaxFramesPerPass;
+
+inline bool claim_counts_fit(int64_t bucket_cap, int frames) { return bucket_cap * (int64_t)frames < (1ll << 32); }
+
 constexpr int64_t kPipelineMaxVoxels = 64000000;
 inline bool pipelines(const tsdf_config &c) { return slab_voxels(c) < kPipelineMaxVoxels; }
 
diff --git a/semantic_slam_amd/csrc/tsdf_capi.hip b/semantic_slam_amd/csrc/tsdf_capi.hip
--- a/semantic_slam_amd/csrc/tsdf_capi.hip
+++ b/semantic_slam_amd/csrc/tsdf_capi.hip
@@ -94,6 +94,9 @@
     Event flush_done[2];
     int flush_parity = 0;
     int table_slot = -1;
+    int table_slot_hi = -1;
+    int pass_frames = tsdfk::kMaxFramesPerLaunch;
+    DevPtr<tsdfk::FramePose> d_frame_blocks;
     int defer_n = tsdfk::kMaxFramesPerLaunch;
     Event pend_copied;
     int pend_count = 0;
@@ -126,6 +129,7 @@
 #ifdef TSDF_EXPERIMENTS
     DevBuf<unsigned int> d_super;
 #endif
+    DevBuf<uint2> d_work_hi;
     DevBuf<uint4> d_work;
     int64_t work_nsuper = 0, work_bucket_supers = 0;
     int work_wedge_mode = -1;
@@ -238,21 +242,28 @@
 
 void store_next_pass(tsdf_volume *v) { v->flush_parity ^= 1; }
 
-int tables_begin(tsdf_volume *v, float2 **tiles, hipStream_t first_user = nullptr)
+int tables_begin(tsdf_volume *v, float2 **tiles, hipStream_t first_user = nullptr, float2 **tiles_hi = nullptr)
 {
     void *dev = nullptr;
-    hipError_t e = tsdf_store::slot_acquire(v->store, &v->store->tables, v, first_user ? first_user : v->stream, true, &v->table_slot, &dev);
+    const hipStream_t s = first_user ? first_user : v->stream;
+    const int quota = tiles_hi ? (s != v->stream ? 4 : 2) : 0;
+    hipError_t e = tsdf_store::slot_acquire(v->store, &v->store->tables, v, s, true, &v->table_slot, &dev, quota);
     if (e != hipSuccess) return fail(TSDF_ERR_HIP, "frame store (tile tables): %s", hipGetErrorString(e));
     *tiles = static_cast<float2 *>(dev);
+    if (tiles_hi) {
+        e = tsdf_store::slot_acquire(v->store, &v->store->tables, v, s, true, &v->table_slot_hi, &dev, quota);
+        if (e != hipSuccess) return fail(TSDF_ERR_HIP, "frame store (tile tables): %s", hipGetErrorString(e));
+        *tiles_hi = static_cast<float2 *>(dev);
+    }
     return TSDF_OK;
 }
 
 int tables_end(tsdf_volume *v)
 {
-    if (v->table_slot < 0) return TSDF_OK;
-    const int slot = v->table_slot;
-    v->table_slot = -1;
-    return store_release(v, &v->store->tables, &slot, 1);
+    if (v->table_slot < 0 && v->table_slot_hi < 0) return TSDF_OK;
+    const int slots[2] = {v->table_slot, v->table_slot_hi};
+    v->table_slot = v->table_slot_hi = -1;
+    return store_release(v, &v->store->tables, slots, 2);
 }
 
 using tsdf_host::brick_shape_ok;
@@ -337,6 +348,10 @@
 }
 
 static_assert(tsdf_host::kMaxFramesPerLaunch == tsdfk::kMaxFramesPerLaunch, "host_derive.h: kMaxFramesPerLaunch");
+static_assert(tsdf_host::kMaxFramesPerPass == tsdfk::kMaxFramesPerPass, "host_derive.h: kMaxFramesPerPass");
+static_assert(tsdf_host::kFreeRunWeightBound == tsdfk::kFreeRunWeightBound, "host_derive.h: kFreeRunWeightBound");
+static_assert(sizeof(tsdfk::MultiParamsInline) + sizeof(tsdfk::BrickListParams) <= 4096 && sizeof(tsdfk::FrameBlockChunk) <= 4096,
+              "kernarg segment: 4 KiB");
 static_assert(tsdf_host::kTileLdsEntries == tsdfk::kTileLdsEntries, "host_derive.h: kTileLdsEntries");
 static_assert(tsdf_host::kFineTile == tsdfk::kFineTile, "host_derive.h: kFineTile");
 static_assert(tsdf_host::kFineLevels == tsdfk::kFineLevels, "host_derive.h: kFineLevels");
@@ -569,13 +584,21 @@
         HIP_TRY(hipGetLastError());
         return TSDF_OK;
     }
+    if (n > tsdfk::kMaxFramesPerPass) return fail(TSDF_ERR_INVALID, "fused launch: %d frames in one pass (at most %d)", n, tsdfk::kMaxFramesPerPass);
     std::memcpy(v->last_cam2base, c2b + 16 * (n - 1), sizeof v->last_cam2base);
     v->flags_known_zero = false;
+    const bool wide = n > tsdfk::kMaxFramesPerLaunch;
+    tsdfk::FramePose blocks[tsdfk::kMaxFramesPerPass];
     tsdfk::MultiParamsInline mi;
     mi.common = make_params(v, depth_dev[0], nullptr, c2b, 4);
     mi.n_frames = n;
-    for (int f = 0; f < n; ++f) fill_pose(mi.frames[f], f);
-    for (int f = n; f < tsdfk::kMaxFramesPerLaunch; ++f) mi.frames[f] = mi.frames[0];
+    mi.frames_ext = nullptr;
+    mi.fine_hi = nullptr;
+    for (int f = 0; f < n; ++f) fill_pose(blocks[f], f);
+    if (wide && !v->d_frame_blocks) {
+        const hipError_t e = dev_alloc(v->d_frame_blocks, 3 * (size_t)tsdfk::kMaxFramesPerPass * sizeof(tsdfk::FramePose));
+        if (e != hipSuccess) return fail(TSDF_ERR_HIP, "frame table: %s", hipGetErrorString(e));
+    }
     mi.labels.label = v->d_label; mi.labels.fp = v->d_fp; mi.labels.bp = v->d_bp; mi.labels.prob_thd = v->prob_thd;
     bool any_mask = false;
     for (int f = 0; f < n && masks_dev; ++f) any_mask = any_mask || masks_dev[f] != nullptr;
@@ -674,6 +697,14 @@
             HIP_TRY(hipStreamSynchronize(v->stream));
         }
         HIP_TRY(v->d_work.ensure(lists * (size_t)total));
+        if (wide) {
+            if (!tsdf_host::claim_counts_fit(cap, n)) return fail(TSDF_ERR_INVALID, "fused launch: %lld bricks per sub-list x %d frames exceed the claim counters", (long long)cap, n);
+            if (!v->d_work_hi.fits(v->d_work.capacity()) && v->d_work_hi) {
+                if (v->pre_stream) HIP_TRY(hipStreamSynchronize(v->pre_stream));
+                HIP_TRY(hipStreamSynchronize(v->stream));
+            }
+            HIP_TRY(v->d_work_hi.ensure(v->d_work.capacity()));
+        }
     }
     const hipStream_t ps = pipelined ? v->pre_stream : v->stream;
     auto unwind = [&](int code) {
@@ -691,15 +722,36 @@
     if (count_claims) mi.common.claim_counter = claims_p + 1;
     if (classify) {
         const size_t per_frame = tsdf_host::tile_table_elems(mi.common.tiles_w, mi.common.tiles_h);
-        float2 *tiles = nullptr;
-        int rc = tables_begin(v, &tiles, ps);
+        float2 *tiles = nullptr, *tiles_hi = nullptr;
+        int rc = tables_begin(v, &tiles, ps, wide ? &tiles_hi : nullptr);
         if (rc) return unwind(rc);
+        const int n_lo = std::min(n, (int)tsdfk::kMaxFramesPerLaunch);
         float2 *fine = v->fine_tables ? tiles + (size_t)tsdfk::kMaxFramesPerLaunch * per_frame : nullptr;
-        rc = build_tile_tables(ps, c, mi.common, depth_dev, masks_dev, n, tiles, claims_p, fine, pipelined);
+        rc = build_tile_tables(ps, c, mi.common, depth_dev, masks_dev, n_lo, tiles, claims_p, fine, pipelined);
         if (rc) return unwind(rc);
         mi.common.fine = fine;
-        for (int f = 0; f < n; ++f) mi.frames[f].tiles = tiles + (size_t)f * per_frame;
-        for (int f = n; f < tsdfk::kMaxFramesPerLaunch; ++f) mi.frames[f] = mi.frames[0];
+        for (int f = 0; f < n_lo; ++f) blocks[f].tiles = tiles + (size_t)f * per_frame;
+        if (wide) {
+            float2 *fine_hi = v->fine_tables ? tiles_hi + (size_t)tsdfk::kMaxFramesPerLaunch * per_frame : nullptr;
+            rc = build_tile_tables(ps, c, mi.common, depth_dev + n_lo, masks_dev ? masks_dev + n_lo : nullptr, n - n_lo, tiles_hi, nullptr, fine_hi, pipelined);
+            if (rc) return unwind(rc);
+            mi.fine_hi = fine_hi;
+            for (int f = n_lo; f < n; ++f) blocks[f].tiles = tiles_hi + (size_t)(f - n_lo) * per_frame;
+        }
+    }
+    if (!wide) {
+        for (int f = 0; f < tsdfk::kMaxFramesPerLaunch; ++f) mi.frames[f] = blocks[f < n ? f : 0];
+    } else {
+        tsdfk::FramePose *table = v->d_frame_blocks + (size_t)(pipelined ? P : 2) * tsdfk::kMaxFramesPerPass;
+        for (int k = 0; k < tsdfk::kMaxFramesPerPass; k += tsdfk::kStageBlocks) {
+            tsdfk::FrameBlockChunk chunk;
+            for (int f = 0; f < tsdfk::kStageBlocks; ++f) chunk.frames[f] = blocks[std::min(k + f, n - 1)];
+            chunk.dst = table + k;
+            chunk.n = tsdfk::kStageBlocks;
+            hipLaunchKernelGGL(tsdfk::stage_frame_blocks, dim3(1), dim3(64), 0, ps, chunk);
+        }
+        for (int f = 0; f < tsdfk::kMaxFramesPerLaunch; ++f) mi.frames[f] = blocks[0];
+        mi.frames_ext = table;
     }
     double claims_total = 0.0;
     bool launched = false;
@@ -713,6 +765,7 @@
         const int64_t per_group = (int64_t)mi.common.brick_groups * mi.common.bricks_per_group;
         uint4 *const work_p = v->d_work + (size_t)P * (v->d_work.capacity() / lists);
         bl.list = work_p;
+        bl.list_hi = wide ? v->d_work_hi + (size_t)P * (v->d_work.capacity() / lists) : nullptr;
         bl.counters = reinterpret_cast<unsigned char *>(claims_p);
         bl.bucket_cap = (unsigned int)cap;
         bl.poses = reinterpret_cast<tsdfk::ClassPoseTable *>(bl.counters + tsdfk::kCounterBytes);
@@ -725,12 +778,13 @@
         const uint4 *wl = work_p;
         const unsigned char *wc = bl.counters;
         const tsdfk::ClassPoseTable *wp = bl.poses;
+        const uint2 *wh = bl.list_hi;
         if (label_ims)
-            hipLaunchKernelGGL((tsdfk::integrate_brick_list<kBrickNT, true, false>), grid_list, block, 0, v->stream, mi, wl, wc, bl.bucket_cap, wp);
+            hipLaunchKernelGGL((tsdfk::integrate_brick_list<kBrickNT, true, false>), grid_list, block, 0, v->stream, mi, wl, wc, bl.bucket_cap, wp, wh);
         else if (any_mask)
-            hipLaunchKernelGGL((tsdfk::integrate_brick_list<kBrickNT, false, true>), grid_list, block, 0, v->stream, mi, wl, wc, bl.bucket_cap, wp);
+            hipLaunchKernelGGL((tsdfk::integrate_brick_list<kBrickNT, false, true>), grid_list, block, 0, v->stream, mi, wl, wc, bl.bucket_cap, wp, wh);
         else
-            hipLaunchKernelGGL((tsdfk::integrate_brick_list<kBrickNT, false, false>), grid_list, block, 0, v->stream, mi, wl, wc, bl.bucket_cap, wp);
+            hipLaunchKernelGGL((tsdfk::integrate_brick_list<kBrickNT, false, false>), grid_list, block, 0, v->stream, mi, wl, wc, bl.bucket_cap, wp, wh);
         claims_total = (double)per_group * nz_groups * n;
         launched = true;
     }
@@ -775,9 +829,9 @@
     return rc_end;
 }
 
-int frames_per_launch(const tsdf_volume *)
-{
-    return tsdfk::kMaxFramesPerLaunch;
+int frames_per_launch(const tsdf_volume *v)
+{
+    return v->pass_frames;
 }
 
 bool can_fuse(const tsdf_volume *v) { return variant_of(v->variant).fuses && v->cfg.dim_x % 4 == 0; }
@@ -790,7 +844,7 @@
     bool seq_event = false;
     for (int k = 0; k < n_frames && rc == TSDF_OK;) {
         const int n = fuse ? std::min(frames_per_launch(v), n_frames - k) : 1;
-        float c2b[16 * tsdfk::kMaxFramesPerLaunch];
+        float c2b[16 * tsdfk::kMaxFramesPerPass];
         for (int i = 0; i < n; ++i) compose_cam2base(v, cam2world + 16 * (k + i), c2b + 16 * i);
         if (fuse && !seq_event && v->seq_ready && v->pipeline_ok && n_frames > n) {
             HIP_TRY(hipEventRecord(v->seq_ready, v->stream));
@@ -1032,6 +1086,8 @@
     if (const char *e = std::getenv("TSDF_PIPELINE")) v->pipeline_ok = std::atoi(e) != 0;
 #endif
     const size_t table_bytes = tsdf_host::launch_table_bytes(*cfg, v->tile, v->fine_tables);
+    v->pass_frames = batch_member ? tsdfk::kMaxFramesPerLaunch : tsdf_host::frames_per_pass(v->n_vox, table_bytes);
+    if (kExperiments) v->pass_frames = tsdfk::kMaxFramesPerLaunch;
     if ((e = tsdf_store::store_ref(cfg->device, (size_t)cfg->im_height * cfg->im_width, table_bytes, &v->store)) != hipSuccess ||
         (e = event_create(v->flush_done[0])) != hipSuccess ||
         (e = event_create(v->flush_done[1])) != hipSuccess ||
@@ -1231,7 +1287,7 @@
     bool seq_event = false;
     for (int k = 0; k < n_frames && rc == TSDF_OK;) {
         const int n = std::min(frames_per_launch(v), n_frames - k);
-        float c2b[16 * tsdfk::kMaxFramesPerLaunch];
+        float c2b[16 * tsdfk::kMaxFramesPerPass];
         for (int i = 0; i < n; ++i) compose_cam2base(v, cam2world + 16 * (k + i), c2b + 16 * i);
         if (!seq_event && v->seq_ready && v->pipeline_ok && n_frames > n) {
             HIP_TRY(hipEventRecord(v->seq_ready, v->stream));
diff --git a/semantic_slam_amd/csrc/tsdf_diag.hip.h b/semantic_slam_amd/csrc/tsdf_diag.hip.h
--- a/semantic_slam_amd/csrc/tsdf_diag.hip.h
+++ b/semantic_slam_amd/csrc/tsdf_diag.hip.h
@@ -356,6 +356,23 @@
     return TSDF_OK;
 }
 
+int tsdf_set_frames_per_pass(tsdf_volume *v, int32_t n_frames)
+{
+    if (!v) return fail(TSDF_ERR_INVALID, "tsdf_set_frames_per_pass: NULL handle");
+    if (n_frames == 0) {
+        const size_t slot = tsdf_host::launch_table_bytes(v->cfg, v->tile, v->fine_tables);
+        v->pass_frames = (v->owner || kExperiments) ? tsdfk::kMaxFramesPerLaunch : tsdf_host::frames_per_pass(v->n_vox, slot);
+        return TSDF_OK;
+    }
+    if (!tsdf_host::pass_frames_ok(n_frames) || (kExperiments && n_frames != tsdfk::kMaxFramesPerLaunch))
+        return fail(TSDF_ERR_INVALID, "tsdf_set_frames_per_pass: %d frames: 32, 48 or 64%s (0: the library's choice)", n_frames,
+                    kExperiments ? " -- and the measurement build takes 32 only" : "");
+    int rc = bind_device(v);
+    if (rc) return rc;
+    v->pass_frames = n_frames;
+    return TSDF_OK;
+}
+
 int tsdf_brick_shape(const tsdf_volume *v, int32_t shape_out[3])
 {
     if (!v || !shape_out) return fail(TSDF_ERR_INVALID, "tsdf_brick_shape: NULL argument");
diff --git a/semantic_slam_amd/csrc/tsdf_multiframe.hip.h b/semantic_slam_amd/csrc/tsdf_multiframe.hip.h
--- a/semantic_slam_amd/csrc/tsdf_multiframe.hip.h
+++ b/semantic_slam_amd/csrc/tsdf_multiframe.hip.h
@@ -4,6 +4,8 @@
 namespace tsdfk {
 
 constexpr int kMaxFramesPerLaunch = 32;
+constexpr int kMaxFramesPerPass = 64;
+constexpr float kFreeRunWeightBound = 16777216.0f - (float)kMaxFramesPerPass;
 constexpr int kFineTile = 4;
 constexpr int kFineLevels = 3;
 __host__ __device__ inline size_t fine_table_elems(int fw, int fh) { return (size_t)kFineLevels * kFineLevels * fw * fh; }
@@ -402,7 +404,7 @@
 static_assert(sizeof(ClassPose) == 64, "four 16-byte words");
 
 struct ClassPoseTable {
-    float4 w[4][kMaxFramesPerLaunch];
+    float4 w[4][kMaxFramesPerPass];
 };
 
 __device__ __forceinline__ ClassPose class_pose(const FramePose &q)
@@ -553,6 +555,8 @@
     FramePose frames[kMaxFramesPerLaunch];
     int n_frames;
     LabelState labels;
+    const FramePose *frames_ext;
+    const float2 *fine_hi;
     int z_fastest;
 #ifdef TSDF_EXPERIMENTS
     const unsigned int *super_mask;
@@ -562,11 +566,55 @@
 
 constexpr int kSuperZ = 4;
 
+__device__ __forceinline__ unsigned long long uniform64(const unsigned long long v)
+{
+    const unsigned int lo = (unsigned int)__builtin_amdgcn_readfirstlane((int)(unsigned int)v);
+    const unsigned int hi = (unsigned int)__builtin_amdgcn_readfirstlane((int)(unsigned int)(v >> 32));
+    return ((unsigned long long)hi << 32) | lo;
+}
+
+__device__ __forceinline__ unsigned long long frames_mask64(const int n) { return n >= 64 ? ~0ull : ((1ull << n) - 1ull); }
+
+__device__ __forceinline__ const FramePose *launch_frames(const MultiParamsInline &mp)
+{
+    typedef const char __attribute__((address_space(4))) *kernarg_ptr;
+    typedef const FramePose __attribute__((address_space(4))) *frames_ptr;
+    const kernarg_ptr base = (kernarg_ptr)__builtin_amdgcn_kernarg_segment_ptr();
+    const frames_ptr in_kernarg = (frames_ptr)(base + offsetof(MultiParamsInline, frames));
+    const frames_ptr ext = (frames_ptr)(uintptr_t)mp.frames_ext;
+    return (const FramePose *)(mp.frames_ext != nullptr ? ext : in_kernarg);
+}
+
+__device__ __forceinline__ const float2 *pass_fine_table(const MultiParamsInline &mp, const int f)
+{
+    const IntegrateParams &p = mp.common;
+    if (p.fine == nullptr) return nullptr;
+    return (f < kMaxFramesPerLaunch ? p.fine : mp.fine_hi) + (size_t)(f & (kMaxFramesPerLaunch - 1)) * fine_table_elems(p.fine_w, p.fine_h);
+}
+
+constexpr int kStageBlocks = kMaxFramesPerLaunch;
+struct FrameBlockChunk {
+    FramePose frames[kStageBlocks];
+    FramePose *dst;
+    int n;
+};
+
+__global__ __launch_bounds__(64) void stage_frame_blocks(FrameBlockChunk c)
+{
+    static_assert(sizeof(FramePose) % 8 == 0, "copied in 8-byte words");
+    constexpr int kWords = (int)(sizeof(FramePose) / 8);
+    static_assert(offsetof(FrameBlockChunk, frames) == 0, "the blocks start the kernarg segment");
+    typedef const unsigned long long __attribute__((address_space(4))) *words_ptr;
+    const words_ptr src = (words_ptr)__builtin_amdgcn_kernarg_segment_ptr();
+    unsigned long long *dst = reinterpret_cast<unsigned long long *>(c.dst);
+    for (int k = threadIdx.x; k < c.n * kWords; k += 64) dst[k] = src[k];
+}
+
 template <int R, bool NT, bool FLAT, bool LABELS = false, bool MASKS = true, bool SHORT = false, bool BRICK = false, bool EAGER_W = false>
 __device__ __forceinline__ void multi_body(const IntegrateParams &p, const FramePose *__restrict__ frames,
                                            const int n_frames, const int b0, const int b1, const int lz,
-                                           const LabelState ls = LabelState(), const unsigned int free_frames = 0u,
-                                           const unsigned int skip_frames = 0u)
+                                           const LabelState ls = LabelState(), const unsigned long long free_frames = 0ull,
+                                           const unsigned long long skip_frames = 0ull)
 {
     static_assert(!SHORT || R == 1, "patch classification is written for one row per lane");
     static_assert(!LABELS || R == 1, "label fusion rides on the one-row kernel");
@@ -748,32 +796,32 @@
         }
     };
 
-    unsigned int todo = n_frames >= 32 ? 0xffffffffu : ((1u << n_frames) - 1u);
+    unsigned long long todo = frames_mask64(n_frames);
     if constexpr (SHORT) {
-        if (p.shortcut_stats != nullptr && (threadIdx.x & 63) == 0 && (skip_frames & todo) != 0u)
-            atomicAdd(p.shortcut_stats + 2, (unsigned)__popc(skip_frames & todo));
+        if (p.shortcut_stats != nullptr && (threadIdx.x & 63) == 0 && (skip_frames & todo) != 0ull)
+            atomicAdd(p.shortcut_stats + 2, (unsigned)__popcll(skip_frames & todo));
         todo &= ~skip_frames;
     }
 #pragma unroll 1
     for (int f = 0; f < n_frames; ++f) {
         if constexpr (SHORT) {
-            if (todo == 0u) break;
-            f = __ffs((int)todo) - 1;
-            todo &= todo - 1u;
-            const bool all_free = (free_frames >> f) & 1u;
+            if (todo == 0ull) break;
+            f = __ffsll((long long)todo) - 1;
+            todo &= todo - 1ull;
+            const bool all_free = (free_frames >> f) & 1ull;
             if (all_free) {
                 if (__ballot(!((touched[0] || have_w) && ones[0] && (fl[0] & 2u))) == 0ull) {
                     touched[0] = true;
-                    const unsigned int rest = ~(free_frames >> f);
-                    unsigned int run = rest != 0u ? (unsigned)(__ffs((int)rest) - 1) : 32u - (unsigned)f;
+                    const unsigned long long rest = ~(free_frames >> f);
+                    unsigned int run = rest != 0ull ? (unsigned)(__ffsll((long long)rest) - 1) : 64u - (unsigned)f;
                     run = min(run, (unsigned)(n_frames - f));
                     const float4 w = w4[0];
                     const bool whole = w.x == truncf(w.x) && w.y == truncf(w.y) && w.z == truncf(w.z) && w.w == truncf(w.w) &&
-                                       fmaxf(fmaxf(w.x, w.y), fmaxf(w.z, w.w)) < 16777184.0f;
+                                       fmaxf(fmaxf(w.x, w.y), fmaxf(w.z, w.w)) < kFreeRunWeightBound;
                     if (run > 1u && __ballot(!whole) == 0ull) {
                         const float k = (float)run;
                         w4[0].x += k; w4[0].y += k; w4[0].z += k; w4[0].w += k;
-                        todo &= ~((run >= 32u ? 0xffffffffu : ((1u << run) - 1u)) << f);
+                        todo &= ~(frames_mask64((int)run) << f);
                         if (p.shortcut_stats != nullptr && (threadIdx.x & 63) == 0) atomicAdd(p.shortcut_stats + 1, run);
                         continue;
                     }
@@ -973,17 +1021,14 @@
 template <int R, bool NT, bool FLAT, bool LABELS = false, bool MASKS = true>
 __global__ __launch_bounds__(256, R == 2 ? 6 : 1) void integrate_multi_inline(MultiParamsInline mp)
 {
-    typedef const char __attribute__((address_space(4))) *kernarg_ptr;
-    kernarg_ptr base = (kernarg_ptr)__builtin_amdgcn_kernarg_segment_ptr();
-    typedef const FramePose __attribute__((address_space(4))) *frames_ptr;
-    frames_ptr frames = (frames_ptr)(base + offsetof(MultiParamsInline, frames));
+    const FramePose *frames = launch_frames(mp);
     const int wg_x = mp.z_fastest ? (int)blockIdx.z : (int)blockIdx.x, wg_y = (int)blockIdx.y;
     int wg_z = mp.z_fastest ? (int)blockIdx.x : (int)blockIdx.z;
     if (mp.z_fastest == 2) {
         wg_z += (int)((unsigned)(wg_x + wg_y) % gridDim.x);
         if (wg_z >= (int)gridDim.x) wg_z -= (int)gridDim.x;
     }
-    multi_body<R, NT, FLAT, LABELS, MASKS>(mp.common, (const FramePose *)frames, mp.n_frames, wg_x, wg_y, wg_z, mp.labels);
+    multi_body<R, NT, FLAT, LABELS, MASKS>(mp.common, frames, mp.n_frames, wg_x, wg_y, wg_z, mp.labels);
 }
 
 constexpr int kSuperBX = 4, kSuperBY = 2, kSuperBZ = 1;
@@ -993,6 +1038,7 @@
 
 struct BrickListParams {
     uint4 *list;
+    uint2 *list_hi;
     unsigned char *counters;
     unsigned int bucket_cap;
     ClassPoseTable *poses;
@@ -1016,9 +1062,7 @@
 
 __global__ __launch_bounds__(256) void classify_brick_list(MultiParamsInline mp, BrickListParams bl)
 {
-    typedef const char __attribute__((address_space(4))) *kernarg_ptr;
-    kernarg_ptr base = (kernarg_ptr)__builtin_amdgcn_kernarg_segment_ptr();
-    const FramePose *frames = (const FramePose *)(base + offsetof(MultiParamsInline, frames));
+    const FramePose *frames = launch_frames(mp);
     const IntegrateParams &p = mp.common;
     const int id = (int)blockIdx.x * 4 + __builtin_amdgcn_readfirstlane((int)threadIdx.y), lane = threadIdx.x;
     if (id >= bl.nsx * bl.nsy * bl.nsz) return;
@@ -1026,25 +1070,28 @@
     const int nzg = (p.nz + p.brick_s - 1) / p.brick_s;
     const int i0 = sx * kSuperBX, g0 = sy * kSuperBY, zg0 = sz * kSuperBZ;
     const int i1 = min(i0 + kSuperBX, p.bricks_per_group) - 1, g1 = min(g0 + kSuperBY, p.brick_groups) - 1, zg1 = min(zg0 + kSuperBZ, nzg) - 1;
-    const unsigned int frames_mask = mp.n_frames >= 32 ? 0xffffffffu : ((1u << mp.n_frames) - 1u);
-    static_assert(kMaxFramesPerLaunch == 32, "one frame per lane of a half-wave");
+    const unsigned long long frames_mask = frames_mask64(mp.n_frames);
+    static_assert(kMaxFramesPerLaunch == 32 && kMaxFramesPerPass == 64, "one frame per lane of a half-wave, or of the wavefront");
     const int xa = i0 * p.brick_q * 4, xb = (i1 + 1) * p.brick_q * 4 - 1;
     const int ya = g0 * p.brick_r, yb = min((g1 + 1) * p.brick_r, p.dim_y) - 1;
     const int z0 = zg0 * p.brick_s, z1 = min((zg1 + 1) * p.brick_s, p.nz) - 1;
-    const ClassPose mine_q = class_pose(frames[lane & 31]);
-    if (id == 0 && lane < kMaxFramesPerLaunch) class_pose_store(bl.poses, lane, mine_q);
-    const float2 *fine_f = p.fine != nullptr ? p.fine + (size_t)(lane & 31) * fine_table_elems(p.fine_w, p.fine_h) : nullptr;
-    const int cls = classify_patch<true>(p, mine_q, xa, xb, ya, yb, p.z_begin + z0, p.z_begin + z1, fine_f);
-    const unsigned int super_free = (unsigned int)__ballot(cls == 1) & frames_mask;
-    const unsigned int super_skip = (unsigned int)__ballot(cls == 2) & frames_mask;
+    const bool wide = mp.n_frames > kMaxFramesPerLaunch;
+    const int my_frame = wide ? min(lane, mp.n_frames - 1) : (lane & 31);
+    const ClassPose mine_q = class_pose(frames[my_frame]);
+    if (id == 0 && lane < (wide ? kMaxFramesPerPass : kMaxFramesPerLaunch)) class_pose_store(bl.poses, lane, mine_q);
+    const float2 *fine_f = pass_fine_table(mp, my_frame);
+    const int cls = wide ? classify_patch<false>(p, mine_q, xa, xb, ya, yb, p.z_begin + z0, p.z_begin + z1, fine_f)
+                         : classify_patch<true>(p, mine_q, xa, xb, ya, yb, p.z_begin + z0, p.z_begin + z1, fine_f);
+    const unsigned long long super_free = __ballot(cls == 1) & frames_mask;
+    const unsigned long long super_skip = __ballot(cls == 2) & frames_mask;
     const int n_in = (i1 - i0 + 1) * (g1 - g0 + 1) * (zg1 - zg0 + 1);
     static_assert(kListBuckets == 64, "six bits: list_bucket");
     const unsigned int bkt = list_bucket((unsigned int)id, sx, sy, sz, bl);
     unsigned char *bucket = bl.counters + (size_t)bkt * kBucketStride;
     if (lane == 0) {
-        if (p.claim_counter != nullptr && (super_free | super_skip) != 0u)
+        if (p.claim_counter != nullptr && (super_free | super_skip) != 0ull)
             atomicAdd(reinterpret_cast<unsigned long long *>(bucket + 8),
-                      ((unsigned long long)(n_in * __popc(super_free)) << 32) | (unsigned long long)(n_in * __popc(super_skip)));
+                      ((unsigned long long)(n_in * __popcll(super_free)) << 32) | (unsigned long long)(n_in * __popcll(super_skip)));
         if (p.shortcut_stats != nullptr) {
             if (super_skip == frames_mask) { atomicAdd(p.shortcut_stats + 2, (unsigned)(n_in * mp.n_frames)); atomicAdd(p.shortcut_stats + 3, 1u); }
             else {
@@ -1064,20 +1111,21 @@
     if (lane == 0) at = atomicAdd(reinterpret_cast<unsigned int *>(bucket) + (undecided ? 0 : 1), n_live);
     at = __builtin_amdgcn_readfirstlane(at);
     at = bkt * bl.bucket_cap + (undecided ? at : bl.bucket_cap - at - n_live);
-    if (mine)
-        bl.list[at + (unsigned)__popcll(live_mask & ((1ull << lane) - 1ull))] =
-            make_uint4((unsigned)(g * p.bricks_per_group + i) | undecided, (unsigned)zg, super_free, super_skip);
+    if (mine) {
+        const unsigned int slot = at + (unsigned)__popcll(live_mask & ((1ull << lane) - 1ull));
+        bl.list[slot] = make_uint4((unsigned)(g * p.bricks_per_group + i) | undecided, (unsigned)zg, (unsigned int)super_free, (unsigned int)super_skip);
+        if (wide) bl.list_hi[slot] = make_uint2((unsigned int)(super_free >> 32), (unsigned int)(super_skip >> 32));
+    }
 }
 
 template <bool NT, bool LABELS, bool MASKS>
 __global__ __launch_bounds__(256, LABELS ? 6 : TSDF_BRICK_WAVES) void integrate_brick_list(MultiParamsInline mp, const uint4 *__restrict__ list,
                                                                                           const unsigned char *__restrict__ counters,
                                                                                           const unsigned int bucket_cap,
-                                                                                          const ClassPoseTable *__restrict__ poses)
-{
-    typedef const char __attribute__((address_space(4))) *kernarg_ptr;
-    kernarg_ptr base = (kernarg_ptr)__builtin_amdgcn_kernarg_segment_ptr();
-    const FramePose *frames = (const FramePose *)(base + offsetof(MultiParamsInline, frames));
+                                                                                          const ClassPoseTable *__restrict__ poses,
+                                                                                          const uint2 *__restrict__ list_hi)
+{
+    const FramePose *frames = launch_frames(mp);
     const unsigned int b = blockIdx.x % kListBuckets, grp = blockIdx.x / kListBuckets;
     const unsigned int wave = (unsigned)__builtin_amdgcn_readfirstlane((int)threadIdx.y);
     const uint2 n = *reinterpret_cast<const uint2 *>(counters + (size_t)b * kBucketStride);
@@ -1093,21 +1141,30 @@
     }
     const uint4 e = list[(size_t)b * bucket_cap + at];
     const int brick = (int)(e.x & ~kBrickUndecided), zg = (int)e.y;
-    unsigned int free_frames = e.z, skip_frames = e.w;
+    unsigned long long free_frames = e.z, skip_frames = e.w;
+    const bool wide = mp.n_frames > kMaxFramesPerLaunch;
+    if (wide) {
+        const uint2 h = list_hi[(size_t)b * bucket_cap + at];
+        free_frames |= (unsigned long long)h.x << 32;
+        skip_frames |= (unsigned long long)h.y << 32;
+    }
     if (e.x & kBrickUndecided) {
         const IntegrateParams &p = mp.common;
         const int lane = threadIdx.x;
-        const unsigned int frames_mask = mp.n_frames >= 32 ? 0xffffffffu : ((1u << mp.n_frames) - 1u);
+        const unsigned long long frames_mask = frames_mask64(mp.n_frames);
         const int g = brick / p.bricks_per_group, i = brick - g * p.bricks_per_group;
         const int xa = i * p.brick_q * 4, ya = g * p.brick_r;
+        const int xb = xa + p.brick_q * 4 - 1, yb = min(ya + p.brick_r - 1, p.dim_y - 1);
         const int z0 = zg * p.brick_s, z1 = min(z0 + p.brick_s - 1, p.nz - 1);
-        const float2 *fine_f = p.fine != nullptr ? p.fine + (size_t)(lane & 31) * fine_table_elems(p.fine_w, p.fine_h) : nullptr;
-        const int cls = classify_patch<true>(p, class_pose(poses, lane & 31), xa, xa + p.brick_q * 4 - 1, ya, min(ya + p.brick_r - 1, p.dim_y - 1),
-                                             p.z_begin + z0, p.z_begin + z1, fine_f);
-        free_frames |= (unsigned int)__ballot(cls == 1) & frames_mask;
-        skip_frames |= (unsigned int)__ballot(cls == 2) & frames_mask;
-        free_frames = __builtin_amdgcn_readfirstlane(free_frames);
-        skip_frames = __builtin_amdgcn_readfirstlane(skip_frames);
+        const int my_frame = wide ? lane : (lane & 31);
+        const float2 *fine_f = pass_fine_table(mp, my_frame);
+        const ClassPose my_q = class_pose(poses, my_frame);
+        const int cls = wide ? classify_patch<false>(p, my_q, xa, xb, ya, yb, p.z_begin + z0, p.z_begin + z1, fine_f)
+                             : classify_patch<true>(p, my_q, xa, xb, ya, yb, p.z_begin + z0, p.z_begin + z1, fine_f);
+        free_frames |= __ballot(cls == 1) & frames_mask;
+        skip_frames |= __ballot(cls == 2) & frames_mask;
+        free_frames = uniform64(free_frames);
+        skip_frames = uniform64(skip_frames);
         if (skip_frames == frames_mask) {
             if (p.shortcut_stats != nullptr && lane == 0) { atomicAdd(p.shortcut_stats + 2, (unsigned)mp.n_frames); atomicAdd(p.shortcut_stats + 6, 1u); }
             return;
```

Result: no change. 421,900 (-0.8%).
